# syamajala/cholesky

Measured on AMD Instinct MI355X. Metric: fp64 factorization GF/s (numeric level loop, F_ref flops) on 3-D Laplacian, higher is better.
Workload: dtype f64; 1 GPU; tests/lapl_3375x3375 (reference fixture: 7-point Laplacian, nested-dissection ordering from the fixture files); n=3375, levels=5, separators=31, B_alg_bytes=2932064, parallelism=single GPU, precision=fp64

## Files before the change

### cholesky_amd/_lib.py

```python
import ctypes as C
import os

_HERE = os.path.dirname(os.path.abspath(__file__))
LIB_PATH = os.environ.get("CHOLAMD_LIB") or os.path.join(_HERE, "lib", "libcholamd.so")
HEADER_PATH = os.path.join(os.path.dirname(_HERE), "include", "cholamd.h")


class Filled(C.Structure):
    _fields_ = [("filled", C.c_int), ("sep_x", C.c_int), ("sep_y", C.c_int), ("interval", C.c_int), ("cluster", C.c_int),
                ("lo_x", C.c_int), ("lo_y", C.c_int), ("hi_x", C.c_int), ("hi_y", C.c_int)]


class Op(C.Structure):
    _fields_ = [("op", C.c_int), ("level", C.c_int), ("m", C.c_int), ("n", C.c_int), ("k", C.c_int),
                ("a_sx", C.c_int), ("a_sy", C.c_int), ("a_z", C.c_int), ("b_sx", C.c_int), ("b_sy", C.c_int), ("b_z", C.c_int),
                ("c_sx", C.c_int), ("c_sy", C.c_int), ("c_z", C.c_int)]


class Region(C.Structure):
    _fields_ = [("ptr", C.c_void_p), ("ld", C.c_int), ("lo_x", C.c_int), ("lo_y", C.c_int), ("hi_x", C.c_int), ("hi_y", C.c_int),
                ("tile_row", C.POINTER(C.c_int))]


class SepInfo(C.Structure):
    _fields_ = [("levels", C.c_int), ("num_separators", C.c_int)]


_lib = None


def load():
    global _lib
    if _lib is not None:
        return _lib
    if not os.path.exists(LIB_PATH):
        raise ImportError(f"{LIB_PATH} is missing: run `make` (or __graft_entry__.build()) first; "
                          "cholesky_amd has no fallback path without its HIP library")
    try:
        import torch
    except ImportError:
        pass
    L = C.CDLL(LIB_PATH)
    vp, ci, cd, i64 = C.c_void_p, C.c_int, C.c_double, C.c_int64
    L.cholamd_last_error.restype = C.c_char_p
    L.cholamd_version.restype = C.c_char_p
    L.cholamd_read_separators.argtypes = [C.c_char_p, ci, vp, vp, C.POINTER(SepInfo)]
    L.cholamd_read_clusters.argtypes = [C.c_char_p, vp, vp, vp, i64, C.POINTER(i64)]
    L.cholamd_read_matrix.argtypes = [C.c_char_p, ci, vp, vp, vp]
    L.cholamd_read_vector.argtypes = [C.c_char_p, ci, vp]
    L.cholamd_write_solution.argtypes = [C.c_char_p, vp, ci, ci]
    L.cholamd_plan_create.argtypes = [C.c_char_p, C.c_char_p, C.c_char_p, C.POINTER(vp)]
    L.cholamd_plan_create_from_arrays.argtypes = [ci, ci, vp, vp, vp, vp, vp, i64, i64, vp, vp, vp, C.c_char_p, C.POINTER(vp)]
    L.cholamd_plan_destroy.argtypes = [vp]
    L.cholamd_generate_laplacian.argtypes = [ci, ci, ci, ci, ci, C.POINTER(vp)]
    L.cholamd_problem_destroy.argtypes = [vp]
    L.cholamd_problem_n.argtypes = [vp]
    L.cholamd_problem_nz.argtypes = [vp]
    L.cholamd_problem_write.argtypes = [vp, C.c_char_p]
    L.cholamd_plan_create_from_problem.argtypes = [vp, C.POINTER(vp)]
    L.cholamd_problem_rhs.argtypes = [vp, vp]
    for f in ("n", "nz", "levels", "num_separators", "max_int_size", "num_blocks"):
        getattr(L, "cholamd_plan_" + f).argtypes = [vp]
    for f in ("arena_doubles", "dropped_entries", "num_ops", "nnz_a", "nnz_l", "alg_bytes"):
        fn = getattr(L, "cholamd_plan_" + f)
        fn.argtypes = [vp]
        fn.restype = i64
    L.cholamd_plan_nnz_tiles.argtypes = [vp]
    L.cholamd_plan_nnz_tiles.restype = i64
    L.cholamd_plan_fmin.argtypes = [vp]
    L.cholamd_plan_fmin.restype = cd
    L.cholamd_plan_banner.argtypes = [vp]
    L.cholamd_plan_banner.restype = C.c_char_p
    for f in ("perm", "sep_sizes", "sep_offsets", "tree", "blocks", "ops"):
        getattr(L, "cholamd_plan_" + f).argtypes = [vp, vp]
    L.cholamd_plan_snapshot_count.argtypes = [vp, ci]
    L.cholamd_plan_snapshot_count.restype = i64
    L.cholamd_plan_snapshot.argtypes = [vp, ci, vp]
    L.cholamd_plan_counts.argtypes = [vp, ci, vp, vp]
    L.cholamd_plan_flops.argtypes = [vp]
    L.cholamd_plan_flops.restype = cd
    L.cholamd_plan_fill_host.argtypes = [vp, vp]
    L.cholamd_plan_arena_to_dense.argtypes = [vp, vp, vp]
    L.cholamd_plan_entries.argtypes = [vp, vp, vp]
    L.cholamd_plan_value_map.argtypes = [vp, vp]
    L.cholamd_plan_fill_host_values.argtypes = [vp, vp, i64, vp]
    L.cholamd_device_set_values.argtypes = [vp, vp, i64, ci, vp]
    L.cholamd_device_values_status.argtypes = [vp, vp, vp]
    L.cholamd_plan_fill_host_part.argtypes = [vp, vp, ci, ci, C.POINTER(i64)]
    L.cholamd_plan_level_work_counts.argtypes = [vp, ci, ci, ci, vp]
    L.cholamd_plan_level_work_volume.argtypes = [vp, ci, ci, ci, ci, vp]
    L.cholamd_plan_program_check.argtypes = [vp, ci, ci]
    L.cholamd_plan_program_check_opts.argtypes = [vp, ci, ci, ci, ci]
    L.cholamd_plan_program_counts.argtypes = [vp, ci, vp]
    L.cholamd_plan_program_jobs.argtypes = [vp, ci, i64, vp]
    L.cholamd_plan_program_jobs.restype = i64
    L.cholamd_plan_write_matrix.argtypes = [vp, vp, C.c_char_p, ci]
    L.cholamd_plan_write_debug_log.argtypes = [vp, vp]
    L.cholamd_device_create.argtypes = [vp, ci, C.POINTER(vp)]
    L.cholamd_device_destroy.argtypes = [vp]
    L.cholamd_device_set_partition.argtypes = [vp, ci, ci]
    L.cholamd_device_set_option.argtypes = [vp, C.c_char_p, ci]
    L.cholamd_comm_unique_id.argtypes = [vp]
    L.cholamd_comm_create.argtypes = [vp, ci, ci, vp, C.POINTER(vp)]
    L.cholamd_comm_create_local.argtypes = [vp, ci, vp]
    L.cholamd_factor_multi.argtypes = [vp, vp, vp, ci, vp]
    L.cholamd_gather_factor.argtypes = [vp, vp, ci, vp]
    L.cholamd_comm_adopt.argtypes = [vp, ci, ci, C.POINTER(vp)]
    L.cholamd_comm_destroy.argtypes = [vp]
    L.cholamd_comm_destroy.restype = None
    L.cholamd_comm_allreduce.argtypes = [vp, vp, i64, vp]
    L.cholamd_device_tail_offset.argtypes = [vp]
    L.cholamd_device_tail_offset.restype = i64
    L.cholamd_exchange_tail.argtypes = [vp, vp, vp, vp]
    L.cholamd_factor_sharded.argtypes = [vp, vp, vp, vp]
    L.cholamd_factor_sharded_f32.argtypes = [vp, vp, vp, vp]
    L.cholamd_gather_to_root.argtypes = [vp, vp, ci, vp, vp]
    L.cholamd_exchange_volume.argtypes = [vp, vp]
    L.cholamd_plan_exchange_volume.argtypes = [vp, ci, ci, ci, vp]
    L.cholamd_plan_exchange_pieces.argtypes = [vp, ci, ci, ci, vp]
    L.cholamd_plan_solve_counts.argtypes = [vp, ci, ci, ci, vp]
    L.cholamd_plan_solve_skips.argtypes = [vp, ci, vp, vp]
    L.cholamd_solve_sharded.argtypes = [vp, vp, vp, vp, vp, vp]
    L.cholamd_solve_sharded_f32.argtypes = [vp, vp, vp, vp, vp, vp]
    L.cholamd_solve_refine_sharded.argtypes = [vp, vp, vp, vp, ci, C.c_double, vp, vp, vp, vp]
    L.cholamd_solve_multi.argtypes = [vp, vp, vp, vp, vp, ci, vp]
    L.cholamd_solve_refine_multi.argtypes = [vp, vp, vp, vp, ci, C.c_double, vp, vp, vp, ci, vp]
    L.cholamd_follow_rounds.argtypes = [ci, ci, ci, vp, vp]
    L.cholamd_plan_program_followers.argtypes = [vp, i64, vp]
    L.cholamd_plan_program_followers.restype = i64
    L.cholamd_factor_multi_f32.argtypes = [vp, vp, vp, ci, vp]
    L.cholamd_gather_factor_f32.argtypes = [vp, vp, ci, vp]
    L.cholamd_device_alloc.argtypes = [vp, i64, C.POINTER(vp)]
    L.cholamd_device_free.argtypes = [vp, vp]
    L.cholamd_device_upload.argtypes = [vp, vp, vp, i64, vp]
    L.cholamd_device_download.argtypes = [vp, vp, vp, i64, vp]
    L.cholamd_device_sync.argtypes = [vp, vp]
    L.cholamd_device_fill.argtypes = [vp, vp, vp]
    L.cholamd_factor.argtypes = [vp, vp, vp]
    L.cholamd_factor_levels.argtypes = [vp, vp, ci, ci, vp]
    L.cholamd_device_program_trace.argtypes = [vp, vp, vp, i64, vp, C.POINTER(ci)]
    L.cholamd_factor_info.argtypes = [vp, C.POINTER(ci)]
    L.cholamd_solve.argtypes = [vp, vp, vp, vp, vp]
    L.cholamd_device_fill_f32.argtypes = [vp, vp, vp]
    L.cholamd_factor_f32.argtypes = [vp, vp, vp]
    L.cholamd_factor_levels_f32.argtypes = [vp, vp, ci, ci, vp]
    L.cholamd_solve_f32.argtypes = [vp, vp, vp, vp, vp]
    L.cholamd_solve_refine.argtypes = [vp, vp, vp, vp, ci, cd, C.POINTER(ci), C.POINTER(cd), vp]
    L.cholamd_residual.argtypes = [vp, vp, vp, vp, C.POINTER(cd), vp]
    L.cholamd_solve_nrhs.argtypes = [vp, vp, vp, i64, vp, i64, ci, vp]
    L.cholamd_solve_nrhs_f32.argtypes = [vp, vp, vp, i64, vp, i64, ci, vp]
    L.cholamd_solve_refine_nrhs.argtypes = [vp, vp, vp, i64, vp, i64, ci, ci, cd, C.POINTER(ci), vp, vp]
    L.cholamd_solve_half.argtypes = [vp, vp, vp, vp, ci, vp]
    L.cholamd_solve_half_f32.argtypes = [vp, vp, vp, vp, ci, vp]
    L.cholamd_solve_half_nrhs.argtypes = [vp, vp, vp, i64, vp, i64, ci, ci, vp]
    L.cholamd_solve_half_nrhs_f32.argtypes = [vp, vp, vp, i64, vp, i64, ci, ci, vp]
    L.cholamd_factor_logdet.argtypes = [vp, vp, C.POINTER(cd), vp]
    L.cholamd_factor_logdet_f32.argtypes = [vp, vp, C.POINTER(cd), vp]
    L.cholamd_factor_diag.argtypes = [vp, vp, vp, vp]
    L.cholamd_factor_diag_f32.argtypes = [vp, vp, vp, vp]
    L.cholamd_plan_diag_list.argtypes = [vp, vp, vp, vp, vp, vp, vp]
    L.cholamd_selinv.argtypes = [vp, vp, vp, vp]
    L.cholamd_selinv_diag.argtypes = [vp, vp, vp, vp]
    L.cholamd_selinv_entries.argtypes = [vp, vp, vp, i64, vp]
    L.cholamd_plan_selinv_blocks.argtypes = [vp, ci]
    L.cholamd_plan_selinv_front.argtypes = [vp, ci, ci, ci, vp, vp, vp]
    L.cholamd_device_alloc_arena.argtypes = [vp, ci, C.POINTER(vp), C.POINTER(C.c_int64)]
    L.cholamd_device_free_arena.argtypes = [vp, vp]
    L.cholamd_device_set_timing.argtypes = [vp, ci]
    L.cholamd_device_get_timing.argtypes = [vp, vp, vp]
    L.cholamd_device_get_timing_ex.argtypes = [vp, vp, vp]
    L.cholamd_device_bcast_phases.argtypes = [vp]
    L.cholamd_comm_count.argtypes = [vp, C.POINTER(ci)]
    L.cholamd_device_event_overhead.argtypes = [vp, vp, C.POINTER(C.c_float)]
    RP, FP = C.POINTER(Region), C.POINTER(Filled)
    L.cholamd_plan_region.argtypes = [vp, vp, ci, ci, RP]
    L.cholamd_plan_level_work_volume_opts.argtypes = [vp, ci, ci, ci, vp]
    L.cholamd_plan_level_mt_fill.argtypes = [vp, ci, vp]
    L.cholamd_plan_arena_dense_doubles.argtypes = [vp]
    L.cholamd_plan_arena_dense_doubles.restype = C.c_int64
    L.cholamd_plan_block_tile_map.argtypes = [vp, ci, ci, vp]
    L.cholamd_fused_dpotrf.argtypes = [RP, FP, ci, ci, ci, ci, vp]
    L.cholamd_fused_dtrsm.argtypes = [RP, RP, FP, ci, FP, ci, ci, ci, ci, vp]
    L.cholamd_fused_dsyrk.argtypes = [RP, RP, RP, FP, ci, FP, ci, FP, ci, ci, ci, ci, ci, vp]
    L.cholamd_fused_dgemm.argtypes = [RP, RP, RP, FP, ci, FP, ci, FP, ci, ci, ci, ci, ci, vp]
    L.cholamd_LAPACKE_dpotrf.argtypes = [ci, C.c_char, ci, vp, ci]
    L.cholamd_cblas_dtrsm.argtypes = [ci, ci, ci, ci, ci, ci, ci, cd, vp, ci, vp, ci]
    L.cholamd_cblas_dtrsm.restype = None
    L.cholamd_cblas_dgemm.argtypes = [ci, ci, ci, ci, ci, ci, cd, vp, ci, vp, ci, cd, vp, ci]
    L.cholamd_cblas_dgemm.restype = None
    L.cholamd_cblas_dsyrk.argtypes = [ci, ci, ci, ci, ci, cd, vp, ci, cd, vp, ci]
    L.cholamd_cblas_dsyrk.restype = None
    L.cholamd_cblas_dtrsv.argtypes = [ci, ci, ci, ci, ci, vp, ci, vp, ci]
    L.cholamd_cblas_dtrsv.restype = None
    L.cholamd_cblas_dgemv.argtypes = [ci, ci, ci, ci, cd, vp, ci, vp, ci, cd, vp, ci]
    L.cholamd_cblas_dgemv.restype = None
    L.cholamd_openblas_set_num_threads.argtypes = [ci]
    L.cholamd_openblas_set_num_threads.restype = None
    L.cholamd_dpotrf_dev.argtypes = [ci, vp, ci, vp, vp]
    L.cholamd_dtrsm_dev.argtypes = [ci, ci, vp, ci, vp, ci, vp]
    L.cholamd_dgemm_dev.argtypes = [ci, ci, ci, vp, ci, vp, ci, vp, ci, vp]
    L.cholamd_dsyrk_dev.argtypes = [ci, ci, vp, ci, vp, ci, vp]
    L.cholamd_dtrsv_dev.argtypes = [ci, ci, vp, ci, vp, vp]
    L.cholamd_dgemv_dev.argtypes = [ci, ci, ci, vp, ci, vp, vp, vp]
    _lib = L
    return L


class CholamdError(RuntimeError):
    pass


def check(rc, what=""):
    if rc != 0:
        msg = load().cholamd_last_error().decode(errors="replace")
        raise CholamdError(f"{what} failed with code {rc}: {msg}")
```

### cholesky_amd/csrc/chol_api.cpp

```cpp
#include <hip/hip_runtime.h>
#include <rccl/rccl.h>

#include <cstdio>
#include <algorithm>
#include <cstdlib>
#include <cfloat>
#include <cmath>
#include <cstring>
#include <string>
#include <type_traits>
#include <vector>

#include "chol_kernels.h"
#include "chol_plan.h"
#include "cholamd.h"

#define HIPCHK(call)                                                                                  \
  do {                                                                                                \
    hipError_t e_ = (call);                                                                           \
    if (e_ != hipSuccess) {                                                                           \
      chol_set_error("%s failed: %s (%s:%d)", #call, hipGetErrorString(e_), __FILE__, __LINE__);     \
      return (e_ == hipErrorNoDevice || e_ == hipErrorInvalidDevice) ? CHOLAMD_ERR_NO_DEVICE : CHOLAMD_ERR_HIP; \
    }                                                                                                 \
  } while (0)

struct level_dev {
  int n_potrf = 0, n_trsm = 0, n_task = 0, n_src = 0;
  std::vector<chol_phase> phase;
  chol_potrf_desc *potrf = nullptr;
  chol_trsm_desc *trsm = nullptr;
  chol_upd_task *task = nullptr, *task_mt = nullptr;
  chol_upd_src *src = nullptr;
  std::vector<chol_bcast> bcast;
};
struct solve_dev {
  int n_trsv = 0, n_grp = 0, n_fw = 0, n_bw = 0;
  chol_trsv_desc *trsv = nullptr;
  chol_gemv_desc *fw = nullptr, *bw = nullptr;
  int *grp_start = nullptr, *grp_rows = nullptr, *bw_start = nullptr;
  int n_ifw = 0, n_ibw = 0, max_n = 0, max_under = 0;
  int64_t w256_off = -1;
  int *ifw = nullptr, *ibw = nullptr;
};
struct selinv_dev {
  std::vector<chol_selinv_sep> host;
  chol_selinv_sep *sep = nullptr; chol_selinv_tile *tile = nullptr;
  int *chain_ld = nullptr, *chain_pos0 = nullptr; int64_t *rowoff = nullptr;
  int max_nblk = 0;
};
struct timed_launch { hipEvent_t a, b; int kind; };

struct cholamd_device {
  struct vmm_arena { void *va; size_t total; std::vector<hipMemGenericAllocationHandle_t> handles; };
  std::vector<vmm_arena> vmm;

  const cholamd_plan *plan = nullptr;
  int dev = 0, rank = 0, world = 1;
  std::vector<level_dev> lv;
  std::vector<solve_dev> sv;
  bool solve_ready = false;
  int solve_rank = 0, solve_world = 1;
  int *zr_sub = nullptr; int n_zr_sub = 0;
  double *ws = nullptr;
  double *ws_solve = nullptr;
  int *step_flags = nullptr;
  int step_gen = 0;
  double *w256 = nullptr;
  double *step_xt = nullptr;
  bool keep_inverses = false;
  int *info = nullptr;
  int *info_last = nullptr;
  int info_parity = 0; bool info_foreign = false;
  int *progress = nullptr;
  int epoch = 0, done_total = 0;
  int64_t *a_dst = nullptr; double *a_val = nullptr; int *perm = nullptr; double *ytmp = nullptr;
  int64_t *top_dst[2] = { nullptr, nullptr }; double *top_val[2] = { nullptr, nullptr }; int *top_e[2] = { nullptr, nullptr }; int64_t top_n[2] = { 0, 0 }; int top_gen[2] = { -1, -1 };
  int *a_src = nullptr, *csr_src = nullptr; unsigned char *e_cls = nullptr;
  int64_t *vs_dev = nullptr, *vs_init = nullptr, *vs_host = nullptr;
  int64_t vs_last[4] = { 0, 0, 0, 0 };
  bool vs_called = false, vs_last_valid = false;
  bool vs_in_force = false;
  bool f32_pending = false;
  bool timing = false;
  std::vector<timed_launch> tl;
  std::vector<hipEvent_t> pool;
  level_dev prog;
  chol_job *jobs = nullptr; chol_wait *pwaits = nullptr; chol_ext *exts = nullptr;
  int *pctr = nullptr, *pctr_total = nullptr;
  int n_job = 0, n_pctr = 0, prog_grid = 0, prog_epoch = 0, prog_epoch_limit = 0;
  bool prog_ready = false;
  unsigned long long *trace = nullptr;
  std::vector<chol_job> jobs_host;
  std::vector<level_dev> lv32;
  float *ws32 = nullptr;
  int f32_range = -1; int64_t f32_bad = -1;
  int64_t *csr_ptr = nullptr; int *csr_col = nullptr; double *csr_val = nullptr;
  double *rvec = nullptr, *dxvec = nullptr, *partial = nullptr;
  void *xstage = nullptr; size_t xstage_bytes = 0; void *xdesc = nullptr; int xdesc_gen = -1, xdesc_elem = 0, sched_gen = 0;
  chol_sched_opts opt;
  bool solve_reference_shape = false;
  double *ynrhs = nullptr, *bnrhs = nullptr, *rnrhs = nullptr, *dxnrhs = nullptr, *pnrhs = nullptr;
  chol_trsv_desc *dg_desc = nullptr; int *dg_prefix = nullptr; int n_dg = 0;
  double *ld_part = nullptr; int64_t *ld_ipart = nullptr, *ld_res = nullptr;
  std::vector<selinv_dev> si; double *si_ws = nullptr; bool si_ready = false;
};

static int no_device_error()
{
  chol_set_error("no usable HIP device (libcholamd has no CPU fallback)");
  return CHOLAMD_ERR_NO_DEVICE;
}

extern "C" int cholamd_device_count(void)
{
  int n = 0;
  if (hipGetDeviceCount(&n) != hipSuccess) return 0;
  return n;
}

template <class T> static int upload_vec(T **dptr, const T *h, size_t n)
{
  *dptr = nullptr;
  if (n == 0) return 0;
  HIPCHK(hipMalloc((void **)dptr, n * sizeof(T)));
  HIPCHK(hipMemcpy(*dptr, h, n * sizeof(T), hipMemcpyHostToDevice));
  return 0;
}

#define CHOL_POISON_GUARD ((size_t)64 << 10)
static bool poison_on()
{
  const char *e = std::getenv("CHOLAMD_POISON");
  return e && *e && atoi(e) != 0;
}
static hipError_t poison_fill(void *p, size_t bytes)
{
  hipError_t e = hipMemset(p, 0xFF, bytes);
  return e == hipSuccess ? hipDeviceSynchronize() : e;
}
static hipError_t fp_malloc(void **dptr, size_t bytes)
{
  if (!poison_on()) return hipMalloc(dptr, bytes);
  hipError_t e = hipMalloc(dptr, bytes + CHOL_POISON_GUARD);
  return e == hipSuccess ? poison_fill(*dptr, bytes + CHOL_POISON_GUARD) : e;
}

static void free_level(level_dev &l)
{
  (void)hipFree(l.potrf); (void)hipFree(l.trsm); (void)hipFree(l.task); (void)hipFree(l.task_mt); (void)hipFree(l.src);
  l = level_dev();
}
static void free_levels(cholamd_device *d)
{
  for (auto &l : d->lv) free_level(l);
  d->lv.clear();
  for (auto &l : d->lv32) free_level(l);
  d->lv32.clear();
  free_level(d->prog);
  (void)hipFree(d->jobs); (void)hipFree(d->pwaits); (void)hipFree(d->exts); (void)hipFree(d->pctr); (void)hipFree(d->pctr_total);
  d->jobs = nullptr; d->pwaits = nullptr; d->exts = nullptr; d->pctr = nullptr; d->pctr_total = nullptr;
  d->prog_ready = false;
}
static void free_solve_lists(cholamd_device *d)
{
  for (auto &s : d->sv) { (void)hipFree(s.trsv); (void)hipFree(s.fw); (void)hipFree(s.bw); (void)hipFree(s.grp_start); (void)hipFree(s.grp_rows); (void)hipFree(s.bw_start); (void)hipFree(s.ifw); (void)hipFree(s.ibw); }
  d->sv.clear();
  (void)hipFree(d->w256); d->w256 = nullptr;
  (void)hipFree(d->dg_desc); d->dg_desc = nullptr; (void)hipFree(d->dg_prefix); d->dg_prefix = nullptr; d->n_dg = 0;
  (void)hipFree(d->zr_sub); d->zr_sub = nullptr; d->n_zr_sub = 0;
  d->solve_ready = false;
}
static void free_selinv(cholamd_device *d)
{
  for (auto &l : d->si) { (void)hipFree(l.sep); (void)hipFree(l.tile); (void)hipFree(l.chain_ld); (void)hipFree(l.chain_pos0); (void)hipFree(l.rowoff); }
  d->si.clear();
  (void)hipFree(d->si_ws); d->si_ws = nullptr;
  d->si_ready = false;
}
static int upload_level(level_dev &l, const chol_level_work &w, bool with_tables = true)
{
  l.n_potrf = w.n_potrf; l.n_trsm = w.n_trsm; l.n_task = w.n_task; l.n_src = w.n_src;
  l.phase.assign(w.phase, w.phase + w.n_phase);
  l.bcast.assign(w.bcast, w.bcast + w.n_bcast);
  int rc = 0;
  if (w.n_potrf > 0 && with_tables && !std::getenv("CHOLAMD_NO_ROLE_TABLES")) {
    const size_t dbytes = ((size_t)w.n_potrf * sizeof(chol_potrf_desc) + 15) / 16 * 16;
    std::vector<unsigned char> buf(dbytes + (size_t)w.n_potrf * CHOL_RR_TAB_BYTES);
    for (int i = 0; i < w.n_potrf; i++) {
      chol_potrf_desc pd = w.potrf[i];
      if (pd.n <= CHOL_RR_MAXN) {
        const size_t at = dbytes + (size_t)i * CHOL_RR_TAB_BYTES;
        pd.tab = (int)(at - (size_t)i * sizeof(chol_potrf_desc));
        chol_potrf_table(pd.n, pd.sky, buf.data() + at);
      }
      std::memcpy(buf.data() + (size_t)i * sizeof(chol_potrf_desc), &pd, sizeof pd);
    }
    HIPCHK(hipMalloc((void **)&l.potrf, buf.size()));
    HIPCHK(hipMemcpy(l.potrf, buf.data(), buf.size(), hipMemcpyHostToDevice));
  } else rc = upload_vec(&l.potrf, w.potrf, (size_t)w.n_potrf);
  if (!rc) rc = upload_vec(&l.trsm, w.trsm, (size_t)w.n_trsm);
  if (!rc) rc = upload_vec(&l.task, w.task, (size_t)w.n_task);
  if (!rc) rc = upload_vec(&l.task_mt, w.task_mt, (size_t)w.n_task_mt);
  if (!rc) rc = upload_vec(&l.src, w.src, (size_t)w.n_src);
  return rc;
}

static int build_levels(cholamd_device *d)
{
  free_levels(d);
  d->sched_gen++;
  const int L = d->plan->levels;
  d->lv.resize(L);
  for (int lvl = 0; lvl < L; lvl++) {
    chol_level_work w;
    int rc = chol_build_level_work(d->plan, &d->opt, lvl, d->rank, d->world, &w);
    if (rc) return rc;
    rc = upload_level(d->lv[lvl], w);
    chol_level_work_free(&w);
    if (rc) return rc;
  }
  if (d->world == 1 && d->opt.program) {
    chol_level_work w;
    chol_program g;
    const bool built = chol_build_program(d->plan, &d->opt, &w, &g) == 0;
    const bool live = built && chol_program_check_built(d->plan, &d->opt, 4, &w, &g) == 0;
    if (built && !live) { chol_level_work_free(&w); chol_program_free(&g); }
    if (live) {
      int rc = upload_level(d->prog, w);
      std::vector<int> tot(g.ctr_total, g.ctr_total + g.n_ctr);
      int ncu = 256;
      hipDeviceProp_t prop;
      if (hipGetDeviceProperties(&prop, d->dev) == hipSuccess && prop.multiProcessorCount > 0) ncu = prop.multiProcessorCount;
      d->prog_grid = g.n_job < ncu ? g.n_job : ncu;
      tot.push_back(g.n_job + d->prog_grid);
      int mx = 1;
      for (int t : tot) mx = t > mx ? t : mx;
      d->prog_epoch_limit = (1 << 30) / mx;
      d->n_job = g.n_job; d->n_pctr = (int)tot.size(); d->prog_epoch = 0;
      d->jobs_host.assign(g.job, g.job + g.n_job);
      if (!rc) rc = upload_vec(&d->jobs, g.job, (size_t)g.n_job);
      const chol_wait no_wait = { 0, 0 };
      chol_ext no_ext;
      std::memset(&no_ext, 0, sizeof no_ext);
      if (!rc) rc = g.n_wait > 0 ? upload_vec(&d->pwaits, g.wait, (size_t)g.n_wait) : upload_vec(&d->pwaits, &no_wait, (size_t)1);
      if (!rc) rc = g.n_ext > 0 ? upload_vec(&d->exts, g.ext, (size_t)g.n_ext) : upload_vec(&d->exts, &no_ext, (size_t)1);
      if (!rc) rc = upload_vec(&d->pctr_total, tot.data(), tot.size());
      if (!rc) {
        HIPCHK(hipMalloc((void **)&d->pctr, tot.size() * sizeof(int)));
        HIPCHK(hipMemset(d->pctr, 0, tot.size() * sizeof(int)));
      }
      chol_level_work_free(&w);
      chol_program_free(&g);
      if (rc) return rc;
      d->prog_ready = d->n_job > 0;
    }
  }
  return 0;
}

extern "C" int cholamd_device_create(const cholamd_plan *plan, int device_id, cholamd_device **out)
{
  *out = nullptr;
  if (!plan) { chol_set_error("null plan"); return CHOLAMD_ERR_ARG; }
  int ndev = 0;
  if (hipGetDeviceCount(&ndev) != hipSuccess || ndev <= 0) return no_device_error();
  if (device_id < 0 || device_id >= ndev) { chol_set_error("device %d out of range (%d devices)", device_id, ndev); return CHOLAMD_ERR_NO_DEVICE; }
  HIPCHK(hipSetDevice(device_id));
  cholamd_device *d = new cholamd_device();
  d->plan = plan; d->dev = device_id;
  chol_sched_opts_from_env(&d->opt);
  { const char *e = getenv("CHOLAMD_SOLVE_REFERENCE_SHAPE"); d->solve_reference_shape = e && *e && atoi(e) != 0; }
  int rc = build_levels(d);
  if (!rc) {
    hipError_t e = fp_malloc((void **)&d->ws, (size_t)(plan->ws_doubles > 0 ? plan->ws_doubles : 1) * sizeof(double));
    if (e == hipSuccess) e = hipMalloc((void **)&d->info, 4 * sizeof(int));
    if (e == hipSuccess) e = hipMemset(d->info, 0, 4 * sizeof(int));
    if (e == hipSuccess) e = hipMalloc((void **)&d->progress, (size_t)(plan->nsep + 2) * sizeof(int));
    if (e == hipSuccess) e = hipMemset(d->progress, 0, (size_t)(plan->nsep + 2) * sizeof(int));
    if (e != hipSuccess) { chol_set_error("hipMalloc: %s", hipGetErrorString(e)); rc = CHOLAMD_ERR_HIP; }
  }
  if (!rc) rc = upload_vec(&d->a_dst, plan->a_dst, (size_t)plan->nnz_a);
  if (!rc) rc = upload_vec(&d->a_val, plan->a_val, (size_t)plan->nnz_a);
  if (!rc) rc = upload_vec(&d->perm, plan->perm, (size_t)plan->n);
  if (rc) { cholamd_device_destroy(d); return rc; }
  *out = d;
  return 0;
}

extern "C" void cholamd_device_destroy(cholamd_device *d)
{
  if (!d) return;
  (void)hipSetDevice(d->dev);
  free_levels(d);
  for (auto &a : d->vmm) {
    (void)hipDeviceSynchronize();
    (void)hipMemUnmap(a.va, a.total);
    for (auto h : a.handles) (void)hipMemRelease(h);
    (void)hipMemAddressFree(a.va, a.total);
  }
  free_solve_lists(d);
  free_selinv(d);
  (void)hipFree(d->ws32); (void)hipFree(d->csr_ptr); (void)hipFree(d->csr_col); (void)hipFree(d->csr_val); (void)hipFree(d->rvec); (void)hipFree(d->dxvec); (void)hipFree(d->partial);
  (void)hipFree(d->xstage); (void)hipFree(d->xdesc);
  (void)hipFree(d->ws); (void)hipFree(d->ws_solve); (void)hipFree(d->step_flags); (void)hipFree(d->w256); (void)hipFree(d->step_xt); (void)hipFree(d->info); (void)hipFree(d->progress); (void)hipFree(d->a_dst); (void)hipFree(d->a_val); (void)hipFree(d->perm); (void)hipFree(d->ytmp);
  (void)hipFree(d->ld_part); (void)hipFree(d->ld_ipart); (void)hipFree(d->ld_res);
  (void)hipFree(d->ynrhs); (void)hipFree(d->bnrhs); (void)hipFree(d->rnrhs); (void)hipFree(d->dxnrhs); (void)hipFree(d->pnrhs);
  for (int q = 0; q < 2; q++) { (void)hipFree(d->top_dst[q]); (void)hipFree(d->top_val[q]); (void)hipFree(d->top_e[q]); }
  (void)hipFree(d->a_src); (void)hipFree(d->csr_src); (void)hipFree(d->e_cls); (void)hipFree(d->vs_dev); (void)hipFree(d->vs_init); (void)hipHostFree(d->vs_host);
  for (auto &t : d->tl) { d->pool.push_back(t.a); d->pool.push_back(t.b); }
  for (auto e : d->pool) (void)hipEventDestroy(e);
  delete d;
}

extern "C" int cholamd_device_set_partition(cholamd_device *d, int rank, int world)
{
  HIPCHK(hipSetDevice(d->dev));
  if (world < 1 || (world & (world - 1)) || rank < 0 || rank >= world || chol_split_level(world) > d->plan->levels - 1) {
    chol_set_error("bad partition: rank %d of %d for a %d-level tree", rank, world, d->plan->levels);
    return CHOLAMD_ERR_ARG;
  }
  d->rank = rank; d->world = world;
  free_solve_lists(d);
  return build_levels(d);
}

extern "C" int cholamd_device_bcast_phases(const cholamd_device *d)
{
  int n = 0;
  for (const level_dev &l : d->lv) for (const chol_phase &ph : l.phase) n += ph.kind == 6;
  return n;
}
extern "C" int cholamd_device_set_option(cholamd_device *d, const char *name, int value)
{
  HIPCHK(hipSetDevice(d->dev));
  const std::string n(name ? name : "");
  bool rebuild = true;
  if (n == "split_min") d->opt.split_min = value;
  else if (n == "split_nb") d->opt.split_nb = value;
  else if (n == "fuse") d->opt.fuse = value != 0;
  else if (n == "fuse_update_max") d->opt.fuse_update_max = value;
  else if (n == "mt_min_tiles") d->opt.mt_min_tiles = value;
  else if (n == "cells") d->opt.cells = value != 0;
  else if (n == "program") d->opt.program = value != 0;
  else if (n == "follow") d->opt.follow = value != 0;
  else if (n == "super_blocks") d->opt.super_blocks = value;
  else if (n == "follow_tail") d->opt.follow_tail = value;
  else if (n == "follow_tail_split") d->opt.follow_tail_split = value;
  else if (n == "staged") d->opt.staged = value != 0;
  else if (n == "fine_upd") d->opt.fine_upd = value != 0;
  else if (n == "skyline") d->opt.skyline = value != 0;
  else if (n == "merge_targets") d->opt.merge_targets = value != 0;
  else if (n == "leaf_envelope") d->opt.leaf_envelope = value != 0;
  else if (n == "trsm_wt_min") d->opt.trsm_wt_min = value < 0 ? 0 : value;
  else if (n == "stage_chunk") d->opt.stage_chunk = value < 0 ? 0 : value;
  else if (n == "dist_top") d->opt.dist_top = value;
  else if (n == "solve_reference_shape") { d->solve_reference_shape = value != 0; rebuild = false; }
  else { chol_set_error("unknown option '%s'", n.c_str()); return CHOLAMD_ERR_ARG; }
  return rebuild ? build_levels(d) : 0;
}

extern "C" int cholamd_device_alloc(cholamd_device *d, int64_t doubles, double **dptr)
{
  HIPCHK(hipSetDevice(d->dev));
  HIPCHK(fp_malloc((void **)dptr, (size_t)doubles * sizeof(double)));
  return 0;
}
extern "C" int cholamd_device_free(cholamd_device *d, double *dptr)
{
  HIPCHK(hipSetDevice(d->dev));
  HIPCHK(hipFree(dptr));
  return 0;
}
extern "C" int cholamd_device_upload(cholamd_device *d, double *d_dst, const double *h_src, int64_t doubles, void *stream)
{
  HIPCHK(hipSetDevice(d->dev));
  HIPCHK(hipMemcpyAsync(d_dst, h_src, (size_t)doubles * sizeof(double), hipMemcpyHostToDevice, (hipStream_t)stream));
  HIPCHK(hipStreamSynchronize((hipStream_t)stream));
  return 0;
}
extern "C" int cholamd_device_download(cholamd_device *d, double *h_dst, const double *d_src, int64_t doubles, void *stream)
{
  HIPCHK(hipSetDevice(d->dev));
  HIPCHK(hipMemcpyAsync(h_dst, d_src, (size_t)doubles * sizeof(double), hipMemcpyDeviceToHost, (hipStream_t)stream));
  HIPCHK(hipStreamSynchronize((hipStream_t)stream));
  return 0;
}
extern "C" int cholamd_device_sync(cholamd_device *d, void *stream)
{
  HIPCHK(hipSetDevice(d->dev));
  HIPCHK(hipStreamSynchronize((hipStream_t)stream));
  return 0;
}

static void owned_ranges(const cholamd_device *d, std::vector<std::pair<int64_t, int64_t>> &out)
{
  const cholamd_plan *p = d->plan;
  out.clear();
  if (d->world <= 1 || d->rank == 0) { out.push_back({ 0, p->arena }); return; }
  for (int s = 1; s <= p->nsep; s++) {
    const int o = chol_owner_of(p, s, d->world);
    if (o >= 0 && o != d->rank) continue;
    const int64_t lo = p->panel_off[s], hi = s < p->nsep ? p->panel_off[s + 1] : p->arena;
    if (!out.empty() && out.back().second == lo) out.back().second = hi; else out.push_back({ lo, hi });
  }
}
static int clear_owned(cholamd_device *d, void *arena, size_t elem, hipStream_t st)
{
  bool sharded = false;
  for (const auto &v : d->vmm) if (v.va == arena) sharded = true;
  if (!sharded) { HIPCHK(hipMemsetAsync(arena, 0, (size_t)d->plan->arena * elem, st)); return 0; }
  std::vector<std::pair<int64_t, int64_t>> r;
  owned_ranges(d, r);
  for (auto &x : r) HIPCHK(hipMemsetAsync((char *)arena + (size_t)x.first * elem, 0, (size_t)(x.second - x.first) * elem, st));
  return 0;
}
#define CHOL_VMM_CHUNK ((size_t)2 << 20)
#define CHOL_VMM_SCRATCH ((size_t)64 << 20)
extern "C" int cholamd_device_alloc_arena(cholamd_device *d, int elem_bytes, void **dptr, int64_t *backed_bytes)
{
  HIPCHK(hipSetDevice(d->dev));
  if (elem_bytes != 4 && elem_bytes != 8) { chol_set_error("alloc_arena: element size %d", elem_bytes); return CHOLAMD_ERR_ARG; }
  const size_t full = (size_t)d->plan->arena * (size_t)elem_bytes;
  if (d->world <= 1 || d->rank == 0) {
    HIPCHK(fp_malloc(dptr, full > 0 ? full : 1));
    if (backed_bytes) *backed_bytes = (int64_t)full;
    return 0;
  }
  hipMemAllocationProp prop = {};
// ... 141 lines not shown
{
  float ms[CHOL_TIMING_KINDS]; int n[CHOL_TIMING_KINDS];
  const int rc = cholamd_device_get_timing_ex(d, ms, n);
  if (rc) return rc;
  for (int k = 0; k < 4; k++) { ms_by_kind[k] = ms[k]; launches_by_kind[k] = n[k]; }
  return 0;
}

extern "C" int cholamd_device_event_overhead(cholamd_device *d, void *stream, float *ms_out)
{
  HIPCHK(hipSetDevice(d->dev));
  hipStream_t st = (hipStream_t)stream;
  const int reps = 64;
  std::vector<hipEvent_t> ev(2 * reps);
  for (auto &e : ev) e = get_event(d);
  for (int i = 0; i < reps; i++) { HIPCHK(hipEventRecord(ev[2 * i], st)); HIPCHK(hipEventRecord(ev[2 * i + 1], st)); }
  HIPCHK(hipStreamSynchronize(st));
  double acc = 0.0;
  for (int i = 0; i < reps; i++) { float ms = 0.f; HIPCHK(hipEventElapsedTime(&ms, ev[2 * i], ev[2 * i + 1])); acc += ms; }
  for (auto e : ev) d->pool.push_back(e);
  *ms_out = (float)(acc / reps);
  return 0;
}

static int launch_phase(cholamd_device *d, const level_dev &l, const chol_phase &ph, double *d_arena, hipStream_t st)
{
  if (ph.kind == 5) {
    if (d->epoch >= (1 << 24) || d->done_total >= (1 << 30)) { HIPCHK(hipMemsetAsync(d->progress, 0, (size_t)(d->plan->nsep + 2) * sizeof(int), st)); d->epoch = 0; d->done_total = 0; }
    d->epoch++;
    if (ph.n3 > 0) d->done_total += (ph.n2 + 2) / 3;
    HIPCHK((hipError_t)chol_launch_potrf_trsm(d_arena, d->ws, l.potrf + ph.first, ph.n, l.trsm + ph.first2, ph.n2, l.task + ph.first3, l.src, ph.n3,
                                              d->info, d->progress, d->epoch * 64, d->progress + d->plan->nsep + 1, d->done_total, st));
  } else if (ph.kind == 0) HIPCHK((hipError_t)chol_launch_potrf(d_arena, d->ws, l.potrf + ph.first, ph.n, d->info, st));
  else if (ph.kind == 1) HIPCHK((hipError_t)chol_launch_trsm(d_arena, d->ws, l.trsm + ph.first, ph.n, st));
  else if (ph.kind == 4) HIPCHK((hipError_t)chol_launch_trsm_w(d_arena, d->ws, l.trsm + ph.first, ph.n, st));
  else if (ph.kind == 7) HIPCHK((hipError_t)chol_launch_trsm_wt(d_arena, d->ws, l.trsm + ph.first, ph.n, st));
  else if (ph.kind == 2) HIPCHK((hipError_t)chol_launch_update(d_arena, l.task + ph.first, l.src, ph.n, st));
  else if (ph.kind == 3) HIPCHK((hipError_t)chol_launch_update_mt(d_arena, l.task_mt + ph.first, l.src, ph.n, (int64_t)d->plan->arena, st));
  return 0;
}
struct cholamd_comm;
static int bcast_rank(cholamd_device *d, const level_dev &l, const chol_phase &ph, double *d_arena, cholamd_comm *c, hipStream_t st);
static int factor_levels_comm(cholamd_device *d, double *d_arena, int level_hi, int level_lo, cholamd_comm *c, hipStream_t st)
{
  HIPCHK(hipSetDevice(d->dev));
  const int L = d->plan->levels;
  if (level_hi >= L) level_hi = L - 1;
  if (level_lo < 0) level_lo = 0;
  if (level_hi == L - 1) HIPCHK(hipMemsetAsync(d->info, 0, 2 * sizeof(int), st));
  d->info_last = d->info; d->info_foreign = true;
  for (int lvl = level_hi; lvl >= level_lo; lvl--) {
    const level_dev &l = d->lv[lvl];
    for (const chol_phase &ph : l.phase) {
      if (ph.kind == 6) {
        scoped_timer t(d, st, CHOL_TK_BCAST, ph.n > 0);
        int rc = bcast_rank(d, l, ph, d_arena, c, st);
        if (rc) return rc;
        continue;
      }
      scoped_timer t(d, st, ph.kind == 3 ? 2 : (ph.kind == 4 || ph.kind == 7) ? 1 : ph.kind == 5 ? 0 : ph.kind, ph.n > 0);
      int rc = launch_phase(d, l, ph, d_arena, st);
      if (rc) return rc;
    }
  }
  return 0;
}
extern "C" int cholamd_factor_levels(cholamd_device *d, double *d_arena, int level_hi, int level_lo, void *stream)
{
  return factor_levels_comm(d, d_arena, level_hi, level_lo, nullptr, (hipStream_t)stream);
}
extern "C" int cholamd_factor(cholamd_device *d, double *d_arena, void *stream)
{
  if (!d->prog_ready) return cholamd_factor_levels(d, d_arena, d->plan->levels - 1, 0, stream);
  HIPCHK(hipSetDevice(d->dev));
  hipStream_t st = (hipStream_t)stream;
  if (d->info_foreign) { HIPCHK(hipMemsetAsync(d->info, 0, 4 * sizeof(int), st)); d->info_foreign = false; }
  int *const info_cur = d->info + 2 * d->info_parity, *const info_next = d->info + 2 * (d->info_parity ^ 1);
  d->info_parity ^= 1; d->info_last = info_cur;
  if (d->prog_epoch >= d->prog_epoch_limit) { HIPCHK(hipMemsetAsync(d->pctr, 0, (size_t)d->n_pctr * sizeof(int), st)); d->prog_epoch = 0; }
  const level_dev &l = d->prog;
  {
    scoped_timer t(d, st, 3, true);
    HIPCHK((hipError_t)chol_launch_program(d_arena, d->ws, d->jobs, d->n_job, d->pwaits, l.potrf, l.trsm, l.task, l.src, d->exts, d->pctr, d->pctr_total, d->prog_epoch,
                                           d->pctr + d->n_pctr - 1, d->prog_epoch * (d->n_job + d->prog_grid), d->prog_grid, info_cur, info_next, d->trace, st));
  }
  d->prog_epoch++;
  return 0;
}
extern "C" int cholamd_device_program_trace(cholamd_device *d, double *d_arena, void *stream, int64_t cap, int64_t *out, int *njobs_out)
{
  HIPCHK(hipSetDevice(d->dev));
  if (!d->prog_ready) { chol_set_error("no program launch for this problem / these options"); return CHOLAMD_ERR_ARG; }
  *njobs_out = d->n_job;
  if (cap < (int64_t)5 * d->n_job) return 0;
  const size_t nst = (size_t)(4 + CHOL_TRACE_X) * d->n_job;
  HIPCHK(hipMalloc((void **)&d->trace, nst * sizeof(unsigned long long)));
  HIPCHK(hipMemset(d->trace, 0, nst * sizeof(unsigned long long)));
  int rc = cholamd_factor(d, d_arena, stream);
  std::vector<unsigned long long> h(nst);
  if (!rc) {
    HIPCHK(hipStreamSynchronize((hipStream_t)stream));
    HIPCHK(hipMemcpy(h.data(), d->trace, h.size() * sizeof(unsigned long long), hipMemcpyDeviceToHost));
  }
  (void)hipFree(d->trace);
  d->trace = nullptr;
  if (rc) return rc;
  unsigned long long t0 = ~0ull;
  for (int j = 0; j < d->n_job; j++) if (h[4 * j] && h[4 * j] < t0) t0 = h[4 * j];
  for (int j = 0; j < d->n_job; j++) {
    out[5 * j] = d->jobs_host[j].kind + (d->jobs_host[j].kind == 0 && d->jobs_host[j].n_ext > 0 ? 10 : 0);
    for (int q = 0; q < 3; q++) out[5 * j + 1 + q] = (int64_t)(h[4 * j + q] - t0);
    out[5 * j + 4] = (int64_t)h[4 * j + 3];
  }
  if (const char *path = getenv("CHOLAMD_TRACE_FOLLOW")) {
    if (FILE *fp = fopen(path, "w")) {
      for (int j = 0; j < d->n_job; j++) {
        const unsigned long long *x = &h[(size_t)4 * d->n_job + (size_t)CHOL_TRACE_X * j];
        const int kind = d->jobs_host[j].kind;
        bool any = false;
        for (int i = 0; i < CHOL_TRACE_X; i++) any = any || x[i] != 0;
        if (kind == 2 || !any) continue;
        fprintf(fp, "job %d kind %d", j, kind);
        if (kind == 0 && x[1]) {
          fprintf(fp, " items %llu own-tiles-wait-over %.1f rounds:", x[1], x[0] ? (double)(x[0] - t0) * 0.01 : -1.0);
          for (unsigned long long i = 0; i < x[1] && i < 44; i++) if (x[2 + i]) fprintf(fp, " %llu:%.1f", i, (double)(x[2 + i] - t0) * 0.01);
        }
        if (kind == 0 && x[24]) { fprintf(fp, " | prologue (entry, LDS init, tables, slot tables read, columns 0-1 requested, tiles requested, columns 0-1 parked):"); const int ord[7] = { 0, 1, 2, 5, 6, 3, 4 }; for (int k = 0; k < 7; k++) fprintf(fp, " %.1f", x[24 + ord[k]] ? (double)(x[24 + ord[k]] - t0) * 0.01 : -1.0); }
        fprintf(fp, kind == 0 ? " | column started:" : " | POTRF column seen:");
        for (int k = 0; k < 24; k++) if (x[72 + k]) fprintf(fp, " %d:%.1f", k, (double)(x[72 + k] - t0) * 0.01);
        fprintf(fp, kind == 0 ? " | column published:" : " | column tile on the channel:");
        for (int k = 0; k < 24; k++) if (x[48 + k]) fprintf(fp, " %d:%.1f", k, (double)(x[48 + k] - t0) * 0.01);
        fprintf(fp, "\n");
      }
      fclose(fp);
    }
  }
  return 0;
}
extern "C" int cholamd_factor_info(cholamd_device *d, int *sep_out)
{
  HIPCHK(hipSetDevice(d->dev));
  int h[2] = { 0, 0 };
  HIPCHK(hipMemcpy(h, d->info_last ? d->info_last : d->info, sizeof h, hipMemcpyDeviceToHost));
  if (sep_out) *sep_out = h[1];
  if (h[0] == CHOLAMD_ERR_STALL)
    chol_set_error("factorisation stalled: a workgroup of a fused launch waited ~50 ms for a progress word of the same launch and gave up; the factor is not valid");
  else if (h[0] < 0) chol_set_error("factorisation failed with internal code %d", h[0]);
  return h[0];
}

__global__ void k_zero_ranges(double *y, const int *ranges, int nr)
{
  const int off = ranges[2 * blockIdx.y], len = ranges[2 * blockIdx.y + 1];
  for (int i = blockIdx.x * blockDim.x + threadIdx.x; i < len; i += gridDim.x * blockDim.x) y[off + i] = 0.0;
}
static int build_solve(cholamd_device *d, int rank = 0, int world = 1)
{
  const int L = d->plan->levels;
  if (d->solve_ready && d->solve_rank == rank && d->solve_world == world) return 0;
  free_solve_lists(d);
  d->solve_rank = rank; d->solve_world = world;
  d->sv.resize(L);
  if (world > 1) {
    const cholamd_plan *p = d->plan;
    std::vector<int> zr;
    for (int s = 1; s <= p->nsep; s++) {
      const int o = chol_owner_of(p, s, world);
      if ((o >= 0 && o != rank) || (o < 0 && rank != 0)) {
        if (!zr.empty() && zr[zr.size() - 2] + zr.back() == p->sep_off[s]) zr.back() += p->sep_size[s];
        else { zr.push_back(p->sep_off[s]); zr.push_back(p->sep_size[s]); }
      }
    }
    d->n_zr_sub = (int)zr.size() / 2;
    if (!zr.empty()) { int rc = upload_vec(&d->zr_sub, zr.data(), zr.size()); if (rc) return rc; }
  }
  std::vector<chol_trsv_desc> diag;
  for (int lvl = 0; lvl < L; lvl++) {
    chol_solve_level w;
    int rc = chol_build_solve_level_part(d->plan, lvl, rank, world, &w);
    if (rc) return rc;
    if (world == 1) diag.insert(diag.end(), w.trsv, w.trsv + w.n_trsv);
    solve_dev &s = d->sv[lvl];
    s.n_trsv = w.n_trsv; s.n_grp = w.n_grp; s.n_fw = w.n_fw; s.n_bw = w.n_bw;
    rc = upload_vec(&s.trsv, w.trsv, (size_t)w.n_trsv);
    if (!rc) rc = upload_vec(&s.fw, w.fw, (size_t)w.n_fw);
    if (!rc) rc = upload_vec(&s.bw, w.bw, (size_t)w.n_bw);
    if (!rc) rc = upload_vec(&s.grp_start, w.grp_start, (size_t)w.n_grp + 1);
    if (!rc) rc = upload_vec(&s.grp_rows, w.grp_rows, (size_t)2 * w.n_grp);
    if (!rc) rc = upload_vec(&s.bw_start, w.bw_start, (size_t)w.n_trsv + 1);
    s.n_ifw = w.n_ifw; s.n_ibw = w.n_ibw; s.max_n = w.max_n; s.max_under = w.banded && w.max_rows_under_span > 0 ? -w.max_rows_under_span : w.max_rows_under_span;
    if (!rc) rc = upload_vec(&s.ifw, w.ifw, (size_t)4 * w.n_ifw);
    if (!rc) rc = upload_vec(&s.ibw, w.ibw, (size_t)4 * w.n_ibw);
    chol_solve_level_free(&w);
    if (rc) return rc;
  }
  if (!diag.empty()) {
    std::vector<int> prefix(diag.size() + 1);
    int rc = chol_diag_list(d->plan, diag.data(), (int)diag.size(), prefix.data());
    if (!rc) rc = upload_vec(&d->dg_desc, diag.data(), diag.size());
    if (!rc) rc = upload_vec(&d->dg_prefix, prefix.data(), prefix.size());
    if (rc) return rc;
    d->n_dg = (int)diag.size();
  }
  if (!d->ytmp) HIPCHK(fp_malloc((void **)&d->ytmp, (size_t)d->plan->n * sizeof(double)));
  if (!d->ws_solve) HIPCHK(fp_malloc((void **)&d->ws_solve, (size_t)(d->plan->ws_doubles > 0 ? d->plan->ws_doubles : 1) * sizeof(double)));
  if (!d->step_flags) { HIPCHK(hipMalloc((void **)&d->step_flags, CHOL_STEPW_MAX_SEPS * 16 * sizeof(int))); HIPCHK(hipMemset(d->step_flags, 0, CHOL_STEPW_MAX_SEPS * 16 * sizeof(int))); }
  if (!d->step_xt) { HIPCHK(fp_malloc((void **)&d->step_xt, CHOL_STEPW_MAX_SEPS * 256 * sizeof(double))); HIPCHK(hipMemset(d->step_xt, 0, CHOL_STEPW_MAX_SEPS * 256 * sizeof(double))); }
  int64_t w256 = 0;
  if (!std::getenv("CHOLAMD_SOLVE_NO_INV256"))
    for (int lvl = 0; lvl < L; lvl++) {
      solve_dev &s = d->sv[lvl];
      if (s.n_trsv < 1 || s.n_trsv > CHOL_STEPW_MAX_SEPS || s.max_n <= 256 || s.max_under < 0) continue;
      s.w256_off = w256;
      w256 += (int64_t)s.n_trsv * ((s.max_n + 255) / 256) * 65536;
    }
  if (w256 > 0) HIPCHK(fp_malloc((void **)&d->w256, (size_t)w256 * sizeof(double)));
  d->solve_ready = true;
  return 0;
}

// ... 1889 lines not shown
```

### cholesky_amd/csrc/chol_kernels.h

```cpp
#ifndef CHOL_KERNELS_H
#define CHOL_KERNELS_H
#include <hip/hip_runtime_api.h>
#include <stdint.h>
#include "chol_plan.h"
#ifdef __cplusplus
extern "C" {
#endif
int chol_launch_scatter(double *arena, const int64_t *dst, const double *val, int64_t nnz, hipStream_t st);
#define CHOL_VALUES_STATUS 1
#define CHOL_VALUES_GATHER 2
int chol_launch_set_values(const double *vals, int64_t nz, const unsigned char *cls, double *a_val, const int *a_src, int64_t nnz_a,
                           double *csr_val, const int *csr_src, int64_t ncsr, int parts, int64_t *status, hipStream_t st);
int chol_launch_gather(double *out, const double *in, const int *idx, int64_t n, hipStream_t st);
int chol_launch_potrf(double *base, double *ws, const chol_potrf_desc *descs, int n, int *info, hipStream_t st);
int chol_launch_potrf_big(double *base, double *ws, const chol_potrf_desc *descs, int n, int *info, hipStream_t st);
int chol_launch_potrf_trsm(double *base, double *ws, const chol_potrf_desc *pdescs, int n_potrf, const chol_trsm_desc *tdescs, int n_trsm,
                           const chol_upd_task *tasks, const chol_upd_src *srcs, int n_task,
                           int *info, int *progress, int progress_base, int *done, int done_target, hipStream_t st);
int chol_launch_program(double *base, double *ws, const chol_job *jobs, int njobs, const chol_wait *waits, const chol_potrf_desc *pdescs, const chol_trsm_desc *tdescs,
                        const chol_upd_task *tasks, const chol_upd_src *srcs, const chol_ext *exts, int *ctr, const int *ctr_total, int epoch, int *head, int head_base,
                        int grid, int *info, int *info_next, unsigned long long *trace, hipStream_t st);
int chol_launch_trsm_w(double *base, const double *ws, const chol_trsm_desc *descs, int n, hipStream_t st);
int chol_launch_trsm_wt(double *base, const double *ws, const chol_trsm_desc *descs, int n, hipStream_t st);
int chol_launch_trsm_big(double *base, const double *ws, const chol_trsm_desc *descs, int n, hipStream_t st);
int chol_launch_dinv(const double *L, int n, int ldl, double *W, hipStream_t st);
int chol_launch_trsm(double *base, const double *ws, const chol_trsm_desc *descs, int n, hipStream_t st);
int chol_launch_update(double *base, const chol_upd_task *tasks, const chol_upd_src *srcs, int ntask, hipStream_t st);
int chol_launch_update_mt(double *base, const chol_upd_task *tasks, const chol_upd_src *srcs, int ntask, int64_t arena_elems, hipStream_t st);
int chol_launch_permute(const double *in, const int *perm, double *out, int n, int inverse, hipStream_t st);
int chol_launch_solve_dinv(const double *base, const chol_trsv_desc *descs, int n, int max_n, double *W, hipStream_t st);
int chol_launch_solve_trsv(const double *base, const chol_trsv_desc *descs, int n, int max_n, int max_under, const double *W, double *y, int backward, int *flags, int *gen, const double *W256, double *xt, hipStream_t st);
#define CHOL_STEPW_MAX_SEPS 128
int chol_launch_solve_inv256(const double *base, const chol_trsv_desc *descs, int n, int max_n, const double *W16, double *W256, hipStream_t st);
int chol32_launch_solve_inv256(const float *base, const chol_trsv_desc *descs, int n, int max_n, const double *W16, double *W256, hipStream_t st);
int chol_launch_solve_offdiag(const double *base, const chol_gemv_desc *blocks, const int *items, int n_items, double *y, int backward, hipStream_t st);
int chol_launch_trsv_fwd(const double *base, const chol_trsv_desc *descs, int n, double *y, hipStream_t st);
int chol_launch_gemv_fwd(const double *base, const chol_gemv_desc *descs, const int *grp_start, const int *grp_rows, int ngroups, double *y, hipStream_t st);
int chol_launch_bwd(const double *base, const chol_trsv_desc *descs, const chol_gemv_desc *gd, const int *gstart, int n, double *y, hipStream_t st);
int chol32_launch_scatter(float *arena, const int64_t *dst, const double *val, int64_t nnz, hipStream_t st);
int chol32_launch_potrf(float *base, float *ws, const chol_potrf_desc *descs, int n, int *info, hipStream_t st);
int chol32_launch_trsm(float *base, const float *ws, const chol_trsm_desc *descs, int n, hipStream_t st);
int chol32_launch_trsm_wt(float *base, const float *ws, const chol_trsm_desc *descs, int n, hipStream_t st);
int chol32_launch_update(float *base, const chol_upd_task *tasks, const chol_upd_src *srcs, int ntask, hipStream_t st);
int chol32_launch_update_mt(float *base, const chol_upd_task *tasks, const chol_upd_src *srcs, int ntask, int64_t arena_elems, hipStream_t st);
int chol32_launch_solve_dinv(const float *base, const chol_trsv_desc *descs, int n, int max_n, double *W, hipStream_t st);
int chol32_launch_solve_trsv(const float *base, const chol_trsv_desc *descs, int n, int max_n, int max_under, const double *W, double *y, int backward, int *flags, int *gen, const double *W256, double *xt, hipStream_t st);
int chol32_launch_solve_offdiag(const float *base, const chol_gemv_desc *blocks, const int *items, int n_items, double *y, int backward, hipStream_t st);
int chol_launch_residual(const int64_t *ptr, const int *col, const double *val, const double *b, const double *x, double *r, int n, double *partial, hipStream_t st);
int chol_launch_axpy1(double *x, const double *dx, int n, hipStream_t st);
#define CHOL_NRHS_W 32
int chol_nrhs_launch_permute(const double *B, int64_t ldb, const int *perm, double *Y, double *X, int64_t ldx, int n, int c0, int cols, int inverse, hipStream_t st);
int chol_nrhs_launch_trsv(const double *base, const chol_trsv_desc *descs, int n, int max_n, int max_under, const double *W16, const double *W256, double *Y, int backward, hipStream_t st);
int chol32_nrhs_launch_trsv(const float *base, const chol_trsv_desc *descs, int n, int max_n, int max_under, const double *W16, const double *W256, double *Y, int backward, hipStream_t st);
int chol_nrhs_launch_offdiag(const double *base, const chol_gemv_desc *blocks, const int *items, int n_items, double *Y, int backward, hipStream_t st);
int chol32_nrhs_launch_offdiag(const float *base, const chol_gemv_desc *blocks, const int *items, int n_items, double *Y, int backward, hipStream_t st);
int chol_nrhs_launch_residual(const int64_t *ptr, const int *col, const double *val, const double *B, int64_t ldb, const double *X, int64_t ldx, double *R, int64_t ldr,
                              int n, int cols, double *partial, hipStream_t st);
int chol_nrhs_launch_axpy(double *X, int64_t ldx, const double *D, int64_t ldd, int n, int cols, hipStream_t st);
#define CHOL_LOGDET_MAX_BLOCKS 1024
int chol_launch_factor_diag(const double *base, const chol_trsv_desc *descs, const int *prefix, int nd, int n, const int *perm, double *diag, hipStream_t st);
int chol32_launch_factor_diag(const float *base, const chol_trsv_desc *descs, const int *prefix, int nd, int n, const int *perm, double *diag, hipStream_t st);
int chol_launch_factor_logdet(const double *base, const chol_trsv_desc *descs, const int *prefix, int nd, int n, double *part, int64_t *ipart, int64_t *res, hipStream_t st);
int chol32_launch_factor_logdet(const float *base, const chol_trsv_desc *descs, const int *prefix, int nd, int n, double *part, int64_t *ipart, int64_t *res, hipStream_t st);
int chol_launch_selinv_step(const double *L, double *Z, double *ws, const chol_selinv_sep *seps, int n_act, const chol_selinv_tile *tiles, const int *chain_ld,
                            const int *chain_pos0, const int64_t *rowoff, int step, int max_below_tiles, hipStream_t st);
int chol_launch_selinv_entries(const double *Z, const int64_t *a_dst, const int *a_src, int64_t nnz, double *vals, int64_t nz, hipStream_t st);
#define CHOL_TRACE_X 96
#ifdef __cplusplus
}
#endif
#endif
```

### cholesky_amd/csrc/chol_kernels.hip

```cpp
#include <hip/hip_runtime.h>
#include <float.h>
#include <stdint.h>

#include "chol_plan.h"
#include "chol_kernels.h"

typedef double d4 __attribute__((ext_vector_type(4)));

__device__ __forceinline__ void lds_barrier()
{
  asm volatile("s_waitcnt lgkmcnt(0)\n\ts_barrier" ::: "memory");
}


template <bool PUB> __device__ __forceinline__ void gstore(double *p, double v)
{
  if (PUB) __hip_atomic_store(p, v, __ATOMIC_RELAXED, __HIP_MEMORY_SCOPE_AGENT);
  else *p = v;
}
template <bool PUB> __device__ __forceinline__ double gload(const double *p)
{
  if (PUB) return __hip_atomic_load(p, __ATOMIC_RELAXED, __HIP_MEMORY_SCOPE_AGENT);
  return *p;
}
// ... 1495 lines not shown
          const d4 x = solve16(tile[s1], wpre);
          tile[s1] = x;
          PUBLISH_X(J + 1, x);
        }
      } else {
        if (J >= 1 && (J & 3) == wave) {
#pragma unroll
          for (int s = 0; s < SLOTS; ++s) {
            const int J2 = wave + 4 * s;
            if (J2 > J && J2 < T && J2 <= J - 1 + bw) APPLY_X(J - 1, s);
          }
        }
#pragma unroll
        for (int s = 0; s < SLOTS; ++s) {
          const int J2 = wave + 4 * s;
          if (J2 > J + 1 && J2 < T && J2 <= J + bw) APPLY_X(J, s);
        }
      }
      STAMP(2);
      if ((J + 2 < T) && (((J + 2) & 3) == wave)) LOAD_W(J + 2, wpre);
      LOAD_L(J + 2, lpre[(J + 2) % 3]);
      STAMP(3);
    }
  }
  if (wave == 1 && blockIdx.x == 0) { STAMP_FLUSH; }
#undef LOAD_L
#undef LOAD_W
#undef PUBLISH_X
#undef APPLY_X
#undef LS
#undef VOFF
}

__global__ __launch_bounds__(256) void k_trsm_rr(double *__restrict__ base, const double *__restrict__ ws,
                                                 const chol_trsm_desc *__restrict__ descs)
{
  __shared__ double sX[3][TS * TS];
  trsm_rr_body<false, TRSM_SLOTS>(base, ws, descs[blockIdx.x], sX, __builtin_amdgcn_readfirstlane(threadIdx.x >> 6), threadIdx.x & 63, nullptr, 0, nullptr);
}

#define FUSED_SLOTS ((CHOL_FUSE_MAXN / TS + 3) / 4)
__global__ __launch_bounds__(RR_THREADS) void k_potrf_trsm(double *__restrict__ base, double *__restrict__ ws,
                                                           const chol_potrf_desc *__restrict__ pdescs, int n_potrf,
                                                           const chol_trsm_desc *__restrict__ tdescs, int n_trsm,
                                                           const chol_upd_task *__restrict__ tasks, const chol_upd_src *__restrict__ srcs, int n_task, int n_upd_wg,
                                                           int *__restrict__ info, int *__restrict__ progress, int progress_base,
                                                           int *__restrict__ done, int done_target)
{
  __shared__ double smem[RR_SMEM_DOUBLES];
  const int wave = __builtin_amdgcn_readfirstlane(threadIdx.x >> 6);
  const int lane = threadIdx.x & 63;
  const int grp = wave >> 2;
  const int n_tg = (n_trsm + 2) / 3;
  if ((int)blockIdx.x < n_potrf) {
    potrf_rr_body<true>(base, ws, pdescs[blockIdx.x], info, progress + blockIdx.x, progress_base, smem, pdescs[blockIdx.x].sky);
  } else if ((int)blockIdx.x < n_potrf + n_tg) {
    double (*sX)[3][TS * TS] = (double (*)[3][TS * TS])smem;
    const int id = ((int)blockIdx.x - n_potrf) * 3 + grp;
    chol_trsm_desc d = tdescs[min(id, n_trsm - 1)];
    if (id >= n_trsm) d.m = 0;
    trsm_rr_body<true, FUSED_SLOTS>(base, ws, d, sX[grp], wave & 3, lane, progress + d.flag, progress_base, info);
    if (n_task > 0) {
      asm volatile("s_waitcnt vmcnt(0)" ::: "memory");
      lds_barrier();
      if (threadIdx.x == 0) __hip_atomic_fetch_add(done, 1, __ATOMIC_RELAXED, __HIP_MEMORY_SCOPE_AGENT);
    }
  } else {
    double (*sAcc)[3][3][4][64] = (double (*)[3][3][4][64])smem;
    const int u = (int)blockIdx.x - n_potrf - n_tg;
    int round = 0;
    for (int t0 = u * 3; t0 < n_task; t0 += n_upd_wg * 3, ++round) {
      const int tid = t0 + grp;
      const bool live = tid < n_task;
      update_task_body<true>(base, tasks[live ? tid : t0], srcs, sAcc[round & 1][grp], wave & 3, lane, live, round == 0 ? done : nullptr, done_target, info);
    }
  }
}

template <bool TR>
__global__ __launch_bounds__(RR_THREADS) void k_program(double *__restrict__ base, double *__restrict__ ws, const chol_job *__restrict__ jobs, int njobs,
                                                        const chol_wait *__restrict__ waits, const chol_potrf_desc *__restrict__ pdescs,
                                                        const chol_trsm_desc *__restrict__ tdescs, const chol_upd_task *__restrict__ tasks,
                                                        const chol_upd_src *__restrict__ srcs, const chol_ext *__restrict__ exts,
                                                        int *__restrict__ ctr, const int *__restrict__ ctr_total, int epoch, int *__restrict__ head, int head_base,
                                                        int *__restrict__ info, int *__restrict__ info_next, unsigned long long *__restrict__ trace)
{
  if (info_next && blockIdx.x == 0 && threadIdx.x == 0) { info_next[0] = 0; info_next[1] = 0; }
  __shared__ double smem[RR_SMEM_DOUBLES];
  __shared__ int s_job;
  const int wave_id = __builtin_amdgcn_readfirstlane(threadIdx.x >> 6);
  for (;;) {
#ifdef TID_PLAIN
    int tid = threadIdx.x;
#else
    int tid = wave_id * 64 + (int)__builtin_amdgcn_mbcnt_hi(~0u, __builtin_amdgcn_mbcnt_lo(~0u, 0u));
#endif
    asm volatile("" : "+v"(tid));
    const int wave = wave_id;
    const int lane = tid & 63;
    const int grp = wave >> 2;
    __syncthreads();
    if (tid == 0) s_job = atomicAdd(head, 1) - head_base;
    __syncthreads();
    const int j = s_job;
    if (j >= njobs) break;
    const chol_job jb = jobs[j];
    if (TR && trace && tid == 0) { trace[4 * j] = __builtin_amdgcn_s_memrealtime(); trace[4 * j + 3] = blockIdx.x; }
    chol_upd_task tpre;
    if (jb.kind == 2) {
      const int tk = jb.first + min(jb.mode == 0 ? wave : grp, jb.n - 1);
      tpre = tasks[tk];
      int touch = 0;
      for (int sx = tpre.src_begin; sx < tpre.src_end; ++sx) touch += srcs[sx].k;
      asm volatile("" :: "s"(touch));
    }
    if (jb.n_pre > 0 && !(jb.kind == 0 && jb.n_ext > 0)) {
      if (wave == 0) wait_list(waits + jb.wait_first, jb.n_pre, ctr, ctr_total, epoch, lane, info);
      lds_barrier();
    }
    if (TR && trace && tid == 0) trace[4 * j + 1] = __builtin_amdgcn_s_memrealtime();
    if (jb.kind == 0) {
      const chol_potrf_desc pd = pdescs[jb.first];
      follow_args fa;
      fa.ext = exts + jb.ext_first; fa.n_ext = jb.n_ext; fa.ctr = ctr; fa.ctr_total = ctr_total; fa.epoch = epoch; fa.wl = waits + jb.wait_first; fa.n_wl = jb.n_wait; fa.stamp = TR && trace ? &trace[4 * j + 1] : nullptr; fa.xstamp = TR && trace ? &trace[4 * njobs + CHOL_TRACE_X * j] : nullptr;
      potrf_rr_body<true, true, TR>(base, ws, pd, info, ctr + pd.ctr, epoch * ctr_total[pd.ctr], smem, pdescs[jb.first].sky, fa, tid);
    } else if (jb.kind == 1) {
      double (*sX)[3][TS * TS] = (double (*)[3][TS * TS])smem;
      chol_trsm_desc d = tdescs[jb.first + min(grp, jb.n - 1)];
      if (grp >= jb.n) d.m = 0;
      if (d.band > 0)
        trsm_rr_body<true, (CHOL_RR_MAXN / TS + 3) / 4, true, TR>(base, ws, d, sX[grp], wave & 3, lane, ctr + d.flag, epoch * ctr_total[d.flag], info, d.chan >= 0 ? ctr + d.chan : nullptr,
                                                                   TR && trace && grp == 0 ? &trace[4 * njobs + CHOL_TRACE_X * j] : nullptr);
      else
        trsm_rr_body<true, FUSED_SLOTS, false, TR>(base, ws, d, sX[grp], wave & 3, lane, ctr + d.flag, epoch * ctr_total[d.flag], info, d.chan >= 0 ? ctr + d.chan : nullptr,
                                                   TR && trace && grp == 0 ? &trace[4 * njobs + CHOL_TRACE_X * j] : nullptr);
    } else {
      stage_waits sw;
      sw.w = waits + jb.wait_first + jb.n_pre; sw.n = jb.n_wait - jb.n_pre; sw.ctr = ctr; sw.ctr_total = ctr_total; sw.epoch = epoch; sw.info = info;
      if (jb.mode == 0) {
        for (int t0 = jb.first; t0 < jb.first + jb.n; t0 += RR_NW + 1) {
          const int tk = t0 + wave;
          if (tk < jb.first + jb.n) update_task_wave<true>(base, t0 == jb.first ? tpre : tasks[tk], srcs, lane, sw);
        }
      } else {
        double (*sAcc)[3][3][4][64] = (double (*)[3][3][4][64])smem;
        int round = 0;
        for (int t0 = jb.first; t0 < jb.first + jb.n; t0 += 3, ++round) {
          const int tk = t0 + grp;
          const bool live = tk < jb.first + jb.n;
          update_task_body<true>(base, t0 == jb.first ? tpre : tasks[live ? tk : t0], srcs, sAcc[round & 1][grp], wave & 3, lane, live, nullptr, 0, info, sw);
        }
      }
    }
    if (jb.sig[0] >= 0) {
      asm volatile("s_waitcnt vmcnt(0)" ::: "memory");
      lds_barrier();
      if (tid == 0) {
        __hip_atomic_fetch_add(&ctr[jb.sig[0]], jb.sig_add, __ATOMIC_RELAXED, __HIP_MEMORY_SCOPE_AGENT);
        if (jb.sig[1] >= 0) __hip_atomic_fetch_add(&ctr[jb.sig[1]], jb.sig_add, __ATOMIC_RELAXED, __HIP_MEMORY_SCOPE_AGENT);
      }
    }
    if (TR && trace && tid == 0) trace[4 * j + 2] = __builtin_amdgcn_s_memrealtime();
  }
}

#define TW_MAXT ((CHOL_TRSM_W_MAXN + TS - 1) / TS)
template <int T, int NT> __device__ __forceinline__ void trsm_w_solve(d4 (&tile)[NT], const double *s0, double *__restrict__ B, int n, int ldb,
                                                              bool vrow, int r15, int g)
{
#pragma unroll
  for (int J = 0; J < T; ++J) {
    const double *sd = s0 + (J * T - J * (J - 1) / 2) * (TS * TS);
    double wv[4];
#pragma unroll
    for (int st = 0; st < 4; ++st) wv[st] = sd[st * 64];
    const d4 x = solve16(tile[J], wv);
    if (vrow) {
      int ro = r15;
      asm volatile("" : "+v"(ro));
#pragma unroll
      for (int q = 0; q < 4; ++q) {
        const int col = J * TS + g + 4 * q;
        if (J + 1 < T || col < n) B[ro + (int64_t)col * ldb] = x[q];
      }
    }
    double nx[4];
#pragma unroll
    for (int st = 0; st < 4; ++st) {
      nx[st] = -x[st];
      asm volatile("" : "+v"(nx[st]));
// ... 1234 lines not shown
    }
  }
  return (int)hipGetLastError();
}
template <class TL> static int launch_solve_inv256_t(const TL *base, const chol_trsv_desc *descs, int n, int max_n, const double *W16, double *W256, hipStream_t st)
{
  if (n <= 0 || max_n <= SSPAN) return 0;
  const int nspan = (max_n + SSPAN - 1) / SSPAN;
  hipLaunchKernelGGL(k_solve_inv256<TL>, dim3(n, nspan, SSPAN / TS), dim3(64), 0, st, base, descs, W16, W256, nspan);
  return (int)hipGetLastError();
}
template <class TL> static int launch_solve_offdiag_t(const TL *base, const chol_gemv_desc *blocks, const int *items, int n_items, double *y, int backward, hipStream_t st)
{
  if (n_items <= 0) return 0;
  if (backward) hipLaunchKernelGGL(k_solve_gather_bwd<TL>, dim3(n_items), dim3(256), 0, st, base, blocks, items, y);
  else hipLaunchKernelGGL(k_solve_gemv_fwd<TL>, dim3(n_items), dim3(256), 0, st, base, blocks, items, y);
  return (int)hipGetLastError();
}

extern "C" {

int chol_launch_scatter(double *arena, const int64_t *dst, const double *val, int64_t nnz, hipStream_t st)
{
  if (nnz <= 0) return 0;
  int blocks = (int)((nnz + 255) / 256);
  if (blocks > 2048) blocks = 2048;
  hipLaunchKernelGGL(k_scatter, dim3(blocks), dim3(256), 0, st, arena, dst, val, nnz);
  return (int)hipGetLastError();
}
int chol_launch_set_values(const double *vals, int64_t nz, const unsigned char *cls, double *a_val, const int *a_src, int64_t nnz_a,
                           double *csr_val, const int *csr_src, int64_t ncsr, int parts, int64_t *status, hipStream_t st)
{
  const int64_t i0 = (parts & CHOL_VALUES_STATUS) ? 0 : nz, i1 = (parts & CHOL_VALUES_GATHER) ? nz + nnz_a + ncsr : nz;
  if (i1 <= i0) return 0;
  int blocks = (int)((i1 - i0 + 255) / 256);
  if (blocks > 2048) blocks = 2048;
  hipLaunchKernelGGL(k_set_values, dim3(blocks), dim3(256), 0, st, vals, nz, cls, a_val, a_src, nnz_a, csr_val, csr_src, i0, i1, status);
  return (int)hipGetLastError();
}
int chol_launch_gather(double *out, const double *in, const int *idx, int64_t n, hipStream_t st)
{
  if (n <= 0) return 0;
  int blocks = (int)((n + 255) / 256);
  if (blocks > 2048) blocks = 2048;
  hipLaunchKernelGGL(k_gather, dim3(blocks), dim3(256), 0, st, out, in, idx, n);
  return (int)hipGetLastError();
}
int chol_launch_potrf(double *base, double *ws, const chol_potrf_desc *descs, int n, int *info, hipStream_t st)
{
  if (n <= 0) return 0;
  hipLaunchKernelGGL(k_potrf_rr, dim3(n), dim3(RR_THREADS), 0, st, base, ws, descs, info);
  return (int)hipGetLastError();
}
int chol_launch_potrf_big(double *base, double *ws, const chol_potrf_desc *descs, int n, int *info, hipStream_t st)
{
  if (n <= 0) return 0;
  hipLaunchKernelGGL(k_potrf_big, dim3(n), dim3(256), 0, st, base, ws, descs, info);
  return (int)hipGetLastError();
}
int chol_launch_dinv(const double *L, int n, int ldl, double *W, hipStream_t st)
{
  if (n <= 0) return 0;
  hipLaunchKernelGGL(k_dinv, dim3((n + TS - 1) / TS), dim3(64), 0, st, L, n, ldl, W);
  return (int)hipGetLastError();
}
int chol_launch_trsm(double *base, const double *ws, const chol_trsm_desc *descs, int n, hipStream_t st)
{
  if (n <= 0) return 0;
  hipLaunchKernelGGL(k_trsm_rr, dim3(n), dim3(256), 0, st, base, ws, descs);
  return (int)hipGetLastError();
}
int chol_launch_potrf_trsm(double *base, double *ws, const chol_potrf_desc *pdescs, int n_potrf, const chol_trsm_desc *tdescs, int n_trsm,
                           const chol_upd_task *tasks, const chol_upd_src *srcs, int n_task,
                           int *info, int *progress, int progress_base, int *done, int done_target, hipStream_t st)
{
  if (n_potrf <= 0) return 0;
  int n_upd_wg = (n_task + 2) / 3;
  if (n_upd_wg > 1024) n_upd_wg = 1024;
  hipLaunchKernelGGL(k_potrf_trsm, dim3(n_potrf + (n_trsm + 2) / 3 + n_upd_wg), dim3(RR_THREADS), 0, st, base, ws, pdescs, n_potrf, tdescs, n_trsm,
                     tasks, srcs, n_task, n_upd_wg, info, progress, progress_base, done, done_target);
  return (int)hipGetLastError();
}
int chol_launch_program(double *base, double *ws, const chol_job *jobs, int njobs, const chol_wait *waits, const chol_potrf_desc *pdescs, const chol_trsm_desc *tdescs,
                        const chol_upd_task *tasks, const chol_upd_src *srcs, const chol_ext *exts, int *ctr, const int *ctr_total, int epoch, int *head, int head_base,
                        int grid, int *info, int *info_next, unsigned long long *trace, hipStream_t st)
{
  if (njobs <= 0) return 0;
  if (trace) hipLaunchKernelGGL(k_program<true>, dim3(grid), dim3(RR_THREADS), 0, st, base, ws, jobs, njobs, waits, pdescs, tdescs, tasks, srcs, exts, ctr, ctr_total, epoch, head, head_base, info, info_next, trace);
  else hipLaunchKernelGGL(k_program<false>, dim3(grid), dim3(RR_THREADS), 0, st, base, ws, jobs, njobs, waits, pdescs, tdescs, tasks, srcs, exts, ctr, ctr_total, epoch, head, head_base, info, info_next, trace);
  return (int)hipGetLastError();
}
int chol_launch_trsm_w(double *base, const double *ws, const chol_trsm_desc *descs, int n, hipStream_t st)
{
  if (n <= 0) return 0;
  hipLaunchKernelGGL(k_trsm_w, dim3((n + 3) / 4), dim3(256), 0, st, base, ws, descs, n);
  return (int)hipGetLastError();
}
int chol_launch_trsm_wt(double *base, const double *ws, const chol_trsm_desc *descs, int n, hipStream_t st)
{
  if (n <= 0) return 0;
  hipLaunchKernelGGL(k_trsm_wt, dim3((n + TT_WAVES - 1) / TT_WAVES), dim3(64 * TT_WAVES), 0, st, base, ws, descs, n);
  return (int)hipGetLastError();
}
int chol_launch_trsm_big(double *base, const double *ws, const chol_trsm_desc *descs, int n, hipStream_t st)
{
  if (n <= 0) return 0;
  hipLaunchKernelGGL(k_trsm_big, dim3((n + 3) / 4), dim3(256), 0, st, base, ws, descs, n);
  return (int)hipGetLastError();
}
int chol_launch_update(double *base, const chol_upd_task *tasks, const chol_upd_src *srcs, int ntask, hipStream_t st)
{
  if (ntask <= 0) return 0;
  const int per_xcd = (ntask + 7) / 8;
  hipLaunchKernelGGL(k_update, dim3(per_xcd * 8), dim3(256), 0, st, base, tasks, srcs, ntask, per_xcd);
  return (int)hipGetLastError();
}
int chol_launch_update_mt(double *base, const chol_upd_task *tasks, const chol_upd_src *srcs, int ntask, int64_t arena_elems, hipStream_t st)
{
  if (ntask <= 0) return 0;
  const int per_xcd = (ntask + 7) / 8;
  hipLaunchKernelGGL(k_update_mt, dim3(per_xcd * 8), dim3(256), 0, st, base, tasks, srcs, ntask, per_xcd, arena_elems);
  return (int)hipGetLastError();
}
int chol_launch_permute(const double *in, const int *perm, double *out, int n, int inverse, hipStream_t st)
{
  if (n <= 0) return 0;
  if (inverse) hipLaunchKernelGGL(k_permute_out, dim3((n + 255) / 256), dim3(256), 0, st, in, perm, out, n);
  else hipLaunchKernelGGL(k_permute_in, dim3((n + 255) / 256), dim3(256), 0, st, in, perm, out, n);
  return (int)hipGetLastError();
}
int chol_launch_solve_dinv(const double *base, const chol_trsv_desc *descs, int n, int max_n, double *W, hipStream_t st) { return launch_solve_dinv_t(base, descs, n, max_n, W, st); }
int chol_launch_solve_trsv(const double *base, const chol_trsv_desc *descs, int n, int max_n, int max_under, const double *W, double *y, int backward, int *flags, int *gen, const double *W256, double *xt, hipStream_t st) { return launch_solve_trsv_t(base, descs, n, max_n, max_under, W, y, backward, flags, gen, W256, xt, st); }
int chol_launch_solve_inv256(const double *base, const chol_trsv_desc *descs, int n, int max_n, const double *W16, double *W256, hipStream_t st) { return launch_solve_inv256_t(base, descs, n, max_n, W16, W256, st); }
int chol32_launch_solve_inv256(const float *base, const chol_trsv_desc *descs, int n, int max_n, const double *W16, double *W256, hipStream_t st) { return launch_solve_inv256_t(base, descs, n, max_n, W16, W256, st); }
int chol_launch_solve_offdiag(const double *base, const chol_gemv_desc *blocks, const int *items, int n_items, double *y, int backward, hipStream_t st) { return launch_solve_offdiag_t(base, blocks, items, n_items, y, backward, st); }
int chol32_launch_solve_dinv(const float *base, const chol_trsv_desc *descs, int n, int max_n, double *W, hipStream_t st) { return launch_solve_dinv_t(base, descs, n, max_n, W, st); }
int chol32_launch_solve_trsv(const float *base, const chol_trsv_desc *descs, int n, int max_n, int max_under, const double *W, double *y, int backward, int *flags, int *gen, const double *W256, double *xt, hipStream_t st) { return launch_solve_trsv_t(base, descs, n, max_n, max_under, W, y, backward, flags, gen, W256, xt, st); }
int chol32_launch_solve_offdiag(const float *base, const chol_gemv_desc *blocks, const int *items, int n_items, double *y, int backward, hipStream_t st) { return launch_solve_offdiag_t(base, blocks, items, n_items, y, backward, st); }
int chol_launch_trsv_fwd(const double *base, const chol_trsv_desc *descs, int n, double *y, hipStream_t st)
{
  if (n <= 0) return 0;
  hipLaunchKernelGGL(k_trsv_fwd, dim3(n), dim3(256), 0, st, base, descs, y);
  return (int)hipGetLastError();
}
int chol_launch_gemv_fwd(const double *base, const chol_gemv_desc *descs, const int *grp_start, const int *grp_rows, int ngroups, double *y, hipStream_t st)
{
  if (ngroups <= 0) return 0;
  hipLaunchKernelGGL(k_gemv_fwd, dim3(ngroups), dim3(256), 0, st, base, descs, grp_start, grp_rows, y);
  return (int)hipGetLastError();
}
int chol_launch_bwd(const double *base, const chol_trsv_desc *descs, const chol_gemv_desc *gd, const int *gstart, int n, double *y, hipStream_t st)
{
  if (n <= 0) return 0;
  hipLaunchKernelGGL(k_bwd, dim3(n), dim3(256), 0, st, base, descs, gd, gstart, y);
  return (int)hipGetLastError();
}

}
```

### cholesky_amd/csrc/chol_plan.h

```cpp
#ifndef CHOL_PLAN_H
#define CHOL_PLAN_H

#include <stdint.h>
#include "cholamd.h"

#ifdef __cplusplus
extern "C" {
#endif

#define CHOL_ENTRY_OUT 0
#define CHOL_ENTRY_IN 1
#define CHOL_ENTRY_DROPPED 2
#define CHOL_NB 16
#define CHOL_RR_MAXN 272
#ifndef CHOL_FOLLOW_ALL_MAXT
#define CHOL_FOLLOW_ALL_MAXT 4
#endif
#define CHOL_FOLLOW_TAIL 3
#define CHOL_FOLLOW_MAXT 10
#define CHOL32_TRSM_GROUP 16
#define CHOL32_MAXN 128

typedef struct {
  int n_int;
// ... 31 lines not shown
#define CHOL_RR_MAXT 17
#define CHOL_RR_NW 11
#define CHOL_RR_NHEAVY 9
#define CHOL_RR_SLOTS 12
#ifndef CHOL_RR_HEAVY_ONLY
#define CHOL_RR_HEAVY_ONLY 36
#endif
#define CHOL_RR_M_SOLVE0 12
#define CHOL_RR_M_SOLVE1 13
#define CHOL_RR_KM_ZERO 0x80
#define CHOL_RR_TAB_MASK 0
#define CHOL_RR_TAB_IJ (CHOL_RR_MAXT * CHOL_RR_NW * 4)
#define CHOL_RR_TAB_KM (CHOL_RR_TAB_IJ + CHOL_RR_SLOTS * CHOL_RR_NW * 2)
#define CHOL_RR_TAB_BYTES ((CHOL_RR_TAB_KM + CHOL_RR_SLOTS * CHOL_RR_NW + 15) / 16 * 16)
#ifdef __HIPCC__
#define CHOL_HD __host__ __device__ __forceinline__
#else
#define CHOL_HD static inline
#endif
CHOL_HD void chol_rr_tile_of_index(int idx, int T, int *ti, int *tj)
{
  int j = 0;
  while (j < T && idx >= T - j) { idx -= T - j; ++j; }
  if (j >= T) { *ti = -1; *tj = 1 << 20; } else { *ti = j + idx; *tj = j; }
}
CHOL_HD void chol_rr_owner(int idx, int ntl2, int *w, int *slot)
{
  if (ntl2 <= CHOL_RR_HEAVY_ONLY) { const int off = idx % CHOL_RR_NHEAVY; *w = off + off / 3; *slot = idx / CHOL_RR_NHEAVY; return; }
  const int cyc = idx / 51, pos = idx % 51;
  const int round = pos < 11 ? 0 : pos < 20 ? 1 : pos < 31 ? 2 : pos < 40 ? 3 : 4;
  const int off = pos - (round == 0 ? 0 : round == 1 ? 11 : round == 2 ? 20 : round == 3 ? 31 : 40);
  if (off < CHOL_RR_NHEAVY) {
    *w = off + off / 3;
    *slot = cyc * 5 + round;
  } else {
    *w = off == CHOL_RR_NHEAVY ? 3 : 7;
    *slot = cyc * 3 + round / 2;
  }
}
void chol_potrf_table(int n, const unsigned char *sky, unsigned char *out);

typedef struct {
  int64_t l_off;
  int64_t dinv_off;
  int64_t b_off;
  int n, ldl, m, ldb;
  int flag;
  int chan;
  int band, pad;
} chol_trsm_desc;

#define CHOL_TRSM_W_MAXN 64
#define CHOL_TRSM_WT_MAXN 144
#define CHOL_TRSM_WT_GROUP 12
#define CHOL_TRSM_WT_MIN 2048
#define CHOL_FUSE_MAXN 192
#define CHOL_FUSE_UPDATE_MAX 0
#define CHOL_TRSM_ROWS 16

typedef struct {
  int64_t a_off, b_off;
  int lda, ldb, k;
  int range;
  int stage, pad;
} chol_upd_src;

typedef struct {
  int64_t c_off;
  int ldc;
  short mv, nv;
  int lower;
  int src_begin, src_end;
  int ar, br;
  int blk;
} chol_upd_task;

typedef struct { int ctr, value; } chol_wait;
typedef struct {
  int kind;
  int first, n;
  int wait_first, n_wait;
  int sig[2], sig_add;
  int ext_first, n_ext;
  int mode, n_pre;
} chol_job;
typedef struct {
  int64_t off;
  int ld, ncol;
  int ctr, need;
} chol_ext;
#define CHOL_FOLLOW_PAIR_MAXT 17
#define CHOL_FOLLOW_SINGLE_TAIL 0
#define CHOL_FOLLOW_OWN_BEFORE 2
#if defined(__HIPCC__)
#define CHOL_HD __host__ __device__ __forceinline__
#else
#define CHOL_HD static inline
#endif
CHOL_HD int chol_follow_round(int i, int n_ext, int T)
{
  const int pair_lim = 2 * T <= CHOL_FOLLOW_PAIR_MAXT ? n_ext - CHOL_FOLLOW_SINGLE_TAIL : 0;
  return i + 1 < pair_lim ? 2 : 1;
}
CHOL_HD int chol_follow_own_at(int n_ext, int T)
{
  int own_at = 0;
  for (int i = 0; i < n_ext; i += chol_follow_round(i, n_ext, T))
    if (i <= n_ext - CHOL_FOLLOW_OWN_BEFORE) own_at = i;
  return own_at;
}

typedef struct {
  int n_job; chol_job *job;
  int n_wait; chol_wait *wait;
  int n_ext; chol_ext *ext;
  int n_ctr; int *ctr_total;
  int follow;
} chol_program;

typedef struct {
  int kind;
  int first, n, first2, n2, first3, n3;
} chol_phase;
typedef struct { int64_t off, count; int owner, heap; } chol_bcast;
static inline unsigned chol_top_contributors(int heap, int world)
{
  int d = 0, l = 0;
  while ((1 << d) < world) d++;
  while ((heap >> (l + 1)) > 0) l++;
  const int lo = (heap << (d - l)) - (1 << d), hi = ((heap + 1) << (d - l)) - (1 << d);
  unsigned m = 0u;
  for (int g = lo; g < hi; g++) m |= 1u << g;
  return m;
}

#define CHOL_DIST_MIN 1024
#define CHOL_MT_MIN_TILES 8192
typedef struct {
  int split_min, split_nb;
  int fuse;
  int fuse_update_max;
  int mt_min_tiles;
  int trsm_group;
  int trsm_wt_min;
  int cells;
  int program;
  int follow;
  int dist_top;
  int skyline;
  int stage_chunk;
  int fine_upd;
  int staged;
  int follow_tail_split;
  int follow_tail;
  int merge_targets;
  int leaf_envelope;
  int super_blocks;
} chol_sched_opts;
#define CHOL_SUPER_BLOCKS 3
#define CHOL_STAGE_CHUNK 0
void chol_sched_opts_default(chol_sched_opts *o);
void chol_sched_opts_from_env(chol_sched_opts *o);

#define CHOL_SPLIT_MIN 144
#ifndef CHOL_PROG_SPLIT_MIN
#define CHOL_PROG_SPLIT_MIN 176
#endif
#define CHOL_SPLIT_NB 144

typedef struct {
  int level;
  int n_phase; chol_phase *phase;
  int n_potrf; chol_potrf_desc *potrf;
  int n_trsm; chol_trsm_desc *trsm;
  int n_task; chol_upd_task *task;
  int n_task_mt; chol_upd_task *task_mt;
  int n_src; chol_upd_src *src;
  int n_bcast; chol_bcast *bcast;
} chol_level_work;

typedef struct {
  int64_t a_off; int n, lda; int x_off; int sep;
  int64_t dinv_off;
  int band;
} chol_trsv_desc;
typedef struct {
  int64_t a_off; int m, n, lda; int x_off, y_off;
  int c_lo;
} chol_gemv_desc;

struct cholamd_plan {
  int n, nz_file, levels, nsep, max_int_size;
  char banner[160];
  MM_typecode typecode;
  int *perm;
  int *iperm;
  int *sep_of_pos;
  int *sep_size, *sep_off;
  int *tree;
  int *heap_of, *level_of;
  chol_clusters *cl;
  int nblk; chol_block *blk;
  int *blk_index;
  int64_t *panel_off; int *panel_ld, *panel_rows;
  int compact;
  int64_t arena_dense;
  int64_t arena;
  int64_t ws_doubles;
  int64_t *dinv_off;
  int64_t nnz_a, dropped; int64_t *a_dst; double *a_val;
  int64_t *csr_ptr; int *csr_col; double *csr_val;
  int *e_row, *e_col, *a_src, *csr_src; unsigned char *e_cls;
  int64_t *snap_n; cholamd_filled **snap;
  int64_t nops, cap_ops; cholamd_op *ops;
  int64_t calls[16][4]; double flops[16][4];
  int64_t nnz_l;
  int64_t nnz_tiles;
  double fmin;
};

int chol_plan_finish(struct cholamd_plan *p, int nz, const int *a_row, const int *a_col, const double *a_val);
const chol_block *chol_plan_block(const struct cholamd_plan *p, int r, int c);
int chol_ntiles(const struct cholamd_plan *p, int sep, int interval);
int chol_build_program(const struct cholamd_plan *p, const chol_sched_opts *opts, chol_level_work *w, chol_program *prog);
void chol_program_free(chol_program *prog);
int chol_program_check(const struct cholamd_plan *p, const chol_sched_opts *opts, int workers);
int chol_program_check_built(const struct cholamd_plan *p, const chol_sched_opts *opts, int workers, const chol_level_work *w, const chol_program *g);
int chol_build_level_work(const struct cholamd_plan *p, const chol_sched_opts *opts , int level, int rank, int world, chol_level_work *out);
void chol_level_work_free(chol_level_work *w);
int chol_owner_of(const struct cholamd_plan *p, int label, int world);
int chol_split_level(int world);
typedef struct {
  int n_trsv; chol_trsv_desc *trsv;
  int n_fw; chol_gemv_desc *fw;
  int n_grp; int *grp_start; int *grp_rows;
  int n_bw; chol_gemv_desc *bw; int *bw_start;
  int n_ifw; int *ifw;
  int n_ibw; int *ibw;
  int max_n;
  int max_rows_under_span;
  int banded;
} chol_solve_level;
#define CHOL_SOLVE_FW_ROWS 256
#define CHOL_SOLVE_BW_ROWS 1024
#define CHOL_SOLVE_BW_COLS 64
#define CHOL_SOLVE_BW_ITEMS 4096
#define CHOL_SOLVE_COLS 1024
int chol_build_solve_level(const struct cholamd_plan *p, int level, chol_solve_level *out);
int chol_build_solve_level_part(const struct cholamd_plan *p, int level, int rank, int world, chol_solve_level *out);
void chol_solve_level_free(chol_solve_level *w);
int chol_diag_list(const struct cholamd_plan *p, chol_trsv_desc *list, int count, int *prefix);

#define CHOL_SELINV_W 64
#define CHOL_SELINV_MAX_TILES 65535
typedef struct { int q0, nrows, pos0, k; } chol_selinv_tile;
typedef struct {
  int64_t panel_off;
  int64_t ws_off;
  int64_t rowoff_first;
  int ld, w, prows, nblk;
  int sep;
  int tile_first, ntile, nown;
  int chain_first, nchain;
  int pad;
} chol_selinv_sep;
typedef struct {
  int level;
  int n_sep; chol_selinv_sep *sep;
  int n_tile; chol_selinv_tile *tile;
  int n_chain; int *chain_ld, *chain_pos0;
  int64_t n_rowoff; int64_t *rowoff;
  int max_nblk, max_tiles;
  int64_t ws_doubles;
} chol_selinv_level;
int chol_build_selinv_level(const struct cholamd_plan *p, int level, chol_selinv_level *out);
void chol_selinv_level_free(chol_selinv_level *w);
void chol_set_error(const char *fmt, ...);

#ifdef __cplusplus
}
#endif
#endif
```

### cholesky_amd/csrc/chol_schedule.c

```c
#define _GNU_SOURCE
#include <stdlib.h>
#include <string.h>

#include "chol_plan.h"
#include "cholamd.h"

typedef struct cholamd_plan plan_t;
#define BIDX(p, r, c) ((p)->blk_index[(size_t)(r) * ((p)->nsep + 1) + (c)])

int chol_split_level(int world)
{
  int d = 0;
  while ((1 << d) < world) d++;
  return d;
}

int chol_owner_of(const plan_t *p, int label, int world)
{
  int d = chol_split_level(world), lvl = p->level_of[label];
  if (lvl < d) return -1;
  return (p->heap_of[label] >> (lvl - d)) - (1 << d);
}

typedef struct {
  int64_t key;
  int64_t seq;
  int64_t c_off, a_off, b_off;
  int ldc, lda, ldb, m, n, k, syrk;
  int bc, crow, ccol;
  int src_sep;
} upd_tuple;

typedef struct { int i, e, bc, crow, ccol, m, n, syrk; int64_t c_off; int ldc, dead; } tgt_group;
static int cmp_group_rows(const void *x, const void *y)
{
  const tgt_group *a = x, *b = y;
  if (a->bc != b->bc) return a->bc < b->bc ? -1 : 1;
  if (a->ccol != b->ccol) return a->ccol < b->ccol ? -1 : 1;
  if (a->n != b->n) return a->n < b->n ? -1 : 1;
  return a->crow < b->crow ? -1 : (a->crow > b->crow);
}
static int cmp_group_first(const void *x, const void *y)
{
  const tgt_group *a = x, *b = y;
  return a->i < b->i ? -1 : (a->i > b->i);
}
static int cmp_group_source(const void *x, const void *y, void *tu_)
{
  const tgt_group *a = x, *b = y;
  const upd_tuple *cmp_group_tu = tu_;
  const int sa = cmp_group_tu[a->i].src_sep, sb = cmp_group_tu[b->i].src_sep;
  if (sa != sb) return sa < sb ? -1 : 1;
  return a->i < b->i ? -1 : (a->i > b->i);
}
static int same_sources(const upd_tuple *tu, const tgt_group *a, const tgt_group *b, int dr, int dc);

static int cmp_tuple(const void *x, const void *y)
{
  const upd_tuple *a = x, *b = y;
  if (a->key != b->key) return a->key < b->key ? -1 : 1;
  return a->seq < b->seq ? -1 : (a->seq > b->seq);
}

static int same_sources(const upd_tuple *tu, const tgt_group *a, const tgt_group *b, int dr, int dc)
{
  if (a->e - a->i != b->e - b->i) return 0;
  for (int q = 0; q < a->e - a->i; q++) {
    const upd_tuple *x = &tu[a->i + q], *y = &tu[b->i + q];
    if (x->src_sep != y->src_sep || x->lda != y->lda || x->ldb != y->ldb || x->k != y->k || y->a_off != x->a_off + dr || y->b_off != x->b_off + dc) return 0;
  }
  return 1;
}

static void index_snapshot(const plan_t *p, int lbl, int64_t *first, int *count)
{
  for (int b = 0; b < p->nblk; b++) { first[b] = 0; count[b] = 0; }
  const cholamd_filled *v = p->snap[lbl];
  for (int64_t i = 0; i < p->snap_n[lbl]; i++) {
    int b = BIDX(p, v[i].sep_x, v[i].sep_y);
    if (count[b] == 0) first[b] = i;
    count[b]++;
  }
}

typedef struct { int64_t c_off; int ldc, m, n, syrk, src_begin, src_end, blk, ar0, br0; } upd_target;
typedef struct { chol_level_work *w; const chol_sched_opts *o; int force_fine; int cur_blk; const int *follow_lim;
  int dist_world, dist_rank; const struct cholamd_plan *dist_plan; int tgt_sep, tgt_col0; int cap_b;
  const int *sw_of;
  int cur_band; const int *bw_of;
  int cap_p, cap_t, cap_k, cap_km, cap_s, cap_ph; upd_target *pend; int n_pend, cap_pend; } builder;
static int env_int(const char *name, int dflt) { const char *e = getenv(name); return e && *e ? atoi(e) : dflt; }
void chol_sched_opts_default(chol_sched_opts *o)
{
  o->split_min = CHOL_SPLIT_MIN; o->split_nb = CHOL_SPLIT_NB; o->fuse = 1; o->fuse_update_max = CHOL_FUSE_UPDATE_MAX;
  o->mt_min_tiles = CHOL_MT_MIN_TILES; o->trsm_wt_min = CHOL_TRSM_WT_MIN; o->trsm_group = 0; o->cells = 1; o->program = 1; o->follow = 1; o->super_blocks = CHOL_SUPER_BLOCKS; o->dist_top = 2; o->follow_tail = CHOL_FOLLOW_TAIL; o->follow_tail_split = CHOL_FOLLOW_TAIL; o->staged = 1; o->fine_upd = 1; o->skyline = 1; o->stage_chunk = CHOL_STAGE_CHUNK; o->merge_targets = 1; o->leaf_envelope = 1;
}
void chol_sched_opts_from_env(chol_sched_opts *o)
{
  chol_sched_opts_default(o);
  o->split_min = env_int("CHOLAMD_SPLIT_MIN", o->split_min);
  o->split_nb = env_int("CHOLAMD_SPLIT_NB", o->split_nb);
  o->fuse = !env_int("CHOLAMD_NO_FUSE", 0);
  o->fuse_update_max = env_int("CHOLAMD_FUSE_UPDATE_MAX", o->fuse_update_max);
  o->mt_min_tiles = env_int("CHOLAMD_MT_MIN_TILES", o->mt_min_tiles);
  o->trsm_wt_min = env_int("CHOLAMD_TRSM_WT_MIN", o->trsm_wt_min);
  o->cells = !env_int("CHOLAMD_NO_CELLS", 0);
  o->program = !env_int("CHOLAMD_NO_PROGRAM", 0);
  o->follow = !env_int("CHOLAMD_NO_FOLLOW", 0);
  o->dist_top = env_int("CHOLAMD_DIST_TOP", o->dist_top);
  o->super_blocks = env_int("CHOLAMD_SUPER_BLOCKS", o->super_blocks);
  o->follow_tail = env_int("CHOLAMD_FOLLOW_TAIL", o->follow_tail);
  o->follow_tail_split = env_int("CHOLAMD_FOLLOW_TAIL_SPLIT", o->follow_tail_split);
  o->staged = !env_int("CHOLAMD_NO_STAGED", 0);
  o->fine_upd = !env_int("CHOLAMD_NO_FINE_UPD", 0);
  o->skyline = !env_int("CHOLAMD_NO_SKYLINE", 0);
  o->merge_targets = !env_int("CHOLAMD_NO_MERGE_TARGETS", 0);
  o->leaf_envelope = !env_int("CHOLAMD_NO_LEAF_ENVELOPE", 0);
  o->stage_chunk = env_int("CHOLAMD_STAGE_CHUNK", o->stage_chunk);
}
static int split_nb(const chol_sched_opts *o) { int v = o->split_nb; if (v > CHOL_RR_MAXN) v = CHOL_RR_MAXN; v = (v + 15) / 16 * 16; if (v < 16) v = 16; return v; }
static int pivot_blocks(const chol_sched_opts *o, int n) { return n > o->split_min || n > CHOL_RR_MAXN ? (n + split_nb(o) - 1) / split_nb(o) : 1; }
static int pivot_block_width(const chol_sched_opts *o, int n) { const int nb = pivot_blocks(o, n); return nb == 1 ? n : ((n + nb - 1) / nb + 15) / 16 * 16; }


static void push_phase_f(builder *B, int kind, int first, int n, int force);
static void push_phase(builder *B, int kind, int first, int n) { push_phase_f(B, kind, first, n, 0); }
static void push_phase_f(builder *B, int kind, int first, int n, int force)
{
  if (n <= 0 && !force) return;
  if (n < 0) n = 0;
  chol_level_work *w = B->w;
  if (w->n_phase == B->cap_ph) { B->cap_ph = B->cap_ph ? 2 * B->cap_ph : 16; w->phase = realloc(w->phase, B->cap_ph * sizeof(chol_phase)); }
  chol_phase ph = { kind, first, n, 0, 0, 0, 0 };
  w->phase[w->n_phase++] = ph;
}
void chol_potrf_table(int n, const unsigned char *sky, unsigned char *out)
{
  int *mask = (int *)(out + CHOL_RR_TAB_MASK);
  unsigned short *ij = (unsigned short *)(out + CHOL_RR_TAB_IJ);
  unsigned char *km = out + CHOL_RR_TAB_KM;
  memset(out, 0, CHOL_RR_TAB_BYTES);
  for (int t = 0; t < CHOL_RR_SLOTS * CHOL_RR_NW; t++) ij[t] = 0xffff;
  const int T = (n + CHOL_NB - 1) / CHOL_NB, ntl = T * (T + 1) / 2, ntl2 = (T - 2) * (T - 1) / 2;
  for (int t = 2 * T - 1; t < ntl; t++) {
    int ti, tj, ow, os;
    chol_rr_tile_of_index(t, T, &ti, &tj);
    chol_rr_owner(ntl - 1 - t, ntl2, &ow, &os);
    ij[os * CHOL_RR_NW + ow] = (unsigned short)(ti | (tj << 8));
    const int si = sky[ti < 23 ? ti : 23], sj = sky[tj < 23 ? tj : 23], kmin = si > sj ? si : sj;
    km[os * CHOL_RR_NW + ow] = (unsigned char)(kmin | (tj < si ? CHOL_RR_KM_ZERO : 0));
    const int last = ti == tj ? tj - 2 : tj - 1;
    for (int k = kmin < last ? kmin : last; k <= last; k++) mask[k * CHOL_RR_NW + ow] |= 1 << os;
  }
  for (int k = 0; k < T; k++)
    for (int i = k + 2; i < T; i++)
      if (sky[i < 23 ? i : 23] <= k) {
        const int hv = i % CHOL_RR_NHEAVY;
        mask[k * CHOL_RR_NW + hv + hv / 3] |= 1 << (i < k + 2 + CHOL_RR_NHEAVY ? CHOL_RR_M_SOLVE0 : CHOL_RR_M_SOLVE1);
      }
}
static void push_potrf(builder *B, chol_potrf_desc d)
{
  chol_level_work *w = B->w;
  if (w->n_potrf == B->cap_p) { B->cap_p = B->cap_p ? 2 * B->cap_p : 32; w->potrf = realloc(w->potrf, B->cap_p * sizeof(chol_potrf_desc)); }
  w->potrf[w->n_potrf++] = d;
}
static void push_trsm_run(builder *B, int64_t l_off, int64_t dinv_off, int64_t b_off, int n, int ld, int m, int flag)
{
  chol_level_work *w = B->w;
  for (int r0 = 0; r0 < m; r0 += CHOL_TRSM_ROWS) {
    if (w->n_trsm == B->cap_t) { B->cap_t = B->cap_t ? 2 * B->cap_t : 64; w->trsm = realloc(w->trsm, B->cap_t * sizeof(chol_trsm_desc)); }
    const int mm = m - r0 < CHOL_TRSM_ROWS ? m - r0 : CHOL_TRSM_ROWS;
    chol_trsm_desc td = { l_off, dinv_off, b_off + r0, n, ld, mm, ld, flag, -1, B->cur_band, 0 };
    w->trsm[w->n_trsm++] = td;
  }
}
static void pad_trsm_group(builder *B, int phase_first, int group, int64_t l_off, int64_t dinv_off, int64_t b_off, int n, int ld, int flag)
{
  chol_level_work *w = B->w;
  while ((w->n_trsm - phase_first) % group != 0) {
    if (w->n_trsm == B->cap_t) { B->cap_t = B->cap_t ? 2 * B->cap_t : 64; w->trsm = realloc(w->trsm, B->cap_t * sizeof(chol_trsm_desc)); }
    chol_trsm_desc td = { l_off, dinv_off, b_off, n, ld, 0, ld, flag, -1, B->cur_band, 0 };
    w->trsm[w->n_trsm++] = td;
  }
}
static int push_src(builder *B, chol_upd_src sd)
{
  chol_level_work *w = B->w;
  if (w->n_src == B->cap_s) { B->cap_s = B->cap_s ? 2 * B->cap_s : 256; w->src = realloc(w->src, B->cap_s * sizeof(chol_upd_src)); }
  w->src[w->n_src] = sd;
  return w->n_src++;
}
#ifndef MT_ORDER
#define MT_ORDER 8
#endif
static void emit_tasks(builder *B, int macro, int64_t c_off, int ldc, int m, int n, int syrk, int src_begin, int src_end, int blk, int ar0, int br0)
{
  chol_level_work *w = B->w;
  const int ts = macro ? 64 : 16;
  const int tr = (m + ts - 1) / ts, tc = (n + ts - 1) / ts;
  const int blk_o = macro ? MT_ORDER : (tr > tc ? tr : tc) + 1;
// ... 482 lines not shown
            const int fb_ = rows_first(rfirst[s_], (int)((tu[q].b_off - p->panel_off[s_]) % tu[q].ldb), G[a].n, tu[q].k);
            int k0_ = (fa_ > fb_ ? fa_ : fb_) & ~15;
            if (k0_ > ((tu[q].k - 1) & ~15)) k0_ = (tu[q].k - 1) & ~15;
            if (k0_ > 0) { sd.a_off += (int64_t)k0_ * sd.lda; sd.b_off += (int64_t)k0_ * sd.ldb; sd.k -= k0_; }
          }
          push_src(B, sd);
        }
        if (dist) { B->tgt_sep = p->blk[G[a].bc].c; B->tgt_col0 = G[a].ccol; }
        push_tasks(B, G[a].c_off, G[a].ldc, G[a].m, G[a].n, G[a].syrk, sb, w->n_src);
      }
      free(G);
    }
    flush_targets(B);
    if (dist) push_phase(B, 2, k0, w->n_task - k0); else
    if (fused_last >= 0 && fused_last == w->n_phase - 1 && w->phase[fused_last].n3 == 0 && w->n_task - k0 <= opts->fuse_update_max) {
      w->phase[fused_last].first3 = k0;
      w->phase[fused_last].n3 = w->n_task - k0;
    } else push_phase(B, 2, k0, w->n_task - k0);
    push_phase(B, 3, km0, w->n_task_mt - km0);
  }
  if (rfirst) { for (int s = 1; s <= p->nsep; s++) free(rfirst[s]); free(rfirst); }
  free(tu); free(first); free(count); free(hs); free(B->pend); B->pend = NULL; B->cap_pend = 0;
  return 0;
}


#ifndef PROG_JOB_TASKS
#define PROG_JOB_TASKS 12
#endif
#ifndef PROG_HEAVY_STEPS
#define PROG_HEAVY_STEPS 48
#endif
#define PROG_MAX_TASKS 24000
typedef struct { int potrf, c_prog, c_strips, n_groups, c0, nb, emitted; int ch_below, ns_below; int ch_par, ns_par; int64_t par_off;
  int ch_rest, ns_rest;
} pblock;
typedef struct { chol_program *pg; int cap_j, cap_w, cap_e, cap_c;
  int *c_updp, *cnt_updp;
} pbuild;
static int new_ctr(pbuild *P, int total)
{
  chol_program *g = P->pg;
  if (g->n_ctr == P->cap_c) { P->cap_c = P->cap_c ? 2 * P->cap_c : 256; g->ctr_total = realloc(g->ctr_total, P->cap_c * sizeof(int)); }
  g->ctr_total[g->n_ctr] = total;
  return g->n_ctr++;
}
static void add_wait(pbuild *P, int ctr, int value)
{
  chol_program *g = P->pg;
  if (value <= 0) return;
  if (g->n_wait == P->cap_w) { P->cap_w = P->cap_w ? 2 * P->cap_w : 1024; g->wait = realloc(g->wait, P->cap_w * sizeof(chol_wait)); }
  chol_wait wt = { ctr, value };
  g->wait[g->n_wait++] = wt;
}
static int add_ext(pbuild *P, chol_ext e)
{
  chol_program *g = P->pg;
  if (g->n_ext == P->cap_e) { P->cap_e = P->cap_e ? 2 * P->cap_e : 64; g->ext = realloc(g->ext, P->cap_e * sizeof(chol_ext)); }
  g->ext[g->n_ext] = e;
  return g->n_ext++;
}
typedef struct { chol_ext x; int key, seq; } ext_item;
static int cmp_ext_item(const void *a, const void *b)
{
  const ext_item *x = a, *y = b;
  if (x->key != y->key) return x->key < y->key ? -1 : 1;
  return x->seq < y->seq ? -1 : (x->seq > y->seq);
}
static void push_ext_items(ext_item **items, int *n, int *cap, int64_t off, int ld, int k, int chan, int nstrip, int key0, int e_from)
{
  for (int e = e_from; e * CHOL_NB < k; e++) {
    if (*n == *cap) { *cap = *cap ? 2 * *cap : 64; *items = realloc(*items, *cap * sizeof(ext_item)); }
    ext_item *it = &(*items)[(*n)];
    it->x.off = off + (int64_t)e * CHOL_NB * ld; it->x.ld = ld; it->x.ncol = k - e * CHOL_NB < CHOL_NB ? k - e * CHOL_NB : CHOL_NB;
    it->x.ctr = chan + e; it->x.need = nstrip;
    it->key = key0 + e; it->seq = *n;
    (*n)++;
  }
}
static chol_job *add_job(pbuild *P, int kind, int first, int n, int wait_first)
{
  chol_program *g = P->pg;
  if (g->n_job == P->cap_j) { P->cap_j = P->cap_j ? 2 * P->cap_j : 1024; g->job = realloc(g->job, P->cap_j * sizeof(chol_job)); }
  chol_job j = { kind, first, n, wait_first, g->n_wait - wait_first, { -1, -1 }, 0, g->n_ext, 0, 0, g->n_wait - wait_first };
  g->job[g->n_job] = j;
  return &g->job[g->n_job++];
}
void chol_program_free(chol_program *g)
{
  free(g->job); free(g->wait); free(g->ext); free(g->ctr_total);
  memset(g, 0, sizeof *g);
}
static int push_block_rows(builder *B, const plan_t *p, int anc, int s, int lo, int hi, const cholamd_filled *snap, const int64_t *first, const int *count,
                           int64_t diag, int64_t dinv, int nb, int ld, int64_t colbase, int flag, int chan)
{
  chol_level_work *w = B->w;
  const int b = BIDX(p, anc, s);
  const chol_block *Bk = &p->blk[b];
  const int t_before = w->n_trsm;
  int run_lo = -1, run_hi = -1;
  for (int q = 0; q <= count[b]; q++) {
    int a0 = -1, a1 = -1;
    if (q < count[b]) {
      const cholamd_filled *f = &snap[first[b] + q];
      a0 = f->lo_x - Bk->lo_x; a1 = f->hi_x - Bk->lo_x + 1;
      if (a0 < lo) a0 = lo;
      if (a1 > hi) a1 = hi;
      if (a0 >= a1) continue;
      if (run_hi == a0) { run_hi = a1; continue; }
    }
    if (run_lo >= 0) {
      push_trsm_run(B, diag, dinv, chol_block_row(Bk, run_lo) + colbase, nb, ld, run_hi - run_lo, flag);
    }
    run_lo = a0; run_hi = a1;
  }
  for (int i = t_before; i < w->n_trsm; i++) w->trsm[i].chan = chan;
  return w->n_trsm - t_before;
}
static int emit_trsm_jobs(pbuild *P, builder *B, int t0, int c_upd, int need_upd, int c_strips,
                          int ch_par, int c_updp, int need_updp, int ch_below, int c_updd, int need_updd)
{
  chol_level_work *w = B->w;
  int njobs = 0;
  for (int i = t0; i < w->n_trsm;) {
    int e = i + 1;
    while (e < w->n_trsm && e - i < 3 && w->trsm[e].chan == w->trsm[i].chan) e++;
    const int wf = P->pg->n_wait;
    const int ch = w->trsm[i].chan;
    if (ch >= 0 && ch == ch_par && c_updp >= 0) add_wait(P, c_updp, need_updp);
    else if (ch >= 0 && ch == ch_below && ch_par >= -1 && c_updp >= 0) add_wait(P, c_updd, need_updd);
    else add_wait(P, c_upd, need_upd);
    chol_job *j = add_job(P, 1, i, e - i, wf);
    j->sig[0] = c_strips; j->sig_add = 1;
    njobs++;
    i = e;
  }
  return njobs;
}
static void emit_update_jobs(pbuild *P, builder *B, const plan_t *p, int k0, const int *c_upd, const int *c_updd, const int *snap_upd, int *cnt_upd, int *cnt_updd,
                             const int *src_ctr, const int *src_need, int n_src_ctr, const int *stage_sep )
{
  chol_level_work *w = B->w;
  for (int i = k0; i < w->n_task;) {
#define TASK_STEPS(T_) ({ int st_ = 0; for (int q_ = w->task[T_].src_begin; q_ < w->task[T_].src_end; q_++) st_ += (w->src[q_].k + 3) / 4; st_; })
    const int heavy = TASK_STEPS(i) >= PROG_HEAVY_STEPS;
    const int lim = heavy ? 3 : PROG_JOB_TASKS;
    int e = i + 1;
    while (e < w->n_task && e - i < lim && w->task[e].blk == w->task[i].blk && (TASK_STEPS(e) >= PROG_HEAVY_STEPS) == heavy) e++;
#undef TASK_STEPS
    const chol_block *Bc = &p->blk[w->task[i].blk];
    const int wf = P->pg->n_wait;
    if (stage_sep) add_wait(P, c_upd[Bc->c], snap_upd[Bc->c]);
    const int n_pre = P->pg->n_wait - wf;
    for (int q = 0; q < n_src_ctr; q++) add_wait(P, src_ctr[q], src_need[q]);
    if (!stage_sep) add_wait(P, c_upd[Bc->c], snap_upd[Bc->c]);
    chol_job *j = add_job(P, 2, i, e - i, wf);
    j->mode = heavy;
    if (stage_sep) {
      j->n_pre = n_pre;
      for (int t = i; t < e; t++) {
        chol_upd_task *tk = &w->task[t];
        for (int q = tk->src_begin; q < tk->src_end; q++) {
          if (w->src[q].stage > 0) continue;
          int st = n_src_ctr;
          if (w->src[q].stage < 0) {
            const int tag = -w->src[q].stage - 1;
            for (int z = n_src_ctr - 1; z >= 0; z--) if (stage_sep[z] / 64 == tag / 64 && stage_sep[z] % 64 <= tag % 64) { st = z + 1; break; }
// ... 45 lines not shown
    sky[s] = malloc(T);
    for (int i = 0; i < T; i++) {
      int f = n;
      for (int r = i * CHOL_NB; r < n && r < (i + 1) * CHOL_NB; r++) if (first[s][r] < f) f = first[s][r];
      sky[s][i] = (unsigned char)(f / CHOL_NB);
    }
    free(first[s]);
  }
  free(first);
  return sky;
}
static void free_skylines(unsigned char **sky, int ns) { if (!sky) return; for (int s = 1; s <= ns; s++) free(sky[s]); free(sky); }
static int **leaf_row_first(const plan_t *p)
{
  const int ns = p->nsep, L = p->levels;
  int **first = calloc(ns + 1, sizeof(int *));
  for (int h = 1 << (L - 1); h <= ns; h++) {
    const int s = p->tree[h], n = p->sep_size[s], ld = p->panel_ld[s];
    if (n <= 0) continue;
    first[s] = malloc((size_t)ld * sizeof(int));
    for (int r = 0; r < ld; r++) first[s][r] = r < n ? r : n;
  }
  for (int64_t e = 0; e < p->nnz_a; e++) {
    const int64_t off = p->a_dst[e];
    int lo = 1, hi = ns;
    while (lo < hi) { const int mid = (lo + hi + 1) / 2; if (p->panel_off[mid] <= off) lo = mid; else hi = mid - 1; }
    const int s = lo;
    if (!first[s]) continue;
    const int64_t rel = off - p->panel_off[s];
    const int ld = p->panel_ld[s], row = (int)(rel % ld), col = (int)(rel / ld);
    if (col < first[s][row]) first[s][row] = col;
  }
  return first;
}

typedef struct { int64_t off; int ld, k, ctr, need; } early_src;
#ifndef EARLY_CHUNK
#define EARLY_CHUNK 2
#endif
static void emit_early_cells(pbuild *P, builder *B, const plan_t *p, int64_t c_off, int ldc, int lim, int blk, const early_src *es, int nes,
                             const int *c_upd, const int *c_updd, int *snap_upd, int *cnt_upd, int *cnt_updd)
{
  chol_level_work *w = B->w;
  int nst = 0, maxch = 0;
  for (int q = 0; q < nes; q++) if (es[q].k > 0) { const int ch = ((es[q].k + CHOL_NB - 1) / CHOL_NB + EARLY_CHUNK - 1) / EARLY_CHUNK; nst += ch; if (ch > maxch) maxch = ch; }
  if (nst == 0) return;
  int *sc = malloc(nst * sizeof(int)), *sn = malloc(nst * sizeof(int)), *sq = malloc(nst * sizeof(int)), *sch = malloc(nst * sizeof(int));
  nst = 0;
  for (int c = 0; c < maxch; c++)
    for (int q = 0; q < nes; q++) {
      if (es[q].k <= 0) continue;
      const int et = (es[q].k + CHOL_NB - 1) / CHOL_NB;
      if (c * EARLY_CHUNK >= et) continue;
      const int last = (c + 1) * EARLY_CHUNK < et ? (c + 1) * EARLY_CHUNK - 1 : et - 1;
      sc[nst] = es[q].ctr - (et - 1) + last; sn[nst] = es[q].need; sq[nst] = q; sch[nst] = c; nst++;
    }
  const int staged = B->o->staged;
  const int k0 = w->n_task, Tl = (lim + CHOL_NB - 1) / CHOL_NB;
  for (int I = 0; I < Tl; I++)
    for (int J = 0; J <= I; J++) {
      const int sb = w->n_src;
      for (int z = 0; z < nst; z++) {
        const early_src *e = &es[sq[z]];
        const int col0 = sch[z] * EARLY_CHUNK * CHOL_NB, kc = e->k - col0 < EARLY_CHUNK * CHOL_NB ? e->k - col0 : EARLY_CHUNK * CHOL_NB;
        chol_upd_src sd = { e->off + CHOL_NB * I + (int64_t)col0 * e->ld, e->off + CHOL_NB * J + (int64_t)col0 * e->ld, e->ld, e->ld, kc, 0, staged ? z + 1 : 0, 0 };
        push_src(B, sd);
      }
      if (w->n_task == B->cap_k) { B->cap_k = B->cap_k ? 2 * B->cap_k : 256; w->task = realloc(w->task, B->cap_k * sizeof(chol_upd_task)); }
      chol_upd_task *t = &w->task[w->n_task++];
      memset(t, 0, sizeof *t);
      t->c_off = c_off + CHOL_NB * I + (int64_t)(CHOL_NB * J) * ldc; t->ldc = ldc;
      t->mv = (short)(lim - CHOL_NB * I < CHOL_NB ? lim - CHOL_NB * I : CHOL_NB);
      t->nv = (short)(lim - CHOL_NB * J < CHOL_NB ? lim - CHOL_NB * J : CHOL_NB);
      t->lower = I == J;
      t->src_begin = sb; t->src_end = w->n_src;
      t->blk = blk;
    }
  const int col_sep = p->blk[blk].c;
  snap_upd[col_sep] = cnt_upd[col_sep];
  emit_update_jobs(P, B, p, k0, c_upd, c_updd, snap_upd, cnt_upd, cnt_updd, sc, sn, nst, staged ? sq : NULL);
  free(sc); free(sn); free(sq); free(sch);
}

static chol_sched_opts chol_program_opts(const chol_sched_opts *o)
{
  chol_sched_opts r = *o;
  if (r.split_min == CHOL_SPLIT_MIN && r.split_nb == CHOL_SPLIT_NB) r.split_min = CHOL_PROG_SPLIT_MIN;
  return r;
}
int chol_build_program(const plan_t *p, const chol_sched_opts *opts, chol_level_work *w, chol_program *pg)
{
  memset(w, 0, sizeof *w);
  memset(pg, 0, sizeof *pg);
  w->level = -1;
  chol_sched_opts dflt, prog;
  if (!opts) { chol_sched_opts_default(&dflt); opts = &dflt; }
  prog = chol_program_opts(opts); opts = &prog;
  builder Bd; memset(&Bd, 0, sizeof Bd); Bd.w = w; Bd.o = opts; Bd.force_fine = 1;
  builder *B = &Bd;
  pbuild Pd; memset(&Pd, 0, sizeof Pd); Pd.pg = pg;
  pbuild *P = &Pd;
  const int L = p->levels, ns = p->nsep;
  int rc = 0;
  unsigned char **sky = opts->skyline ? leaf_skylines(p) : calloc(ns + 1, sizeof(unsigned char *));
  int *bw_of = malloc((ns + 1) * sizeof(int)), *band_of = calloc(ns + 1, sizeof(int));
  for (int s = 1; s <= ns; s++) {
    const int n = p->sep_size[s];
    bw_of[s] = pivot_block_width(opts, n);
    if (sky[s] && n > CHOL_FUSE_MAXN && n <= CHOL_RR_MAXN && pivot_blocks(opts, n) > 1) {
      int band = 1;
      for (int i = 0; i * CHOL_NB < n; i++) if (i - sky[s][i] > band) band = i - sky[s][i];
      if (band <= 4) { bw_of[s] = n; band_of[s] = band; }
    }
  }
  B->bw_of = bw_of;
  int *sw_of = malloc((ns + 1) * sizeof(int));
  for (int s = 1; s <= ns; s++) {
    sw_of[s] = bw_of[s];
    if (band_of[s] && opts->staged && opts->stage_chunk > 0 && opts->stage_chunk * CHOL_NB < p->sep_size[s]) sw_of[s] = opts->stage_chunk * CHOL_NB;
  }
  B->sw_of = sw_of;
  for (int s = 1; s <= ns && !rc; s++) {
    const int bw = bw_of[s];
    if ((bw > CHOL_FUSE_MAXN && !band_of[s]) || bw > CHOL_RR_MAXN) { chol_set_error("program launch: pivot block of %d columns (separator %d) exceeds %d", bw, s, CHOL_FUSE_MAXN); rc = CHOLAMD_ERR_ARG; }
  }
  {
    double est = 0;
    for (int s = 1; s <= ns; s++) {
      const int n = p->sep_size[s], rows = p->panel_rows[s];
      if (n <= 0) continue;
      const int bw = bw_of[s], nbk = (n + bw - 1) / bw;
      for (int st = 0; st + 1 < nbk; st++) est += (double)((rows - (st + 1) * bw) / 16 + 1) * ((n - (st + 1) * bw) / 16 + 1);
      est += (double)(rows / 16 + 1) * (n / 16 + 1) * (L - 1 - p->level_of[s]);
    }
    if (est > 2.0 * PROG_MAX_TASKS) { chol_set_error("program launch: about %.0f update tasks", est); rc = CHOLAMD_ERR_ARG; }
  }
  if (rc) { free_skylines(sky, ns); free(bw_of); free(band_of); free(sw_of); return rc; }
  const int follow = opts->follow && opts->cells;
  pg->follow = follow;
  int64_t *first = malloc(p->nblk * sizeof(int64_t));
  int *count = malloc(p->nblk * sizeof(int));
  int *c_upd = malloc((ns + 1) * sizeof(int)), *c_updd = malloc((ns + 1) * sizeof(int));
  if (opts->fine_upd && opts->follow && opts->cells) { P->c_updp = malloc((ns + 1) * sizeof(int)); P->cnt_updp = calloc(ns + 1, sizeof(int)); }
  int *cnt_upd = calloc(ns + 1, sizeof(int)), *cnt_updd = calloc(ns + 1, sizeof(int)), *snap_upd = calloc(ns + 1, sizeof(int));
  int *nblk_of = calloc(ns + 1, sizeof(int));
  pblock **pb = calloc(ns + 1, sizeof(pblock *));
  int *follow_lim = calloc(p->nblk, sizeof(int));
  for (int s = 1; s <= ns; s++) {
    c_upd[s] = new_ctr(P, 0); c_updd[s] = new_ctr(P, 0);
    if (P->c_updp) P->c_updp[s] = new_ctr(P, 0);
    const int n = p->sep_size[s];
    const int bw = bw_of[s], nbk = n > 0 ? (n + bw - 1) / bw : 0;
    nblk_of[s] = nbk;
    pb[s] = calloc(nbk > 0 ? nbk : 1, sizeof(pblock));
    for (int st = 0; st < nbk; st++) {
      pblock *b = &pb[s][st];
      b->c0 = st * bw; b->nb = n - b->c0 < bw ? n - b->c0 : bw;
      b->potrf = -1; b->ch_below = b->ch_par = b->ch_rest = -1;
      b->c_prog = new_ctr(P, (b->nb + CHOL_NB - 1) / CHOL_NB);
      b->c_strips = new_ctr(P, 0);
    }
  }
  int *est_start = calloc(ns + 1, sizeof(int));
  for (int h = ns; h >= 1; h--) {
    int st0 = 0;
    for (int c = 2 * h; c <= 2 * h + 1 && c <= ns; c++) {
// ... 324 lines not shown
      if (!rc) {
        if (tuples_are_small(opts, tu, ntu) || any_follow) { B->follow_lim = follow_lim; emit_cell_tasks(B, p, tu, ntu); B->follow_lim = NULL; }
        else {
          for (int i = 0; i < ntu;) {
            int e = i + 1;
            while (e < ntu && tu[e].key == tu[i].key) e++;
            const int sb = w->n_src;
            for (int q = i; q < e; q++) { chol_upd_src sd = { tu[q].a_off, tu[q].b_off, tu[q].lda, tu[q].ldb, tu[q].k, 0, -(64 * tu[q].src_sep + 63) - 1, 0 }; push_src(B, sd); }
            B->cur_blk = tu[i].bc;
            push_tasks(B, tu[i].c_off, tu[i].ldc, tu[i].m, tu[i].n, tu[i].syrk, sb, w->n_src);
            i = e;
          }
          flush_targets(B);
        }
        typedef struct { int i, e, prio; } blk_range;
        int nrg = 0, caprg = 64;
        blk_range *rg = malloc(caprg * sizeof(blk_range));
        for (int i = k0; i < w->n_task;) {
          int e = i + 1;
          while (e < w->n_task && w->task[e].blk == w->task[i].blk) e++;
          const chol_block *Bc = &p->blk[w->task[i].blk];
          if (nrg == caprg) { caprg *= 2; rg = realloc(rg, caprg * sizeof(blk_range)); }
          rg[nrg].i = i; rg[nrg].e = e;
          rg[nrg].prio = (L - p->level_of[Bc->c]) * 4 * L + (Bc->r == Bc->c ? 0 : 1 + (p->level_of[Bc->c] - p->level_of[Bc->r]));
          nrg++;
          i = e;
        }
        for (int a = 1; a < nrg; a++) {
          blk_range t = rg[a];
          int b = a - 1;
          while (b >= 0 && rg[b].prio > t.prio) { rg[b + 1] = rg[b]; b--; }
          rg[b + 1] = t;
        }
        for (int q = 0; q < nrg; q++) {
          const int i = rg[q].i, e = rg[q].e;
          const chol_block *Bc = &p->blk[w->task[i].blk];
          const int hpar = p->heap_of[Bc->c], dl = level - p->level_of[Bc->c];
          int nsc = 0, capsc = 1;
          for (int hh = hpar << dl; hh < ((hpar + 1) << dl); hh++) capsc += nblk_of[p->tree[hh]] + 2 * ((p->sep_size[p->tree[hh]] + CHOL_NB - 1) / CHOL_NB);
          int *sc = malloc(capsc * sizeof(int)), *sn = malloc(capsc * sizeof(int)), *ssep = malloc(capsc * sizeof(int)), *sest = malloc(capsc * sizeof(int));
          for (int hh = hpar << dl; hh < ((hpar + 1) << dl); hh++) {
            const int s = p->tree[hh];
            int through = 0;
            for (int st = 0; st < nblk_of[s]; st++) {
              const pblock *b = &pb[s][st];
              if (sw_of[s] < bw_of[s] && b->n_groups > 0) {
                const int nt = (b->nb + CHOL_NB - 1) / CHOL_NB, ct = sw_of[s] / CHOL_NB;
                for (int c = 0; c * ct < nt; c++) {
                  const int last = (c + 1) * ct < nt ? (c + 1) * ct - 1 : nt - 1;
                  if (b->ch_par >= 0) { sc[nsc] = b->ch_par + last; sn[nsc] = b->ns_par; ssep[nsc] = 64 * s + c; sest[nsc] = est_start[s] + last + 1; nsc++; }
                  if (b->ch_rest >= 0) { sc[nsc] = b->ch_rest + last; sn[nsc] = b->ns_rest; ssep[nsc] = 64 * s + c; sest[nsc] = est_start[s] + last + 1; nsc++; }
                }
                through += nt;
                continue;
              }
              through += (b->nb + CHOL_NB - 1) / CHOL_NB;
              if (b->n_groups > 0) { sc[nsc] = b->c_strips; sn[nsc] = b->n_groups; ssep[nsc] = 64 * s + st; sest[nsc] = est_start[s] + through; nsc++; }
            }
          }
          for (int a = 1; a < nsc; a++) {
            const int c0_ = sc[a], n0_ = sn[a], s0_ = ssep[a], e0_ = sest[a];
            int b = a - 1;
            while (b >= 0 && sest[b] > e0_) { sc[b + 1] = sc[b]; sn[b + 1] = sn[b]; ssep[b + 1] = ssep[b]; sest[b + 1] = sest[b]; b--; }
            sc[b + 1] = c0_; sn[b + 1] = n0_; ssep[b + 1] = s0_; sest[b + 1] = e0_;
          }
          const int keep = w->n_task;
          w->n_task = e;
          emit_update_jobs(P, B, p, i, c_upd, c_updd, snap_upd, cnt_upd, cnt_updd, sc, sn, nsc, opts->staged ? ssep : NULL);
          w->n_task = keep;
          free(ssep); free(sest);
          free(sc); free(sn);
        }
        free(rg);
      }
      free(tu);
    }
    free(hs);
    if (w->n_task > PROG_MAX_TASKS && !rc) { chol_set_error("program launch: more than %d update tasks", PROG_MAX_TASKS); rc = CHOLAMD_ERR_ARG; }
  }
  #undef EMIT_POTRF
  if (!rc && w->n_task_mt > 0) { chol_set_error("program launch: macro-tile update phases"); rc = CHOLAMD_ERR_ARG; }
  if (!rc && w->n_task > PROG_MAX_TASKS) { chol_set_error("program launch: %d update tasks", w->n_task); rc = CHOLAMD_ERR_ARG; }
  for (int s = 1; s <= ns; s++) { pg->ctr_total[c_upd[s]] = cnt_upd[s]; pg->ctr_total[c_updd[s]] = cnt_updd[s]; if (P->c_updp) pg->ctr_total[P->c_updp[s]] = P->cnt_updp[s]; }
  free(P->c_updp); free(P->cnt_updp); P->c_updp = P->cnt_updp = NULL;
  for (int s = 1; s <= ns; s++) free(pb[s]);
  free_skylines(sky, ns); free(bw_of); free(band_of); free(sw_of);
  free(est_start); free(pb); free(nblk_of); free(first); free(count); free(c_upd); free(c_updd); free(cnt_upd); free(cnt_updd); free(snap_upd); free(follow_lim);
  free(B->pend);
  if (rc) { chol_level_work_free(w); chol_program_free(pg); }
  return rc;
}


typedef struct { int64_t a, b, c, d; } quad;
static int cmp_quad(const void *x, const void *y) { return memcmp(x, y, sizeof(quad)); }
int chol_program_check(const plan_t *p, const chol_sched_opts *opts, int workers)
{
  chol_level_work w;
  chol_program g;
  int rc = chol_build_program(p, opts, &w, &g);
  if (rc) return rc;
  rc = chol_program_check_built(p, opts, workers, &w, &g);
  chol_level_work_free(&w);
  chol_program_free(&g);
  return rc;
}
int chol_program_check_built(const plan_t *p, const chol_sched_opts *opts, int workers, const chol_level_work *wp, const chol_program *gp)
{
  const chol_level_work w = *wp;
  const chol_program g = *gp;
  int rc = 0;
  int *val = calloc(g.n_ctr > 0 ? g.n_ctr : 1, sizeof(int));
  char *state = calloc(g.n_job > 0 ? g.n_job : 1, 1);
  int next = 0, running = 0, done = 0;
  while (done < g.n_job && !rc) {
    while (running < workers && next < g.n_job) { state[next++] = 1; running++; }
    int progressed = 0;
    for (int j = 0; j < next; j++) {
      if (state[j] != 1) continue;
      const chol_job *jb = &g.job[j];
      int ok = 1;
      for (int q = 0; q < jb->n_wait && ok; q++) {
        const chol_wait *wt = &g.wait[jb->wait_first + q];
        if (wt->ctr < 0 || wt->ctr >= g.n_ctr || wt->value > g.ctr_total[wt->ctr]) { chol_set_error("program job %d waits for %d on counter %d (total %d)", j, wt->value, wt->ctr, wt->ctr >= 0 && wt->ctr < g.n_ctr ? g.ctr_total[wt->ctr] : -1); rc = CHOLAMD_ERR_ARG; ok = 0; break; }
        if (val[wt->ctr] < wt->value) ok = 0;
      }
      if (rc) break;
      if (ok && jb->kind == 0)
        for (int x = 0; x < jb->n_ext && ok; x++) {
          const chol_ext *e = &g.ext[jb->ext_first + x];
          if (val[e->ctr] < e->need) ok = 0;
        }
      if (ok && jb->kind == 1 && val[w.trsm[jb->first].flag] < g.ctr_total[w.trsm[jb->first].flag]) ok = 0;
      if (!ok) continue;
      if (jb->kind == 0) val[w.potrf[jb->first].ctr] = g.ctr_total[w.potrf[jb->first].ctr];
      if (jb->kind == 1)
        for (int i = jb->first; i < jb->first + jb->n; i++)
          if (w.trsm[i].chan >= 0 && w.trsm[i].m > 0)
            for (int t = 0; t < (w.trsm[i].n + CHOL_NB - 1) / CHOL_NB; t++) val[w.trsm[i].chan + t]++;
      for (int q = 0; q < 2; q++) if (jb->sig[q] >= 0) val[jb->sig[q]] += jb->sig_add;
      state[j] = 2; running--; done++; progressed = 1;
    }
    if (!rc && !progressed && (running == workers || next == g.n_job)) {
      int j = 0;
      while (j < next && state[j] != 1) j++;
      chol_set_error("program dead-locks with %d resident workgroups: job %d (kind %d) can never run; %d of %d jobs done", workers, j, j < g.n_job ? g.job[j].kind : -1, done, g.n_job);
      rc = CHOLAMD_ERR_ARG;
    }
  }
  for (int c = 0; c < g.n_ctr && !rc; c++)
    if (val[c] != g.ctr_total[c]) { chol_set_error("program counter %d ends at %d, total %d", c, val[c], g.ctr_total[c]); rc = CHOLAMD_ERR_ARG; }
  free(val); free(state);
  if (!rc) {
    quad *a = NULL, *b = NULL;
    int64_t na = 0, nb = 0, ca = 0, cb = 0;
#define PUSHQ(V_, N_, C_, A_, B_, C2_, D_) do { if (N_ == C_) { C_ = C_ ? 2 * C_ : 4096; V_ = realloc(V_, C_ * sizeof(quad)); } quad q_ = { A_, B_, C2_, D_ }; V_[N_++] = q_; } while (0)
    for (int l = 0; l < p->levels && !rc; l++) {
      chol_level_work lw;
      chol_sched_opts lo = *opts; lo.leaf_envelope = 0;
      rc = chol_build_level_work(p, &lo, l, 0, 1, &lw);
      if (rc) break;
      for (int i = 0; i < lw.n_potrf; i++) for (int ct = 0; ct * CHOL_NB < lw.potrf[i].n; ct++) for (int r = ct * CHOL_NB; r < lw.potrf[i].n; r++) PUSHQ(a, na, ca, -1, lw.potrf[i].a_off + r + (int64_t)ct * CHOL_NB * lw.potrf[i].lda, 0, 0);
      for (int i = 0; i < lw.n_trsm; i++) for (int r = 0; r < lw.trsm[i].m; r++) for (int ct = 0; ct * CHOL_NB < lw.trsm[i].n; ct++) PUSHQ(a, na, ca, -1, lw.trsm[i].b_off + r + (int64_t)ct * CHOL_NB * lw.trsm[i].ldb, 0, 0);
      chol_level_work_free(&lw);
    }
    for (int i = 0; i < w.n_potrf; i++) for (int ct = 0; ct * CHOL_NB < w.potrf[i].n; ct++) for (int r = ct * CHOL_NB; r < w.potrf[i].n; r++) PUSHQ(b, nb, cb, -1, w.potrf[i].a_off + r + (int64_t)ct * CHOL_NB * w.potrf[i].lda, 0, 0);
    for (int i = 0; i < w.n_trsm; i++) for (int r = 0; r < w.trsm[i].m; r++) for (int ct = 0; ct * CHOL_NB < w.trsm[i].n; ct++) PUSHQ(b, nb, cb, -1, w.trsm[i].b_off + r + (int64_t)ct * CHOL_NB * w.trsm[i].ldb, 0, 0);
#undef PUSHQ
    if (!rc) {
      qsort(a, na, sizeof(quad), cmp_quad);
      qsort(b, nb, sizeof(quad), cmp_quad);
      if (na != nb || (na > 0 && memcmp(a, b, na * sizeof(quad)))) { chol_set_error("program pivot blocks / TRSM rows differ from the level lists (%lld vs %lld items)", (long long)nb, (long long)na); rc = CHOLAMD_ERR_ARG; }
    }
    free(a); free(b);
  }
  return rc;
}
int cholamd_plan_program_check(const cholamd_plan *p, int follow, int workers)
{
  chol_sched_opts o;
  chol_sched_opts_default(&o);
  o.follow = follow;
  return chol_program_check(p, &o, workers);
}
int cholamd_plan_program_check_opts(const cholamd_plan *p, int follow_tail, int split_min, int split_nb, int workers)
{
  chol_sched_opts o;
  chol_sched_opts_from_env(&o);
  if (follow_tail >= 0) o.follow_tail = follow_tail;
  if (split_min >= 0) o.split_min = split_min;
  if (split_nb >= 0) o.split_nb = split_nb;
  return chol_program_check(p, &o, workers);
}
int64_t cholamd_plan_program_jobs(const cholamd_plan *p, int follow, int64_t cap, int *out)
{
  chol_sched_opts o;
  chol_sched_opts_default(&o);
  o.follow = follow;
  chol_level_work w; chol_program g;
  if (chol_build_program(p, &o, &w, &g)) return -1;
  const int64_t need = (int64_t)8 * g.n_job + (int64_t)3 * g.n_wait + 1;
  if (cap >= need) {
    int64_t k = 0;
    for (int j = 0; j < g.n_job; j++) {
      const chol_job *jb = &g.job[j];
      int a = 0, b = 0;
      if (jb->kind == 0) { a = w.potrf[jb->first].sep; b = w.potrf[jb->first].col0; }
      else if (jb->kind == 1) { for (int i = 0; i < w.n_potrf; i++) if (w.potrf[i].ctr == w.trsm[jb->first].flag) { a = w.potrf[i].sep; b = w.potrf[i].col0; } }
      else { a = p->blk[w.task[jb->first].blk].c; b = p->blk[w.task[jb->first].blk].r; }
      out[k++] = jb->kind; out[k++] = a; out[k++] = b; out[k++] = jb->first; out[k++] = jb->n; out[k++] = jb->sig[0]; out[k++] = jb->kind == 1 ? w.trsm[jb->first].chan : jb->sig[1]; out[k++] = jb->n_wait;
    }
    for (int j = 0; j < g.n_job; j++)
      for (int q = 0; q < g.job[j].n_wait; q++) { out[k++] = j; out[k++] = g.wait[g.job[j].wait_first + q].ctr; out[k++] = g.wait[g.job[j].wait_first + q].value; }
    out[k++] = g.n_job;
  }
  chol_level_work_free(&w); chol_program_free(&g);
  return need;
}
int cholamd_follow_rounds(int n_ext, int tile_columns, int cap, int *rounds_out, int *own_at_out)
{
  int n = 0;
  for (int i = 0; i < n_ext; i += chol_follow_round(i, n_ext, tile_columns), n++)
    if (n < cap && rounds_out) rounds_out[n] = chol_follow_round(i, n_ext, tile_columns);
  if (own_at_out) *own_at_out = chol_follow_own_at(n_ext, tile_columns);
  return n;
}
int64_t cholamd_plan_program_followers(const cholamd_plan *p, int64_t cap, int *out)
{
  chol_sched_opts o;
  chol_sched_opts_default(&o);
  chol_level_work w; chol_program g;
  if (chol_build_program(p, &o, &w, &g)) return -1;
  int64_t n = 0;
  for (int j = 0; j < g.n_job; j++) {
    const chol_job *jb = &g.job[j];
    if (jb->kind != 0 || jb->n_ext <= 0) continue;
    if (4 * n + 3 < cap) { out[4 * n] = j; out[4 * n + 1] = jb->n_ext; out[4 * n + 2] = (w.potrf[jb->first].n + CHOL_NB - 1) / CHOL_NB; out[4 * n + 3] = jb->n_wait; }
    n++;
  }
  chol_level_work_free(&w); chol_program_free(&g);
  return n;
}
int cholamd_plan_program_counts(const cholamd_plan *p, int follow, int out[6])
{
  chol_sched_opts o;
  chol_sched_opts_default(&o);
  o.follow = follow;
  chol_level_work w; chol_program g;
  int rc = chol_build_program(p, &o, &w, &g);
  if (rc) return rc;
  int nf = 0;
  for (int j = 0; j < g.n_job; j++) nf += g.job[j].kind == 0 && g.job[j].n_ext > 0;
  out[0] = g.n_job; out[1] = nf; out[2] = w.n_task; out[3] = w.n_trsm; out[4] = g.n_ctr; out[5] = g.n_ext;
  chol_level_work_free(&w); chol_program_free(&g);
  return 0;
}

static int level_work_volume(const cholamd_plan *p, const chol_sched_opts *o, int level, int rank, int world, int64_t out[6], int64_t counts[3])
{
  chol_level_work w;
  int rc = chol_build_level_work(p, o, level, rank, world, &w);
  if (rc) return rc;
  memset(out, 0, 6 * sizeof(int64_t));
  if (counts) { counts[0] = w.n_task; counts[1] = w.n_task_mt; counts[2] = 0; for (int i = 0; i < w.n_trsm; i++) counts[2] += w.trsm[i].m > 0; }
  for (int i = 0; i < w.n_potrf; i++) out[0] += w.potrf[i].n;
  for (int i = 0; i < w.n_trsm; i++) out[1] += (int64_t)w.trsm[i].m * w.trsm[i].n;
  for (int pass = 0; pass < 2; pass++) {
    const chol_upd_task *T = pass ? w.task_mt : w.task;
    const int nt = pass ? w.n_task_mt : w.n_task;
    for (int i = 0; i < nt; i++) {
      const chol_upd_task *t = &T[i];
      int64_t full = 0;
      for (int c = 0; c < t->nv; c++) full += t->lower ? (t->mv - c > 0 ? t->mv - c : 0) : t->mv;
      for (int q = t->src_begin; q < t->src_end; q++) {
        const chol_upd_src *sd = &w.src[q];
        const int r0 = sd->range & 255, r1 = (sd->range >> 8) & 255, c0 = (sd->range >> 16) & 255, c1 = (sd->range >> 24) & 255;
        out[2] += (sd->range ? (int64_t)(r1 - r0) * (c1 - c0) : full) * sd->k;
      }
    }
  }
  out[3] = w.n_bcast;
// ... 513 lines not shown
```

### cholesky_amd/device.py

```python
import ctypes as C

import numpy as np

from ._lib import check, load

_check = check

HALF_FORWARD, HALF_BACKWARD = 0, 1


def _stream_ptr(stream):
    if stream is None:
        return None
    if hasattr(stream, "cuda_stream"):
        return C.c_void_p(stream.cuda_stream)
    return C.c_void_p(int(stream))


class RankArena:

    def __init__(self, dev, ptr, elem_bytes, backed_bytes):
        self.dev, self._ptr, self.elem_bytes, self.backed_bytes = dev, ptr, elem_bytes, backed_bytes
        self.nbytes = dev.plan.arena_doubles * elem_bytes

# ... 34 lines not shown
                self.L.cholamd_device_destroy(self.h)
                self.h = None
        except Exception:
            pass

    def alloc(self, doubles):
        p = C.c_void_p()
        check(self.L.cholamd_device_alloc(self.h, int(doubles), C.byref(p)), "cholamd_device_alloc")
        self._owned.append(p)
        return p.value

    def new_arena(self):
        import torch
        return torch.empty(self.plan.arena_doubles, dtype=torch.float64, device=f"cuda:{self.device_id}")

    def alloc_arena(self, elem_bytes=8):
        p, backed = C.c_void_p(), C.c_int64(0)
        check(self.L.cholamd_device_alloc_arena(self.h, int(elem_bytes), C.byref(p), C.byref(backed)), "cholamd_device_alloc_arena")
        return RankArena(self, p.value, int(elem_bytes), backed.value)

    @staticmethod
    def ptr(t):
        return C.c_void_p(t if isinstance(t, int) else t.data_ptr())

    def upload(self, dptr, host, stream=None):
        host = np.ascontiguousarray(host, dtype=np.float64)
        check(self.L.cholamd_device_upload(self.h, self.ptr(dptr), host.ctypes.data, host.size, _stream_ptr(stream)), "upload")

    def download(self, dptr, doubles, stream=None):
        out = np.empty(int(doubles), dtype=np.float64)
        check(self.L.cholamd_device_download(self.h, out.ctypes.data, self.ptr(dptr), out.size, _stream_ptr(stream)), "download")
        return out

    def sync(self, stream=None):
        check(self.L.cholamd_device_sync(self.h, _stream_ptr(stream)), "sync")

    def fill(self, arena, stream=None):
        check(self.L.cholamd_device_fill(self.h, self.ptr(arena), _stream_ptr(stream)), "cholamd_device_fill")

    VALUES_NOCHECK = 1
    HALF_FORWARD, HALF_BACKWARD = 0, 1

    def set_values(self, values, check=True, stream=None):
        import torch
        nz = self.plan.nz
        if isinstance(values, np.ndarray):
            if values.dtype != np.float64 or values.ndim != 1 or values.size != nz or not values.flags.c_contiguous:
                raise ValueError(f"values must be a contiguous 1-D float64 array of plan.nz = {nz} elements; got {values.dtype} {values.shape}")
            if self._values_buf is None:
                self._values_buf = torch.empty(max(nz, 1), dtype=torch.float64, device=f"cuda:{self.device_id}")
            self.upload(self._values_buf, values, stream)
            ptr = self._values_buf.data_ptr()
        elif isinstance(values, torch.Tensor):
            if values.dtype != torch.float64 or values.dim() != 1 or values.numel() != nz or not values.is_contiguous():
                raise ValueError(f"values must be a contiguous 1-D float64 tensor of plan.nz = {nz} elements; got {values.dtype} {tuple(values.shape)} strides {values.stride()}")
            if not values.is_cuda or values.device.index != self.device_id:
                raise ValueError(f"values must live on cuda:{self.device_id}; got {values.device}")
            ptr = values.data_ptr()
        else:
            raise ValueError("values must be a float64 numpy array or CUDA tensor")
        _check(self.L.cholamd_device_set_values(self.h, C.c_void_p(ptr), nz, 0 if check else self.VALUES_NOCHECK, _stream_ptr(stream)),
               "cholamd_device_set_values")

    def values_status(self, stream=None):
        out = np.zeros(4, dtype=np.int64)
        _check(self.L.cholamd_device_values_status(self.h, _stream_ptr(stream), out.ctypes.data), "cholamd_device_values_status")
        return tuple(int(v) for v in out)

    def factor(self, arena, stream=None):
        check(self.L.cholamd_factor(self.h, self.ptr(arena), _stream_ptr(stream)), "cholamd_factor")

    def factor_levels(self, arena, level_hi, level_lo, stream=None):
        check(self.L.cholamd_factor_levels(self.h, self.ptr(arena), level_hi, level_lo, _stream_ptr(stream)), "cholamd_factor_levels")

    def set_partition(self, rank, world):
        check(self.L.cholamd_device_set_partition(self.h, rank, world), "cholamd_device_set_partition")

    def dist_top_active(self):
        return self.L.cholamd_device_bcast_phases(self.h) > 0

    def set_option(self, name, value):
        check(self.L.cholamd_device_set_option(self.h, name.encode(), int(value)), "cholamd_device_set_option")

    def program_trace(self, arena, stream=None):
        n = C.c_int(0)
        check(self.L.cholamd_device_program_trace(self.h, self.ptr(arena), _stream_ptr(stream), 0, None, C.byref(n)), "cholamd_device_program_trace")
        out = np.zeros((n.value, 5), dtype=np.int64)
        check(self.L.cholamd_device_program_trace(self.h, self.ptr(arena), _stream_ptr(stream), out.size, out.ctypes.data, C.byref(n)), "cholamd_device_program_trace")
        return out

    def tail_offset(self):
        return int(self.L.cholamd_device_tail_offset(self.h))

    def exchange_tail(self, arena, comm, stream=None):
        check(self.L.cholamd_exchange_tail(self.h, self.ptr(arena), comm.h, _stream_ptr(stream)), "cholamd_exchange_tail")

    def factor_sharded(self, arena, comm, stream=None):
        check(self.L.cholamd_factor_sharded(self.h, self.ptr(arena), comm.h if comm is not None else None, _stream_ptr(stream)), "cholamd_factor_sharded")

    def factor_sharded_f32(self, arena32, comm, stream=None):
        check(self.L.cholamd_factor_sharded_f32(self.h, self.ptr(arena32), comm.h if comm is not None else None, _stream_ptr(stream)), "cholamd_factor_sharded_f32")

    def gather_to_root(self, arena, comm, stream=None):
        check(self.L.cholamd_gather_to_root(self.h, self.ptr(arena), int(arena.element_size()), comm.h, _stream_ptr(stream)), "cholamd_gather_to_root")

    def exchange_volume(self):
        out = np.zeros(4, dtype=np.int64)
        check(self.L.cholamd_exchange_volume(self.h, out.ctypes.data), "cholamd_exchange_volume")
        return tuple(int(v) for v in out)

    def info(self):
        sep = C.c_int(0)
        rc = self.L.cholamd_factor_info(self.h, C.byref(sep))
        if rc < 0:
            check(rc, "cholamd_factor_info")
        return rc, sep.value

    def solve(self, arena, b, x, stream=None):
        check(self.L.cholamd_solve(self.h, self.ptr(arena), self.ptr(b), self.ptr(x), _stream_ptr(stream)), "cholamd_solve")

    def new_arena_f32(self):
        import torch
        return torch.empty(self.plan.arena_doubles, dtype=torch.float32, device=f"cuda:{self.device_id}")

    def fill_f32(self, arena32, stream=None):
        check(self.L.cholamd_device_fill_f32(self.h, self.ptr(arena32), _stream_ptr(stream)), "cholamd_device_fill_f32")

    def factor_f32(self, arena32, stream=None):
        check(self.L.cholamd_factor_f32(self.h, self.ptr(arena32), _stream_ptr(stream)), "cholamd_factor_f32")

    def factor_levels_f32(self, arena32, level_hi, level_lo, stream=None):
        check(self.L.cholamd_factor_levels_f32(self.h, self.ptr(arena32), level_hi, level_lo, _stream_ptr(stream)), "cholamd_factor_levels_f32")

    def solve_f32(self, arena32, b, x, stream=None):
        check(self.L.cholamd_solve_f32(self.h, self.ptr(arena32), self.ptr(b), self.ptr(x), _stream_ptr(stream)), "cholamd_solve_f32")

    def solve_refine(self, arena32, b, x, max_iter=20, tol=1e-12, stream=None):
        it, rel = C.c_int(0), C.c_double(0.0)
        check(self.L.cholamd_solve_refine(self.h, self.ptr(arena32), self.ptr(b), self.ptr(x), int(max_iter), float(tol),
                                          C.byref(it), C.byref(rel), _stream_ptr(stream)), "cholamd_solve_refine")
        return it.value, rel.value

    def solve_sharded(self, arena, b, x, comm, stream=None):
        import torch
        f32 = arena.elem_bytes == 4 if isinstance(arena, RankArena) else arena.dtype == torch.float32
        fn = self.L.cholamd_solve_sharded_f32 if f32 else self.L.cholamd_solve_sharded
        check(fn(self.h, self.ptr(arena), self.ptr(b), self.ptr(x), comm.h if comm is not None else None, _stream_ptr(stream)), "cholamd_solve_sharded")

    def solve_refine_sharded(self, arena32, b, x, comm, max_iter=20, tol=1e-12, stream=None):
        it, rel = C.c_int(0), C.c_double(0.0)
        check(self.L.cholamd_solve_refine_sharded(self.h, self.ptr(arena32), self.ptr(b), self.ptr(x), max_iter, tol, C.byref(it), C.byref(rel),
                                                  comm.h if comm is not None else None, _stream_ptr(stream)), "cholamd_solve_refine_sharded")
        return int(it.value), float(rel.value)

    @staticmethod
    def _block(t, what, n):
        import torch
        if not isinstance(t, torch.Tensor) or t.dim() != 2 or not t.is_cuda or t.dtype != torch.float64:
            raise ValueError(f"{what} must be a 2-D CUDA float64 tensor, e.g. torch.empty(k, n).T")
        if t.shape[0] != n:
            raise ValueError(f"{what} has {t.shape[0]} rows, the system has n = {n}")
        if t.shape[1] > 0 and t.stride(0) != 1:
            raise ValueError(f"{what} must be column-major (stride(0) == 1), e.g. torch.empty(k, n).T; got strides {t.stride()}")
        if t.shape[1] > 1 and t.stride(1) < n:
            raise ValueError(f"{what} has column stride {t.stride(1)} < n = {n}: its columns overlap")
        return (int(t.stride(1)) if t.shape[1] > 1 else n), int(t.shape[1])

    def _blocks(self, B, X):
        ldb, k = self._block(B, "B", self.plan.n)
        ldx, kx = self._block(X, "X", self.plan.n)
        if kx != k:
# ... 189 lines not shown
```

### cholesky_amd/plan.py

```python
import ctypes as C
import os

import numpy as np

from ._lib import Filled, Op, check, load

OP_NAMES = ("POTRF", "TRSM", "SYRK", "GEMM")


class Plan:
    def __init__(self, matrix_file=None, separator_file=None, clusters_file=None, _handle=None):
        self.L = load()
        if _handle is not None:
            self.h = _handle
        else:
            h = C.c_void_p()
            check(self.L.cholamd_plan_create(os.fsencode(matrix_file), os.fsencode(separator_file), os.fsencode(clusters_file), C.byref(h)),
                  "cholamd_plan_create")
            self.h = h
        g = self.L
        self.n = g.cholamd_plan_n(self.h)
        self.nz = g.cholamd_plan_nz(self.h)
        self.levels = g.cholamd_plan_levels(self.h)
        self.nsep = g.cholamd_plan_num_separators(self.h)
# ... 130 lines not shown
        return tuple(int(v) for v in out)

    def exchange_volume(self, rank, world, dist_top=2):
        out = np.zeros(4, dtype=np.int64)
        check(self.L.cholamd_plan_exchange_volume(self.h, rank, world, dist_top, out.ctypes.data), "cholamd_plan_exchange_volume")
        return tuple(int(v) for v in out)

    def solve_counts(self, level, rank=0, world=1):
        out = np.zeros(5, dtype=np.int64)
        check(self.L.cholamd_plan_solve_counts(self.h, level, rank, world, out.ctypes.data), "cholamd_plan_solve_counts")
        return tuple(int(v) for v in out)

    def solve_skips(self, level):
        cnt = self.solve_counts(level)
        seps = np.zeros((max(cnt[0], 1), 3), dtype=np.int32)
        runs = np.zeros((max(cnt[1], 1), 5), dtype=np.int32)
        check(self.L.cholamd_plan_solve_skips(self.h, level, seps.ctypes.data, runs.ctypes.data), "cholamd_plan_solve_skips")
        return seps[:cnt[0]], runs[:cnt[1]]

    def diag_list(self):
        m = self.nsep
        a_off = np.zeros(m, dtype=np.int64)
        cols, lda, x_off, sep = (np.zeros(m, dtype=np.int32) for _ in range(4))
        prefix = np.zeros(m + 1, dtype=np.int32)
        n = self.L.cholamd_plan_diag_list(self.h, a_off.ctypes.data, cols.ctypes.data, lda.ctypes.data, x_off.ctypes.data, sep.ctypes.data, prefix.ctypes.data)
        if n < 0:
            check(n, "cholamd_plan_diag_list")
        return a_off[:n], cols[:n], lda[:n], x_off[:n], sep[:n], prefix[:n + 1]

    SELINV_BLOCK = 64
    SELINV_FRONT_MAX = 8192

    def selinv_blocks(self, sep):
        n = self.L.cholamd_plan_selinv_blocks(self.h, int(sep))
        if n < 0:
            check(n, "cholamd_plan_selinv_blocks")
        return n

    def selinv_front(self, sep, block):
        cols = np.zeros(2, dtype=np.int32)
        m = self.L.cholamd_plan_selinv_front(self.h, int(sep), int(block), 0, cols.ctypes.data, None, None)
        if m < 0:
            check(m, "cholamd_plan_selinv_front")
        pos = np.zeros(max(m, 1), dtype=np.int32)
        off = np.zeros((max(m, 1), max(m, 1)), dtype=np.int64)
        m2 = self.L.cholamd_plan_selinv_front(self.h, int(sep), int(block), m, cols.ctypes.data, pos.ctypes.data, off.ctypes.data)
        if m2 < 0:
            check(m2, "cholamd_plan_selinv_front")
        return int(cols[0]), int(cols[1]), pos[:m], off[:m, :m]

    def exchange_pieces(self, world, dist_top=2):
        out = np.zeros((4096, 4), dtype=np.int64)
        n = self.L.cholamd_plan_exchange_pieces(self.h, world, dist_top, len(out), out.ctypes.data)
        if n < 0:
            check(n, "cholamd_plan_exchange_pieces")
        return out[:min(n, len(out))]

    def level_work_volume(self, level, rank=0, world=1, dist_top=2):
        out = np.zeros(6, dtype=np.int64)
        check(self.L.cholamd_plan_level_work_volume(self.h, level, rank, world, dist_top, out.ctypes.data), "cholamd_plan_level_work_volume")
        return tuple(int(v) for v in out)

    def level_work_volume_opts(self, level, merge_targets=1, mt_min_tiles=-1):
        out = np.zeros(9, dtype=np.int64)
        check(self.L.cholamd_plan_level_work_volume_opts(self.h, level, int(merge_targets), int(mt_min_tiles), out.ctypes.data), "cholamd_plan_level_work_volume_opts")
        return tuple(int(v) for v in out)

    def level_mt_fill(self, level):
        out = np.zeros(4, dtype=np.int64)
        check(self.L.cholamd_plan_level_mt_fill(self.h, level, out.ctypes.data), "cholamd_plan_level_mt_fill")
        return tuple(int(v) for v in out)

    def program_check(self, follow=True, workers=64):
        check(self.L.cholamd_plan_program_check(self.h, int(follow), int(workers)), "cholamd_plan_program_check")

    def program_check_opts(self, follow_tail=-1, split_min=-1, split_nb=-1, workers=64):
        check(self.L.cholamd_plan_program_check_opts(self.h, follow_tail, split_min, split_nb, int(workers)), "cholamd_plan_program_check_opts")

    def program_counts(self, follow=True):
        out = np.zeros(6, dtype=np.int32)
        check(self.L.cholamd_plan_program_counts(self.h, int(follow), out.ctypes.data), "cholamd_plan_program_counts")
        return dict(zip(("jobs", "followers", "tasks", "strips", "counters", "followed_panels"), (int(v) for v in out)))

    def program_jobs(self, follow=True):
        need = self.L.cholamd_plan_program_jobs(self.h, int(follow), 0, None)
        buf = np.zeros(need, dtype=np.int32)
        self.L.cholamd_plan_program_jobs(self.h, int(follow), need, buf.ctypes.data)
        nj = int(buf[-1])
        return buf[:8 * nj].reshape(nj, 8), buf[8 * nj:-1].reshape(-1, 3)

    def arena_to_dense(self, arena):
        arena = np.ascontiguousarray(arena, dtype=np.float64)
        assert arena.size == self.arena_doubles
        d = np.zeros((self.n, self.n), dtype=np.float64, order="F")
        check(self.L.cholamd_plan_arena_to_dense(self.h, arena.ctypes.data, d.ctypes.data), "cholamd_plan_arena_to_dense")
        return d

    def write_matrix(self, arena, path, full_precision=False):
        arena = np.ascontiguousarray(arena, dtype=np.float64)
        check(self.L.cholamd_plan_write_matrix(self.h, arena.ctypes.data, os.fsencode(path), int(full_precision)), "cholamd_plan_write_matrix")

    def write_debug_log(self, path):
        libc = C.CDLL(None)
        libc.fopen.restype = C.c_void_p
        libc.fopen.argtypes = [C.c_char_p, C.c_char_p]
        libc.fclose.argtypes = [C.c_void_p]
        fp = libc.fopen(os.fsencode(path), b"w")
        if not fp:
            raise IOError(path)
        try:
            check(self.L.cholamd_plan_write_debug_log(self.h, fp), "cholamd_plan_write_debug_log")
        finally:
            libc.fclose(fp)


def read_vector(path, n):
    out = np.zeros(n, dtype=np.float64)
    check(load().cholamd_read_vector(os.fsencode(path), n, out.ctypes.data), "cholamd_read_vector")
    return out


def write_solution(path, x, full_precision=False):
    x = np.ascontiguousarray(x, dtype=np.float64)
    check(load().cholamd_write_solution(os.fsencode(path), x.ctypes.data, x.size, int(full_precision)), "cholamd_write_solution")


class Problem:

    def __init__(self, nx, ny=1, nz=1, levels=3, tile=32):
        self.L = load()
        h = C.c_void_p()
        check(self.L.cholamd_generate_laplacian(nx, ny, nz, levels, tile, C.byref(h)), "cholamd_generate_laplacian")
        self.h = h
        self.n = self.L.cholamd_problem_n(h)
        self.nz = self.L.cholamd_problem_nz(h)
        self.levels = levels

    def __del__(self):
        try:
            if getattr(self, "h", None):
                self.L.cholamd_problem_destroy(self.h)
                self.h = None
        except Exception:
            pass

    def write(self, prefix):
        check(self.L.cholamd_problem_write(self.h, os.fsencode(prefix)), "cholamd_problem_write")
        lv = self.levels
        return f"{prefix}.mtx", f"{prefix}_ord_{lv}.txt", f"{prefix}_clust_{lv}.txt", f"{prefix}_B.mtx"

    def plan(self):
        h = C.c_void_p()
        check(self.L.cholamd_plan_create_from_problem(self.h, C.byref(h)), "cholamd_plan_create_from_problem")
        return Plan(_handle=h)

    def rhs(self):
        b = np.zeros(self.n, dtype=np.float64)
        self.L.cholamd_problem_rhs(self.h, b.ctypes.data)
        return b
```

### include/cholamd.h

```cpp
#ifndef CHOLAMD_H
#define CHOLAMD_H

#include <stdint.h>
#include <stdio.h>

#ifdef __cplusplus
extern "C" {
#endif

#define CHOLAMD_OK 0
#define CHOLAMD_ERR_IO (-1)
#define CHOLAMD_ERR_FORMAT (-2)
#define CHOLAMD_ERR_INVARIANT (-3)
#define CHOLAMD_ERR_ARG (-4)
#define CHOLAMD_ERR_NO_DEVICE (-5)
#define CHOLAMD_ERR_HIP (-6)
#define CHOLAMD_ERR_NOMEM (-7)
#define CHOLAMD_ERR_COMM (-9)
#define CHOLAMD_ERR_STALL (-8)

const char *cholamd_last_error(void);
const char *cholamd_version(void);

typedef char MM_typecode[4];
// ... 13 lines not shown

typedef struct cholamd_sepinfo { int levels; int num_separators; } cholamd_sepinfo;

int cholamd_read_separators(const char *file, int dim, int *idx_out, int *sep_out, cholamd_sepinfo *info);

int cholamd_read_clusters(const char *file, int *idx_out, int *interval_out, int *sep_out, int64_t cap, int64_t *count_out);

int cholamd_read_matrix(const char *file, int nz, int *row_out, int *col_out, double *val_out);

int cholamd_read_vector(const char *file, int n, double *out);

typedef struct cholamd_plan cholamd_plan;

typedef struct cholamd_filled {
  int filled;
  int sep_x, sep_y;
  int interval;
  int cluster;
  int lo_x, lo_y, hi_x, hi_y;
} cholamd_filled;

typedef struct cholamd_op {
  int op;
  int level;
  int m, n, k;
  int a_sx, a_sy, a_z;
  int b_sx, b_sy, b_z;
  int c_sx, c_sy, c_z;
} cholamd_op;

int cholamd_plan_create(const char *matrix_file, const char *separator_file, const char *clusters_file, cholamd_plan **out);
int cholamd_plan_create_from_arrays(int n, int levels, const int *perm, const int *sep_sizes,
                                    const int *cl_idx, const int *cl_interval, const int *cl_sep, int64_t cl_count,
                                    int64_t nz, const int *a_row, const int *a_col, const double *a_val,
                                    const char *banner, cholamd_plan **out);
void cholamd_plan_destroy(cholamd_plan *p);

int cholamd_plan_n(const cholamd_plan *p);
int cholamd_plan_nz(const cholamd_plan *p);
int cholamd_plan_levels(const cholamd_plan *p);
int cholamd_plan_num_separators(const cholamd_plan *p);
int cholamd_plan_max_int_size(const cholamd_plan *p);
int cholamd_plan_num_blocks(const cholamd_plan *p);
int64_t cholamd_plan_arena_doubles(const cholamd_plan *p);
int64_t cholamd_plan_arena_dense_doubles(const cholamd_plan *p);
int cholamd_plan_block_tile_map(const cholamd_plan *p, int r, int c, int *out);
int64_t cholamd_plan_dropped_entries(const cholamd_plan *p);
const char *cholamd_plan_banner(const cholamd_plan *p);
void cholamd_plan_perm(const cholamd_plan *p, int *out);
void cholamd_plan_sep_sizes(const cholamd_plan *p, int *out);
void cholamd_plan_sep_offsets(const cholamd_plan *p, int *out);
void cholamd_plan_tree(const cholamd_plan *p, int *out);
void cholamd_plan_blocks(const cholamd_plan *p, int *out);
int64_t cholamd_plan_snapshot_count(const cholamd_plan *p, int interval_lbl);
void cholamd_plan_snapshot(const cholamd_plan *p, int interval_lbl, cholamd_filled *out);
int64_t cholamd_plan_num_ops(const cholamd_plan *p);
void cholamd_plan_ops(const cholamd_plan *p, cholamd_op *out);
void cholamd_plan_counts(const cholamd_plan *p, int level , int64_t calls[4], double flops[4]);
double cholamd_plan_flops(const cholamd_plan *p);
int64_t cholamd_plan_nnz_a(const cholamd_plan *p);
int64_t cholamd_plan_nnz_l(const cholamd_plan *p);
int64_t cholamd_plan_nnz_tiles(const cholamd_plan *p);
double cholamd_plan_fmin(const cholamd_plan *p);
int64_t cholamd_plan_alg_bytes(const cholamd_plan *p);

int cholamd_plan_fill_host(const cholamd_plan *p, double *arena);
int cholamd_plan_entries(const cholamd_plan *p, int *row, int *col);
int cholamd_plan_value_map(const cholamd_plan *p, int64_t *src_out);
int cholamd_plan_fill_host_values(const cholamd_plan *p, const double *vals, int64_t count, double *arena);
int cholamd_plan_diag_list(const cholamd_plan *p, int64_t *a_off, int *cols, int *lda, int *x_off, int *sep, int *prefix);
int cholamd_plan_fill_host_part(const cholamd_plan *p, double *arena, int rank, int world, int64_t *tail_offset_out);
int cholamd_plan_level_work_counts(const cholamd_plan *p, int level, int rank, int world, int out[4]);
int cholamd_plan_level_work_volume_opts(const cholamd_plan *p, int level, int merge_targets, int mt_min_tiles, int64_t out[9]);
int cholamd_plan_level_mt_fill(const cholamd_plan *p, int level, int64_t out[4]);
int cholamd_plan_level_work_volume(const cholamd_plan *p, int level, int rank, int world, int dist_top, int64_t out[6]);
int cholamd_plan_exchange_volume(const cholamd_plan *p, int rank, int world, int dist_top, int64_t out[4]);
int cholamd_plan_exchange_pieces(const cholamd_plan *p, int world, int dist_top, int max, int64_t (*out)[4]);
int cholamd_plan_program_check(const cholamd_plan *p, int follow, int workers);
int cholamd_plan_program_check_opts(const cholamd_plan *p, int follow_tail, int split_min, int split_nb, int workers);
int cholamd_plan_program_counts(const cholamd_plan *p, int follow, int out[6]);
int cholamd_follow_rounds(int n_ext, int tile_columns, int cap, int *rounds_out, int *own_at_out);
int64_t cholamd_plan_program_followers(const cholamd_plan *p, int64_t cap, int *out);
int64_t cholamd_plan_program_jobs(const cholamd_plan *p, int follow, int64_t cap, int *out);
int cholamd_plan_arena_to_dense(const cholamd_plan *p, const double *arena, double *dense);
int cholamd_plan_write_matrix(const cholamd_plan *p, const double *arena, const char *file, int full_precision);
int cholamd_write_solution(const char *file, const double *x, int n, int full_precision);
int cholamd_plan_write_debug_log(const cholamd_plan *p, FILE *f);
int cholamd_plan_write_debug_header(const cholamd_plan *p, FILE *f);
int cholamd_plan_write_blocks_txt(const cholamd_plan *p, const double *arena, const char *file, const char *header);
int cholamd_plan_ntiles_at_level(const cholamd_plan *p, int sep, int level);

typedef struct cholamd_problem cholamd_problem;
int cholamd_generate_laplacian(int nx, int ny, int nz, int levels, int tile, cholamd_problem **out);
void cholamd_problem_destroy(cholamd_problem *g);
int cholamd_problem_n(const cholamd_problem *g);
int cholamd_problem_nz(const cholamd_problem *g);
int cholamd_problem_write(const cholamd_problem *g, const char *prefix);
int cholamd_plan_create_from_problem(const cholamd_problem *g, cholamd_plan **out);
void cholamd_problem_rhs(const cholamd_problem *g, double *b);

typedef struct cholamd_device cholamd_device;

int cholamd_device_count(void);
int cholamd_device_create(const cholamd_plan *plan, int device_id, cholamd_device **out);
void cholamd_device_destroy(cholamd_device *d);
int cholamd_device_alloc(cholamd_device *d, int64_t doubles, double **dptr);
int cholamd_device_free(cholamd_device *d, double *dptr);
int cholamd_device_upload(cholamd_device *d, double *d_dst, const double *h_src, int64_t doubles, void *stream);
int cholamd_device_download(cholamd_device *d, double *h_dst, const double *d_src, int64_t doubles, void *stream);
int cholamd_device_sync(cholamd_device *d, void *stream);
int cholamd_device_fill(cholamd_device *d, double *d_arena, void *stream);
#define CHOLAMD_VALUES_NOCHECK 1
int cholamd_device_set_values(cholamd_device *d, const double *d_vals, int64_t count, int flags, void *stream);
int cholamd_device_values_status(cholamd_device *d, void *stream, int64_t out[4]);
int cholamd_factor(cholamd_device *d, double *d_arena, void *stream);
int cholamd_factor_levels(cholamd_device *d, double *d_arena, int level_hi, int level_lo, void *stream);
int cholamd_device_set_partition(cholamd_device *d, int rank, int world);
int cholamd_device_program_trace(cholamd_device *d, double *d_arena, void *stream, int64_t cap, int64_t *out, int *njobs_out);
int cholamd_factor_debug(cholamd_device *d, double *d_arena, const char *dir, int full_precision, void *stream);
int cholamd_factor_info(cholamd_device *d, int *sep_out);
int cholamd_device_set_option(cholamd_device *d, const char *name, int value);
int cholamd_device_bcast_phases(const cholamd_device *d);
int cholamd_solve(cholamd_device *d, const double *d_arena, const double *d_b, double *d_x, void *stream);
int cholamd_device_fill_f32(cholamd_device *d, float *d_arena32, void *stream);
int cholamd_factor_f32(cholamd_device *d, float *d_arena32, void *stream);
int cholamd_factor_levels_f32(cholamd_device *d, float *d_arena32, int level_hi, int level_lo, void *stream);
int cholamd_solve_f32(cholamd_device *d, const float *d_arena32, const double *d_b, double *d_x, void *stream);
int cholamd_solve_refine(cholamd_device *d, const float *d_arena32, const double *d_b, double *d_x, int max_iter, double tol,
                         int *iters_out, double *relres_out, void *stream);
int cholamd_residual(cholamd_device *d, const double *d_b, const double *d_x, double *d_r, double *relres_out, void *stream);
int cholamd_solve_nrhs(cholamd_device *d, const double *d_arena, const double *d_B, int64_t ldb, double *d_X, int64_t ldx, int nrhs, void *stream);
int cholamd_solve_nrhs_f32(cholamd_device *d, const float *d_arena32, const double *d_B, int64_t ldb, double *d_X, int64_t ldx, int nrhs, void *stream);
int cholamd_solve_refine_nrhs(cholamd_device *d, const float *d_arena32, const double *d_B, int64_t ldb, double *d_X, int64_t ldx, int nrhs, int max_iter,
                              double tol, int *iters_out, double *relres_out , void *stream);
#define CHOLAMD_HALF_FORWARD  0
#define CHOLAMD_HALF_BACKWARD 1
int cholamd_solve_half(cholamd_device *d, const double *d_arena, const double *d_b, double *d_x, int which, void *stream);
int cholamd_solve_half_f32(cholamd_device *d, const float *d_arena32, const double *d_b, double *d_x, int which, void *stream);
int cholamd_solve_half_nrhs(cholamd_device *d, const double *d_arena, const double *d_B, int64_t ldb, double *d_X, int64_t ldx, int nrhs, int which, void *stream);
int cholamd_solve_half_nrhs_f32(cholamd_device *d, const float *d_arena32, const double *d_B, int64_t ldb, double *d_X, int64_t ldx, int nrhs, int which, void *stream);
int cholamd_factor_logdet(cholamd_device *d, const double *d_arena, double *logdet_out, void *stream);
int cholamd_factor_logdet_f32(cholamd_device *d, const float *d_arena32, double *logdet_out, void *stream);
int cholamd_factor_diag(cholamd_device *d, const double *d_arena, double *d_diag, void *stream);
int cholamd_factor_diag_f32(cholamd_device *d, const float *d_arena32, double *d_diag, void *stream);
#define CHOLAMD_SELINV_BLOCK 64
#define CHOLAMD_SELINV_FRONT_MAX 8192
int cholamd_selinv(cholamd_device *d, const double *d_arena, double *d_zarena, void *stream);
int cholamd_selinv_diag(cholamd_device *d, const double *d_zarena, double *d_diag, void *stream);
int cholamd_selinv_entries(cholamd_device *d, const double *d_zarena, double *d_vals, int64_t count, void *stream);
int cholamd_plan_selinv_blocks(const cholamd_plan *p, int sep);
int cholamd_plan_selinv_front(const cholamd_plan *p, int sep, int block, int cap, int cols[2], int *pos, int64_t *off);
int cholamd_device_set_timing(cholamd_device *d, int on);
int cholamd_device_get_timing(cholamd_device *d, float ms_by_kind[4], int launches_by_kind[4]);
int cholamd_device_get_timing_ex(cholamd_device *d, float ms_by_kind[8], int launches_by_kind[8]);
int cholamd_device_event_overhead(cholamd_device *d, void *stream, float *ms_out);

typedef struct cholamd_comm cholamd_comm;
#define CHOLAMD_UNIQUE_ID_BYTES 128
int cholamd_comm_unique_id(char id[CHOLAMD_UNIQUE_ID_BYTES]);
int cholamd_comm_create(cholamd_device *d, int world, int rank, const char id[CHOLAMD_UNIQUE_ID_BYTES], cholamd_comm **out);
int cholamd_comm_create_all(cholamd_device *const *devs, int n, cholamd_comm **out );
int cholamd_comm_create_local(cholamd_device *const *devs, int n, cholamd_comm **out );
int cholamd_comm_adopt(void *nccl_comm , int world, int rank, cholamd_comm **out);
int cholamd_comm_count(const cholamd_comm *c, int *ranks_out);
void cholamd_comm_destroy(cholamd_comm *c);
int cholamd_comm_allreduce(cholamd_comm *c, double *d_buf, int64_t count, void *stream);
int cholamd_device_alloc_arena(cholamd_device *d, int elem_bytes, void **dptr, int64_t *backed_bytes);
int cholamd_device_free_arena(cholamd_device *d, void *dptr);
int64_t cholamd_device_tail_offset(const cholamd_device *d);
int cholamd_exchange_tail(cholamd_device *d, double *d_arena, cholamd_comm *c, void *stream);
int cholamd_exchange_volume(const cholamd_device *d, int64_t out[4]);
int cholamd_factor_sharded(cholamd_device *d, double *d_arena, cholamd_comm *c, void *stream);
int cholamd_factor_sharded_f32(cholamd_device *d, float *d_arena32, cholamd_comm *c, void *stream);
int cholamd_gather_to_root(cholamd_device *d, void *d_arena, int elem_bytes, cholamd_comm *c, void *stream);
int cholamd_factor_multi(cholamd_device *const *devs, double *const *arenas, cholamd_comm *const *comms, int n, void *const *streams );
int cholamd_gather_factor(cholamd_device *const *devs, double *const *arenas, int n, void *const *streams );
int cholamd_factor_multi_f32(cholamd_device *const *devs, float *const *arenas32, cholamd_comm *const *comms, int n, void *const *streams );
int cholamd_gather_factor_f32(cholamd_device *const *devs, float *const *arenas32, int n, void *const *streams );
int cholamd_plan_solve_counts(const cholamd_plan *p, int level, int rank, int world, int64_t out[5]);
int cholamd_plan_solve_skips(const cholamd_plan *p, int level, int *seps, int *runs);
int cholamd_solve_sharded(cholamd_device *d, const double *d_arena, const double *d_b, double *d_x, cholamd_comm *c, void *stream);
int cholamd_solve_sharded_f32(cholamd_device *d, const float *d_arena32, const double *d_b, double *d_x, cholamd_comm *c, void *stream);
int cholamd_solve_refine_sharded(cholamd_device *d, const float *d_arena32, const double *d_b, double *d_x, int max_iter, double tol,
                                 int *iters_out, double *relres_out, cholamd_comm *c, void *stream);
int cholamd_solve_multi(cholamd_device *const *devs, const double *const *arenas, const double *const *bs, double *const *xs, cholamd_comm *const *comms,
                        int n, void *const *streams);
int cholamd_solve_refine_multi(cholamd_device *const *devs, const float *const *arenas32, const double *const *bs, double *const *xs, int max_iter, double tol,
                               int *iters_out, double *relres_out, cholamd_comm *const *comms, int n, void *const *streams);

typedef struct cholamd_region {
  double *ptr;
  int ld;
  int lo_x, lo_y, hi_x, hi_y;
  const int *tile_row;
} cholamd_region;
int cholamd_plan_region(const cholamd_plan *plan, double *d_arena, int r, int c, cholamd_region *out);

int cholamd_fused_dpotrf(const cholamd_region *rA, const cholamd_filled *filled_rA, int nA, int level, int interval, int debug, void *stream);
int cholamd_fused_dtrsm(const cholamd_region *rA, const cholamd_region *rB, const cholamd_filled *filled_rA, int nA,
                        const cholamd_filled *filled_rB, int nB, int level, int interval, int debug, void *stream);
int cholamd_fused_dsyrk(const cholamd_region *rA, const cholamd_region *rB, const cholamd_region *rC,
// ... 34 lines not shown
```

Measured before the change: 800.6 GF/s.

## Add optional XCD-affine per-queue job dispatch to persistent program kernel

Adds an optional scheme in which the persistent program kernel pulls jobs from several queues. Workgroups in bound 'drawers' take jobs from the queue matching their XCD slot (blockIdx & 7) and fall back to a shared last queue. Jobs are reordered by queue on upload, and a separate deadlock checker validates the queue layout, with a fallback to the single-queue program if the check fails. The aim is to keep related jobs on one XCD for L2 locality and to reduce contention on a single global head counter. The feature is off by default (xcd_queues=0), so the default path only changes how the grid size and head counter are set up.

```diff
diff --git a/cholesky_amd/_lib.py b/cholesky_amd/_lib.py
--- a/cholesky_amd/_lib.py
+++ b/cholesky_amd/_lib.py
@@ -94,6 +94,11 @@
     L.cholamd_plan_program_counts.argtypes = [vp, ci, vp]
     L.cholamd_plan_program_jobs.argtypes = [vp, ci, i64, vp]
     L.cholamd_plan_program_jobs.restype = i64
+    L.cholamd_plan_program_jobs_queues.argtypes = [vp, ci, ci, i64, vp]
+    L.cholamd_plan_program_jobs_queues.restype = i64
+    L.cholamd_plan_program_queues.argtypes = [vp, ci, ci, ci, ci, i64, vp]
+    L.cholamd_plan_program_queues.restype = i64
+    L.cholamd_plan_program_check_queues.argtypes = [vp, ci, ci, ci, ci]
     L.cholamd_plan_write_matrix.argtypes = [vp, vp, C.c_char_p, ci]
     L.cholamd_plan_write_debug_log.argtypes = [vp, vp]
     L.cholamd_device_create.argtypes = [vp, ci, C.POINTER(vp)]
@@ -139,6 +144,7 @@
     L.cholamd_factor.argtypes = [vp, vp, vp]
     L.cholamd_factor_levels.argtypes = [vp, vp, ci, ci, vp]
     L.cholamd_device_program_trace.argtypes = [vp, vp, vp, i64, vp, C.POINTER(ci)]
+    L.cholamd_device_program_trace_queues.argtypes = [vp, vp, vp, i64, vp, C.POINTER(ci)]
     L.cholamd_factor_info.argtypes = [vp, C.POINTER(ci)]
     L.cholamd_solve.argtypes = [vp, vp, vp, vp, vp]
     L.cholamd_device_fill_f32.argtypes = [vp, vp, vp]
diff --git a/cholesky_amd/csrc/chol_api.cpp b/cholesky_amd/csrc/chol_api.cpp
--- a/cholesky_amd/csrc/chol_api.cpp
+++ b/cholesky_amd/csrc/chol_api.cpp
@@ -88,6 +88,8 @@
   chol_job *jobs = nullptr; chol_wait *pwaits = nullptr; chol_ext *exts = nullptr;
   int *pctr = nullptr, *pctr_total = nullptr;
   int n_job = 0, n_pctr = 0, prog_grid = 0, prog_epoch = 0, prog_epoch_limit = 0;
+  chol_queues queues;
+  std::vector<int> job_of_slot;
   bool prog_ready = false;
   unsigned long long *trace = nullptr;
   std::vector<chol_job> jobs_host;
@@ -222,23 +224,40 @@
   if (d->world == 1 && d->opt.program) {
     chol_level_work w;
     chol_program g;
-    const bool built = chol_build_program(d->plan, &d->opt, &w, &g) == 0;
-    const bool live = built && chol_program_check_built(d->plan, &d->opt, 4, &w, &g) == 0;
+    int hipcus = 256;
+    hipDeviceProp_t prop;
+    if (hipGetDeviceProperties(&prop, d->dev) == hipSuccess && prop.multiProcessorCount > 0) hipcus = prop.multiProcessorCount;
+    chol_sched_opts po = d->opt;
+    po.prog_cus = hipcus;
+    bool built = chol_build_program(d->plan, &po, &w, &g) == 0;
+    bool live = built && (g.n_queue > 1 ? chol_program_check_queues(d->plan, &po, 1, 1, &w, &g) : chol_program_check_built(d->plan, &po, 4, &w, &g)) == 0;
+    if (built && !live && g.n_queue > 1) {
+      chol_level_work_free(&w); chol_program_free(&g);
+      po.xcd_queues = 0;
+      built = chol_build_program(d->plan, &po, &w, &g) == 0;
+      live = built && chol_program_check_built(d->plan, &po, 4, &w, &g) == 0;
+    }
     if (built && !live) { chol_level_work_free(&w); chol_program_free(&g); }
     if (live) {
       int rc = upload_level(d->prog, w);
-      std::vector<int> tot(g.ctr_total, g.ctr_total + g.n_ctr);
-      int ncu = 256;
-      hipDeviceProp_t prop;
-      if (hipGetDeviceProperties(&prop, d->dev) == hipSuccess && prop.multiProcessorCount > 0) ncu = prop.multiProcessorCount;
-      d->prog_grid = g.n_job < ncu ? g.n_job : ncu;
-      tot.push_back(g.n_job + d->prog_grid);
+      std::vector<int> tot(g.ctr_total, g.ctr_total + g.n_ctr + g.n_queue);
+      d->prog_grid = g.grid;
+      std::memset(&d->queues, 0, sizeof d->queues);
+      d->queues.n_queue = g.n_queue; d->queues.bound_drawers = g.bound_drawers; d->queues.head0 = g.n_ctr;
+      for (int q = 0; q < g.n_queue; q++) { d->queues.first[q + 1] = d->queues.first[q] + g.q_jobs[q]; d->queues.total[q] = g.ctr_total[g.n_ctr + q]; }
+      d->job_of_slot.assign((size_t)g.n_job, 0);
+      std::vector<chol_job> ordered((size_t)g.n_job);
+      {
+        int fill[CHOL_PROG_QUEUES] = { 0 };
+        for (int j = 0; j < g.n_job; j++) { const int q = g.job[j].queue, at = d->queues.first[q] + fill[q]++; d->job_of_slot[(size_t)at] = j; ordered[(size_t)at] = g.job[j]; }
+      }
       int mx = 1;
       for (int t : tot) mx = t > mx ? t : mx;
       d->prog_epoch_limit = (1 << 30) / mx;
+      if (const char *e = getenv("CHOLAMD_PROG_EPOCH_LIMIT")) { const int v = atoi(e); if (v > 0 && v < d->prog_epoch_limit) d->prog_epoch_limit = v; }
       d->n_job = g.n_job; d->n_pctr = (int)tot.size(); d->prog_epoch = 0;
       d->jobs_host.assign(g.job, g.job + g.n_job);
-      if (!rc) rc = upload_vec(&d->jobs, g.job, (size_t)g.n_job);
+      if (!rc) rc = upload_vec(&d->jobs, ordered.data(), (size_t)g.n_job);
       const chol_wait no_wait = { 0, 0 };
       chol_ext no_ext;
       std::memset(&no_ext, 0, sizeof no_ext);
@@ -344,6 +363,8 @@
   else if (n == "program") d->opt.program = value != 0;
   else if (n == "follow") d->opt.follow = value != 0;
   else if (n == "super_blocks") d->opt.super_blocks = value;
+  else if (n == "xcd_queues") d->opt.xcd_queues = value < 0 ? 0 : value;
+  else if (n == "xcd_drawers") d->opt.xcd_drawers = value < 1 ? 1 : value;
   else if (n == "follow_tail") d->opt.follow_tail = value;
   else if (n == "follow_tail_split") d->opt.follow_tail_split = value;
   else if (n == "staged") d->opt.staged = value != 0;
@@ -651,35 +672,41 @@
   {
     scoped_timer t(d, st, 3, true);
     HIPCHK((hipError_t)chol_launch_program(d_arena, d->ws, d->jobs, d->n_job, d->pwaits, l.potrf, l.trsm, l.task, l.src, d->exts, d->pctr, d->pctr_total, d->prog_epoch,
-                                           d->pctr + d->n_pctr - 1, d->prog_epoch * (d->n_job + d->prog_grid), d->prog_grid, info_cur, info_next, d->trace, st));
+                                           &d->queues, d->prog_grid, info_cur, info_next, d->trace, st));
   }
   d->prog_epoch++;
   return 0;
 }
-extern "C" int cholamd_device_program_trace(cholamd_device *d, double *d_arena, void *stream, int64_t cap, int64_t *out, int *njobs_out)
+static int program_trace(cholamd_device *d, double *d_arena, void *stream, int cols, int64_t cap, int64_t *out, int *njobs_out)
 {
   HIPCHK(hipSetDevice(d->dev));
   if (!d->prog_ready) { chol_set_error("no program launch for this problem / these options"); return CHOLAMD_ERR_ARG; }
   *njobs_out = d->n_job;
-  if (cap < (int64_t)5 * d->n_job) return 0;
+  if (cap < (int64_t)cols * d->n_job) return 0;
   const size_t nst = (size_t)(4 + CHOL_TRACE_X) * d->n_job;
   HIPCHK(hipMalloc((void **)&d->trace, nst * sizeof(unsigned long long)));
   HIPCHK(hipMemset(d->trace, 0, nst * sizeof(unsigned long long)));
   int rc = cholamd_factor(d, d_arena, stream);
-  std::vector<unsigned long long> h(nst);
+  std::vector<unsigned long long> hs(nst), h(nst);
   if (!rc) {
     HIPCHK(hipStreamSynchronize((hipStream_t)stream));
-    HIPCHK(hipMemcpy(h.data(), d->trace, h.size() * sizeof(unsigned long long), hipMemcpyDeviceToHost));
+    HIPCHK(hipMemcpy(hs.data(), d->trace, hs.size() * sizeof(unsigned long long), hipMemcpyDeviceToHost));
   }
   (void)hipFree(d->trace);
   d->trace = nullptr;
   if (rc) return rc;
+  for (int sl = 0; sl < d->n_job; sl++) {
+    const int j = d->job_of_slot[(size_t)sl];
+    std::memcpy(&h[(size_t)4 * j], &hs[(size_t)4 * sl], 4 * sizeof(unsigned long long));
+    std::memcpy(&h[(size_t)4 * d->n_job + (size_t)CHOL_TRACE_X * j], &hs[(size_t)4 * d->n_job + (size_t)CHOL_TRACE_X * sl], CHOL_TRACE_X * sizeof(unsigned long long));
+  }
   unsigned long long t0 = ~0ull;
   for (int j = 0; j < d->n_job; j++) if (h[4 * j] && h[4 * j] < t0) t0 = h[4 * j];
   for (int j = 0; j < d->n_job; j++) {
-    out[5 * j] = d->jobs_host[j].kind + (d->jobs_host[j].kind == 0 && d->jobs_host[j].n_ext > 0 ? 10 : 0);
-    for (int q = 0; q < 3; q++) out[5 * j + 1 + q] = (int64_t)(h[4 * j + q] - t0);
-    out[5 * j + 4] = (int64_t)h[4 * j + 3];
+    out[cols * j] = d->jobs_host[j].kind + (d->jobs_host[j].kind == 0 && d->jobs_host[j].n_ext > 0 ? 10 : 0);
+    for (int q = 0; q < 3; q++) out[cols * j + 1 + q] = (int64_t)(h[4 * j + q] - t0);
+    out[cols * j + 4] = (int64_t)(h[4 * j + 3] & 0xffffffffull);
+    if (cols >= 7) { out[cols * j + 5] = d->jobs_host[j].queue; out[cols * j + 6] = (int64_t)(h[4 * j + 3] >> 32); }
   }
   if (const char *path = getenv("CHOLAMD_TRACE_FOLLOW")) {
     if (FILE *fp = fopen(path, "w")) {
@@ -705,6 +732,14 @@
     }
   }
   return 0;
+}
+extern "C" int cholamd_device_program_trace(cholamd_device *d, double *d_arena, void *stream, int64_t cap, int64_t *out, int *njobs_out)
+{
+  return program_trace(d, d_arena, stream, 5, cap, out, njobs_out);
+}
+extern "C" int cholamd_device_program_trace_queues(cholamd_device *d, double *d_arena, void *stream, int64_t cap, int64_t *out, int *njobs_out)
+{
+  return program_trace(d, d_arena, stream, 7, cap, out, njobs_out);
 }
 extern "C" int cholamd_factor_info(cholamd_device *d, int *sep_out)
 {
diff --git a/cholesky_amd/csrc/chol_kernels.h b/cholesky_amd/csrc/chol_kernels.h
--- a/cholesky_amd/csrc/chol_kernels.h
+++ b/cholesky_amd/csrc/chol_kernels.h
@@ -18,7 +18,7 @@
                            const chol_upd_task *tasks, const chol_upd_src *srcs, int n_task,
                            int *info, int *progress, int progress_base, int *done, int done_target, hipStream_t st);
 int chol_launch_program(double *base, double *ws, const chol_job *jobs, int njobs, const chol_wait *waits, const chol_potrf_desc *pdescs, const chol_trsm_desc *tdescs,
-                        const chol_upd_task *tasks, const chol_upd_src *srcs, const chol_ext *exts, int *ctr, const int *ctr_total, int epoch, int *head, int head_base,
+                        const chol_upd_task *tasks, const chol_upd_src *srcs, const chol_ext *exts, int *ctr, const int *ctr_total, int epoch, const chol_queues *queues,
                         int grid, int *info, int *info_next, unsigned long long *trace, hipStream_t st);
 int chol_launch_trsm_w(double *base, const double *ws, const chol_trsm_desc *descs, int n, hipStream_t st);
 int chol_launch_trsm_wt(double *base, const double *ws, const chol_trsm_desc *descs, int n, hipStream_t st);
diff --git a/cholesky_amd/csrc/chol_kernels.hip b/cholesky_amd/csrc/chol_kernels.hip
--- a/cholesky_amd/csrc/chol_kernels.hip
+++ b/cholesky_amd/csrc/chol_kernels.hip
@@ -1601,13 +1601,15 @@
                                                         const chol_wait *__restrict__ waits, const chol_potrf_desc *__restrict__ pdescs,
                                                         const chol_trsm_desc *__restrict__ tdescs, const chol_upd_task *__restrict__ tasks,
                                                         const chol_upd_src *__restrict__ srcs, const chol_ext *__restrict__ exts,
-                                                        int *__restrict__ ctr, const int *__restrict__ ctr_total, int epoch, int *__restrict__ head, int head_base,
+                                                        int *__restrict__ ctr, const int *__restrict__ ctr_total, int epoch, const chol_queues Q,
                                                         int *__restrict__ info, int *__restrict__ info_next, unsigned long long *__restrict__ trace)
 {
   if (info_next && blockIdx.x == 0 && threadIdx.x == 0) { info_next[0] = 0; info_next[1] = 0; }
   __shared__ double smem[RR_SMEM_DOUBLES];
   __shared__ int s_job;
   const int wave_id = __builtin_amdgcn_readfirstlane(threadIdx.x >> 6);
+  const int q_last = Q.n_queue - 1;
+  int q = Q.n_queue > 1 && (int)(blockIdx.x >> 3) < Q.bound_drawers ? (int)(blockIdx.x & 7) : q_last;
   for (;;) {
 #ifdef TID_PLAIN
     int tid = threadIdx.x;
@@ -1619,12 +1621,27 @@
     const int lane = tid & 63;
     const int grp = wave >> 2;
     __syncthreads();
-    if (tid == 0) s_job = atomicAdd(head, 1) - head_base;
+    if (tid == 0) {
+      int i = atomicAdd(&ctr[Q.head0 + q], 1) - epoch * Q.total[q];
+      int at = Q.first[q], end = Q.first[q + 1];
+      if (i >= end - at && q != q_last) {
+        i = atomicAdd(&ctr[Q.head0 + q_last], 1) - epoch * Q.total[q_last];
+        at = Q.first[q_last]; end = Q.first[q_last + 1];
+      }
+      s_job = (unsigned)i < (unsigned)(end - at) ? at + i : -1;
+    }
     __syncthreads();
     const int j = s_job;
-    if (j >= njobs) break;
+    if (j < 0) break;
+    if (j >= Q.first[q_last]) q = q_last;
     const chol_job jb = jobs[j];
-    if (TR && trace && tid == 0) { trace[4 * j] = __builtin_amdgcn_s_memrealtime(); trace[4 * j + 3] = blockIdx.x; }
+    if constexpr (TR) {
+      if (trace && tid == 0) {
+        unsigned xcc;
+        asm volatile("s_getreg_b32 %0, hwreg(HW_REG_XCC_ID, 0, 4)" : "=s"(xcc));
+        trace[4 * j] = __builtin_amdgcn_s_memrealtime(); trace[4 * j + 3] = (unsigned long long)blockIdx.x | ((unsigned long long)xcc << 32);
+      }
+    }
     chol_upd_task tpre;
     if (jb.kind == 2) {
       const int tk = jb.first + min(jb.mode == 0 ? wave : grp, jb.n - 1);
@@ -3025,12 +3042,13 @@
   return (int)hipGetLastError();
 }
 int chol_launch_program(double *base, double *ws, const chol_job *jobs, int njobs, const chol_wait *waits, const chol_potrf_desc *pdescs, const chol_trsm_desc *tdescs,
-                        const chol_upd_task *tasks, const chol_upd_src *srcs, const chol_ext *exts, int *ctr, const int *ctr_total, int epoch, int *head, int head_base,
+                        const chol_upd_task *tasks, const chol_upd_src *srcs, const chol_ext *exts, int *ctr, const int *ctr_total, int epoch, const chol_queues *queues,
                         int grid, int *info, int *info_next, unsigned long long *trace, hipStream_t st)
 {
   if (njobs <= 0) return 0;
-  if (trace) hipLaunchKernelGGL(k_program<true>, dim3(grid), dim3(RR_THREADS), 0, st, base, ws, jobs, njobs, waits, pdescs, tdescs, tasks, srcs, exts, ctr, ctr_total, epoch, head, head_base, info, info_next, trace);
-  else hipLaunchKernelGGL(k_program<false>, dim3(grid), dim3(RR_THREADS), 0, st, base, ws, jobs, njobs, waits, pdescs, tdescs, tasks, srcs, exts, ctr, ctr_total, epoch, head, head_base, info, info_next, trace);
+  const chol_queues Q = *queues;
+  if (trace) hipLaunchKernelGGL(k_program<true>, dim3(grid), dim3(RR_THREADS), 0, st, base, ws, jobs, njobs, waits, pdescs, tdescs, tasks, srcs, exts, ctr, ctr_total, epoch, Q, info, info_next, trace);
+  else hipLaunchKernelGGL(k_program<false>, dim3(grid), dim3(RR_THREADS), 0, st, base, ws, jobs, njobs, waits, pdescs, tdescs, tasks, srcs, exts, ctr, ctr_total, epoch, Q, info, info_next, trace);
   return (int)hipGetLastError();
 }
 int chol_launch_trsm_w(double *base, const double *ws, const chol_trsm_desc *descs, int n, hipStream_t st)
diff --git a/cholesky_amd/csrc/chol_plan.h b/cholesky_amd/csrc/chol_plan.h
--- a/cholesky_amd/csrc/chol_plan.h
+++ b/cholesky_amd/csrc/chol_plan.h
@@ -137,6 +137,7 @@
   int wait_first, n_wait;
   int sig[2], sig_add;
   int ext_first, n_ext;
+  int queue;
   int mode, n_pre;
 } chol_job;
 typedef struct {
@@ -165,13 +166,22 @@
   return own_at;
 }
 
+#define CHOL_PROG_BOUND 8
+#define CHOL_PROG_QUEUES (CHOL_PROG_BOUND + 1)
+#define CHOL_XCD_DRAWERS 16
+#define CHOL_XCD_QUEUES 0
 typedef struct {
   int n_job; chol_job *job;
   int n_wait; chol_wait *wait;
   int n_ext; chol_ext *ext;
   int n_ctr; int *ctr_total;
   int follow;
+  int n_queue;
+  int grid;
+  int bound_drawers;
+  int q_jobs[CHOL_PROG_QUEUES];
 } chol_program;
+typedef struct { int n_queue, bound_drawers, head0; int first[CHOL_PROG_QUEUES + 1]; int total[CHOL_PROG_QUEUES]; } chol_queues;
 
 typedef struct {
   int kind;
@@ -210,6 +220,9 @@
   int follow_tail;
   int merge_targets;
   int leaf_envelope;
+  int xcd_queues;
+  int xcd_drawers;
+  int prog_cus;
   int super_blocks;
 } chol_sched_opts;
 #define CHOL_SUPER_BLOCKS 3
@@ -281,6 +294,7 @@
 void chol_program_free(chol_program *prog);
 int chol_program_check(const struct cholamd_plan *p, const chol_sched_opts *opts, int workers);
 int chol_program_check_built(const struct cholamd_plan *p, const chol_sched_opts *opts, int workers, const chol_level_work *w, const chol_program *g);
+int chol_program_check_queues(const struct cholamd_plan *p, const chol_sched_opts *opts, int bound, int shared, const chol_level_work *w, const chol_program *g);
 int chol_build_level_work(const struct cholamd_plan *p, const chol_sched_opts *opts , int level, int rank, int world, chol_level_work *out);
 void chol_level_work_free(chol_level_work *w);
 int chol_owner_of(const struct cholamd_plan *p, int label, int world);
diff --git a/cholesky_amd/csrc/chol_schedule.c b/cholesky_amd/csrc/chol_schedule.c
--- a/cholesky_amd/csrc/chol_schedule.c
+++ b/cholesky_amd/csrc/chol_schedule.c
@@ -94,6 +94,7 @@
 {
   o->split_min = CHOL_SPLIT_MIN; o->split_nb = CHOL_SPLIT_NB; o->fuse = 1; o->fuse_update_max = CHOL_FUSE_UPDATE_MAX;
   o->mt_min_tiles = CHOL_MT_MIN_TILES; o->trsm_wt_min = CHOL_TRSM_WT_MIN; o->trsm_group = 0; o->cells = 1; o->program = 1; o->follow = 1; o->super_blocks = CHOL_SUPER_BLOCKS; o->dist_top = 2; o->follow_tail = CHOL_FOLLOW_TAIL; o->follow_tail_split = CHOL_FOLLOW_TAIL; o->staged = 1; o->fine_upd = 1; o->skyline = 1; o->stage_chunk = CHOL_STAGE_CHUNK; o->merge_targets = 1; o->leaf_envelope = 1;
+  o->xcd_queues = CHOL_XCD_QUEUES; o->xcd_drawers = CHOL_XCD_DRAWERS; o->prog_cus = 256;
 }
 void chol_sched_opts_from_env(chol_sched_opts *o)
 {
@@ -117,6 +118,8 @@
   o->merge_targets = !env_int("CHOLAMD_NO_MERGE_TARGETS", 0);
   o->leaf_envelope = !env_int("CHOLAMD_NO_LEAF_ENVELOPE", 0);
   o->stage_chunk = env_int("CHOLAMD_STAGE_CHUNK", o->stage_chunk);
+  o->xcd_queues = env_int("CHOLAMD_XCD_QUEUES", o->xcd_queues);
+  o->xcd_drawers = env_int("CHOLAMD_XCD_DRAWERS", o->xcd_drawers);
 }
 static int split_nb(const chol_sched_opts *o) { int v = o->split_nb; if (v > CHOL_RR_MAXN) v = CHOL_RR_MAXN; v = (v + 15) / 16 * 16; if (v < 16) v = 16; return v; }
 static int pivot_blocks(const chol_sched_opts *o, int n) { return n > o->split_min || n > CHOL_RR_MAXN ? (n + split_nb(o) - 1) / split_nb(o) : 1; }
@@ -765,7 +768,7 @@
 {
   chol_program *g = P->pg;
   if (g->n_job == P->cap_j) { P->cap_j = P->cap_j ? 2 * P->cap_j : 1024; g->job = realloc(g->job, P->cap_j * sizeof(chol_job)); }
-  chol_job j = { kind, first, n, wait_first, g->n_wait - wait_first, { -1, -1 }, 0, g->n_ext, 0, 0, g->n_wait - wait_first };
+  chol_job j = { kind, first, n, wait_first, g->n_wait - wait_first, { -1, -1 }, 0, g->n_ext, 0, 0, 0, g->n_wait - wait_first };
   g->job[g->n_job] = j;
   return &g->job[g->n_job++];
 }
@@ -977,6 +980,61 @@
   free(sc); free(sn); free(sq); free(sch);
 }
 
+static void assign_queues(const plan_t *p, const chol_sched_opts *opts, const chol_level_work *w, chol_program *pg, const int *est_start)
+{
+  const int ns = p->nsep, nj = pg->n_job;
+  const int cus = opts->prog_cus > 0 ? opts->prog_cus : 256;
+  int R = opts->xcd_drawers;
+  pg->grid = nj < cus ? nj : cus;
+  if (R < 1) R = 1;
+  pg->n_queue = opts->xcd_queues > 0 && pg->grid >= CHOL_PROG_BOUND * (R + 1) ? CHOL_PROG_QUEUES : 1;
+  pg->bound_drawers = pg->n_queue > 1 ? R : 0;
+  memset(pg->q_jobs, 0, sizeof pg->q_jobs);
+  for (int j = 0; j < nj; j++) pg->job[j].queue = 0;
+  if (pg->n_queue > 1) {
+    int *sep_of_ctr = calloc(pg->n_ctr > 0 ? pg->n_ctr : 1, sizeof(int)), *sep_of_job = calloc(nj > 0 ? nj : 1, sizeof(int));
+    int *bound = calloc(ns + 1, sizeof(int)), *chain = calloc(ns + 2, sizeof(int)), *group;
+    for (int i = 0; i < w->n_potrf; i++) sep_of_ctr[w->potrf[i].ctr] = w->potrf[i].sep;
+    for (int j = 0; j < nj; j++) {
+      const chol_job *jb = &pg->job[j];
+      if (jb->kind == 0) sep_of_job[j] = w->potrf[jb->first].sep;
+      else if (jb->kind == 1) sep_of_job[j] = sep_of_ctr[w->trsm[jb->first].flag];
+      if (jb->kind <= 1) bound[sep_of_job[j]]++;
+    }
+    int nchain = 1;
+    chain[1] = 0;
+    for (int h = 1; 2 * h <= ns; h++) {
+      int keep = 2 * h;
+      if (2 * h + 1 <= ns) {
+        const int a = p->tree[2 * h], b = p->tree[2 * h + 1];
+        if (est_start[b] + (p->sep_size[b] + CHOL_NB - 1) / CHOL_NB > est_start[a] + (p->sep_size[a] + CHOL_NB - 1) / CHOL_NB) keep = 2 * h + 1;
+      }
+      for (int c = 2 * h; c <= 2 * h + 1 && c <= ns; c++) chain[c] = c == keep ? chain[h] : nchain++;
+    }
+    int *njc = calloc(nchain, sizeof(int)), load[CHOL_PROG_BOUND] = { 0 };
+    group = calloc(nchain, sizeof(int));
+    for (int h = 1; h <= ns; h++) njc[chain[h]] += bound[p->tree[h]];
+    for (int c = 0; c < nchain; c++) {
+      int g = 0;
+      for (int q = 1; q < CHOL_PROG_BOUND; q++) if (load[q] < load[g]) g = q;
+      group[c] = g; load[g] += njc[c];
+    }
+    for (int j = 0; j < nj; j++) {
+      chol_job *jb = &pg->job[j];
+      if (jb->kind <= 1) jb->queue = group[chain[p->heap_of[sep_of_job[j]]]];
+      else if (opts->xcd_queues >= 2 && jb->sig[1] >= 0) jb->queue = group[chain[p->heap_of[p->blk[w->task[jb->first].blk].c]]];
+      else jb->queue = CHOL_PROG_BOUND;
+    }
+    free(sep_of_ctr); free(sep_of_job); free(bound); free(chain); free(njc); free(group);
+  }
+  for (int j = 0; j < nj; j++) pg->q_jobs[pg->job[j].queue]++;
+  pg->ctr_total = realloc(pg->ctr_total, (size_t)(pg->n_ctr + pg->n_queue) * sizeof(int));
+  for (int q = 0; q < pg->n_queue; q++) {
+    int drawers = pg->grid;
+    if (pg->n_queue > 1 && q < CHOL_PROG_BOUND) { drawers = 0; for (int b = q; b < pg->grid && (b >> 3) < pg->bound_drawers; b += CHOL_PROG_BOUND) drawers++; }
+    pg->ctr_total[pg->n_ctr + q] = pg->q_jobs[q] + drawers;
+  }
+}
 static chol_sched_opts chol_program_opts(const chol_sched_opts *o)
 {
   chol_sched_opts r = *o;
@@ -1467,6 +1525,7 @@
   if (!rc && w->n_task_mt > 0) { chol_set_error("program launch: macro-tile update phases"); rc = CHOLAMD_ERR_ARG; }
   if (!rc && w->n_task > PROG_MAX_TASKS) { chol_set_error("program launch: %d update tasks", w->n_task); rc = CHOLAMD_ERR_ARG; }
   for (int s = 1; s <= ns; s++) { pg->ctr_total[c_upd[s]] = cnt_upd[s]; pg->ctr_total[c_updd[s]] = cnt_updd[s]; if (P->c_updp) pg->ctr_total[P->c_updp[s]] = P->cnt_updp[s]; }
+  if (!rc) assign_queues(p, opts, w, pg, est_start);
   free(P->c_updp); free(P->cnt_updp); P->c_updp = P->cnt_updp = NULL;
   for (int s = 1; s <= ns; s++) free(pb[s]);
   free_skylines(sky, ns); free(bw_of); free(band_of); free(sw_of);
@@ -1490,19 +1549,48 @@
   chol_program_free(&g);
   return rc;
 }
+static int program_simulate(const plan_t *p, const chol_sched_opts *opts, int bound, int shared, int use_queues, const chol_level_work *wp, const chol_program *gp);
 int chol_program_check_built(const plan_t *p, const chol_sched_opts *opts, int workers, const chol_level_work *wp, const chol_program *gp)
+{
+  return program_simulate(p, opts, 0, workers, 0, wp, gp);
+}
+int chol_program_check_queues(const plan_t *p, const chol_sched_opts *opts, int bound, int shared, const chol_level_work *wp, const chol_program *gp)
+{
+  return program_simulate(p, opts, bound, shared, 1, wp, gp);
+}
+static int program_simulate(const plan_t *p, const chol_sched_opts *opts, int bound, int shared, int use_queues, const chol_level_work *wp, const chol_program *gp)
 {
   const chol_level_work w = *wp;
   const chol_program g = *gp;
   int rc = 0;
+  if (bound < 0) bound = 0;
+  if (shared < 0) shared = 0;
+  const int nq = use_queues && g.n_queue > 1 ? g.n_queue : 1, last = nq - 1;
+  if (nq == 1) { shared += use_queues ? bound : 0; bound = 0; }
+  const int workers = bound * (nq - 1) + shared;
   int *val = calloc(g.n_ctr > 0 ? g.n_ctr : 1, sizeof(int));
-  char *state = calloc(g.n_job > 0 ? g.n_job : 1, 1);
-  int next = 0, running = 0, done = 0;
+  int *qlist = malloc((g.n_job > 0 ? g.n_job : 1) * sizeof(int)), qfirst[CHOL_PROG_QUEUES + 1] = { 0 }, qnext[CHOL_PROG_QUEUES] = { 0 };
+  for (int j = 0; j < g.n_job; j++) {
+    const int q = nq > 1 ? g.job[j].queue : 0;
+    if (q < 0 || q >= nq) { chol_set_error("program job %d is in queue %d of %d", j, q, nq); rc = CHOLAMD_ERR_ARG; break; }
+    qfirst[q + 1]++;
+  }
+  for (int q = 0; q < nq; q++) qfirst[q + 1] += qfirst[q];
+  if (!rc) { int fill[CHOL_PROG_QUEUES] = { 0 }; for (int j = 0; j < g.n_job; j++) { const int q = nq > 1 ? g.job[j].queue : 0; qlist[qfirst[q] + fill[q]++] = j; } }
+  int *wq = malloc((workers > 0 ? workers : 1) * sizeof(int)), *wjob = malloc((workers > 0 ? workers : 1) * sizeof(int));
+  for (int i = 0; i < workers; i++) { wq[i] = i < bound * (nq - 1) ? i % (nq - 1) : last; wjob[i] = -1; }
+  int done = 0;
   while (done < g.n_job && !rc) {
-    while (running < workers && next < g.n_job) { state[next++] = 1; running++; }
     int progressed = 0;
-    for (int j = 0; j < next; j++) {
-      if (state[j] != 1) continue;
+    for (int i = 0; i < workers; i++)
+      while (wjob[i] < 0 && wq[i] >= 0) {
+        const int q = wq[i];
+        if (qnext[q] < qfirst[q + 1] - qfirst[q]) { wjob[i] = qlist[qfirst[q] + qnext[q]++]; progressed = 1; }
+        else wq[i] = q != last ? last : -1;
+      }
+    for (int i = 0; i < workers; i++) {
+      const int j = wjob[i];
+      if (j < 0) continue;
       const chol_job *jb = &g.job[j];
       int ok = 1;
       for (int q = 0; q < jb->n_wait && ok; q++) {
@@ -1520,22 +1608,24 @@
       if (!ok) continue;
       if (jb->kind == 0) val[w.potrf[jb->first].ctr] = g.ctr_total[w.potrf[jb->first].ctr];
       if (jb->kind == 1)
-        for (int i = jb->first; i < jb->first + jb->n; i++)
-          if (w.trsm[i].chan >= 0 && w.trsm[i].m > 0)
-            for (int t = 0; t < (w.trsm[i].n + CHOL_NB - 1) / CHOL_NB; t++) val[w.trsm[i].chan + t]++;
+        for (int t2 = jb->first; t2 < jb->first + jb->n; t2++)
+          if (w.trsm[t2].chan >= 0 && w.trsm[t2].m > 0)
+            for (int t = 0; t < (w.trsm[t2].n + CHOL_NB - 1) / CHOL_NB; t++) val[w.trsm[t2].chan + t]++;
       for (int q = 0; q < 2; q++) if (jb->sig[q] >= 0) val[jb->sig[q]] += jb->sig_add;
-      state[j] = 2; running--; done++; progressed = 1;
-    }
-    if (!rc && !progressed && (running == workers || next == g.n_job)) {
-      int j = 0;
-      while (j < next && state[j] != 1) j++;
-      chol_set_error("program dead-locks with %d resident workgroups: job %d (kind %d) can never run; %d of %d jobs done", workers, j, j < g.n_job ? g.job[j].kind : -1, done, g.n_job);
+      wjob[i] = -1; done++; progressed = 1;
+    }
+    if (!rc && !progressed) {
+      int j = -1;
+      for (int i = 0; i < workers; i++) if (wjob[i] >= 0 && (j < 0 || wjob[i] < j)) j = wjob[i];
+      if (j < 0) for (int q = 0; q < nq && j < 0; q++) if (qnext[q] < qfirst[q + 1] - qfirst[q]) j = qlist[qfirst[q] + qnext[q]];
+      chol_set_error("program dead-locks with %d + %d resident workgroups on %d queue(s): job %d (kind %d) can never run; %d of %d jobs done", bound, shared, nq, j, j >= 0 && j < g.n_job ? g.job[j].kind : -1, done, g.n_job);
       rc = CHOLAMD_ERR_ARG;
     }
   }
+  free(qlist); free(wq); free(wjob);
   for (int c = 0; c < g.n_ctr && !rc; c++)
     if (val[c] != g.ctr_total[c]) { chol_set_error("program counter %d ends at %d, total %d", c, val[c], g.ctr_total[c]); rc = CHOLAMD_ERR_ARG; }
-  free(val); free(state);
+  free(val);
   if (!rc) {
     quad *a = NULL, *b = NULL;
     int64_t na = 0, nb = 0, ca = 0, cb = 0;
@@ -1577,11 +1667,48 @@
   if (split_nb >= 0) o.split_nb = split_nb;
   return chol_program_check(p, &o, workers);
 }
-int64_t cholamd_plan_program_jobs(const cholamd_plan *p, int follow, int64_t cap, int *out)
+int cholamd_plan_program_check_queues(const cholamd_plan *p, int follow, int xcd_queues, int bound_drawers, int shared_drawers)
 {
   chol_sched_opts o;
   chol_sched_opts_default(&o);
   o.follow = follow;
+  if (xcd_queues >= 0) o.xcd_queues = xcd_queues;
+  chol_level_work w; chol_program g;
+  int rc = chol_build_program(p, &o, &w, &g);
+  if (rc) return rc;
+  rc = chol_program_check_queues(p, &o, bound_drawers, shared_drawers, &w, &g);
+  chol_level_work_free(&w); chol_program_free(&g);
+  return rc;
+}
+int64_t cholamd_plan_program_queues(const cholamd_plan *p, int follow, int xcd_queues, int xcd_drawers, int grid_max, int64_t cap, int *out)
+{
+  chol_sched_opts o;
+  chol_sched_opts_default(&o);
+  o.follow = follow;
+  if (xcd_queues >= 0) o.xcd_queues = xcd_queues;
+  if (xcd_drawers >= 0) o.xcd_drawers = xcd_drawers;
+  if (grid_max >= 0) o.prog_cus = grid_max;
+  chol_level_work w; chol_program g;
+  if (chol_build_program(p, &o, &w, &g)) return -1;
+  const int64_t need = 12 + (int64_t)g.n_job;
+  if (cap >= need) {
+    out[0] = g.n_queue; out[1] = g.grid; out[2] = g.bound_drawers;
+    for (int q = 0; q < CHOL_PROG_QUEUES; q++) out[3 + q] = q < g.n_queue ? g.ctr_total[g.n_ctr + q] : 0;
+    for (int j = 0; j < g.n_job; j++) out[12 + j] = g.job[j].queue;
+  }
+  chol_level_work_free(&w); chol_program_free(&g);
+  return need;
+}
+int64_t cholamd_plan_program_jobs(const cholamd_plan *p, int follow, int64_t cap, int *out)
+{
+  return cholamd_plan_program_jobs_queues(p, follow, -1, cap, out);
+}
+int64_t cholamd_plan_program_jobs_queues(const cholamd_plan *p, int follow, int xcd_queues, int64_t cap, int *out)
+{
+  chol_sched_opts o;
+  chol_sched_opts_default(&o);
+  o.follow = follow;
+  if (xcd_queues >= 0) o.xcd_queues = xcd_queues;
   chol_level_work w; chol_program g;
   if (chol_build_program(p, &o, &w, &g)) return -1;
   const int64_t need = (int64_t)8 * g.n_job + (int64_t)3 * g.n_wait + 1;
diff --git a/cholesky_amd/device.py b/cholesky_amd/device.py
--- a/cholesky_amd/device.py
+++ b/cholesky_amd/device.py
@@ -140,11 +140,12 @@
     def set_option(self, name, value):
         check(self.L.cholamd_device_set_option(self.h, name.encode(), int(value)), "cholamd_device_set_option")
 
-    def program_trace(self, arena, stream=None):
+    def program_trace(self, arena, stream=None, queues=False):
         n = C.c_int(0)
-        check(self.L.cholamd_device_program_trace(self.h, self.ptr(arena), _stream_ptr(stream), 0, None, C.byref(n)), "cholamd_device_program_trace")
-        out = np.zeros((n.value, 5), dtype=np.int64)
-        check(self.L.cholamd_device_program_trace(self.h, self.ptr(arena), _stream_ptr(stream), out.size, out.ctypes.data, C.byref(n)), "cholamd_device_program_trace")
+        fn = self.L.cholamd_device_program_trace_queues if queues else self.L.cholamd_device_program_trace
+        check(fn(self.h, self.ptr(arena), _stream_ptr(stream), 0, None, C.byref(n)), "cholamd_device_program_trace")
+        out = np.zeros((n.value, 7 if queues else 5), dtype=np.int64)
+        check(fn(self.h, self.ptr(arena), _stream_ptr(stream), out.size, out.ctypes.data, C.byref(n)), "cholamd_device_program_trace")
         return out
 
     def tail_offset(self):
diff --git a/cholesky_amd/plan.py b/cholesky_amd/plan.py
--- a/cholesky_amd/plan.py
+++ b/cholesky_amd/plan.py
@@ -236,12 +236,28 @@
         check(self.L.cholamd_plan_program_counts(self.h, int(follow), out.ctypes.data), "cholamd_plan_program_counts")
         return dict(zip(("jobs", "followers", "tasks", "strips", "counters", "followed_panels"), (int(v) for v in out)))
 
-    def program_jobs(self, follow=True):
-        need = self.L.cholamd_plan_program_jobs(self.h, int(follow), 0, None)
-        buf = np.zeros(need, dtype=np.int32)
-        self.L.cholamd_plan_program_jobs(self.h, int(follow), need, buf.ctypes.data)
+    def program_jobs(self, follow=True, xcd_queues=None):
+        if xcd_queues is None:
+            need = self.L.cholamd_plan_program_jobs(self.h, int(follow), 0, None)
+            buf = np.zeros(need, dtype=np.int32)
+            self.L.cholamd_plan_program_jobs(self.h, int(follow), need, buf.ctypes.data)
+        else:
+            need = self.L.cholamd_plan_program_jobs_queues(self.h, int(follow), int(xcd_queues), 0, None)
+            buf = np.zeros(need, dtype=np.int32)
+            self.L.cholamd_plan_program_jobs_queues(self.h, int(follow), int(xcd_queues), need, buf.ctypes.data)
         nj = int(buf[-1])
         return buf[:8 * nj].reshape(nj, 8), buf[8 * nj:-1].reshape(-1, 3)
+
+    def program_queues(self, follow=True, xcd_queues=-1, xcd_drawers=-1, grid_max=-1):
+        need = self.L.cholamd_plan_program_queues(self.h, int(follow), int(xcd_queues), int(xcd_drawers), int(grid_max), 0, None)
+        check(0 if need >= 0 else int(need), "cholamd_plan_program_queues")
+        buf = np.zeros(need, dtype=np.int32)
+        self.L.cholamd_plan_program_queues(self.h, int(follow), int(xcd_queues), int(xcd_drawers), int(grid_max), need, buf.ctypes.data)
+        nq = int(buf[0])
+        return dict(queues=nq, grid=int(buf[1]), bound_drawers=int(buf[2]), head_totals=buf[3:3 + nq].copy(), queue=buf[12:].copy())
+
+    def program_check_queues(self, follow=True, xcd_queues=-1, bound_drawers=1, shared_drawers=1):
+        check(self.L.cholamd_plan_program_check_queues(self.h, int(follow), int(xcd_queues), int(bound_drawers), int(shared_drawers)), "cholamd_plan_program_check_queues")
 
     def arena_to_dense(self, arena):
         arena = np.ascontiguousarray(arena, dtype=np.float64)
diff --git a/include/cholamd.h b/include/cholamd.h
--- a/include/cholamd.h
+++ b/include/cholamd.h
@@ -119,6 +119,9 @@
 int cholamd_follow_rounds(int n_ext, int tile_columns, int cap, int *rounds_out, int *own_at_out);
 int64_t cholamd_plan_program_followers(const cholamd_plan *p, int64_t cap, int *out);
 int64_t cholamd_plan_program_jobs(const cholamd_plan *p, int follow, int64_t cap, int *out);
+int64_t cholamd_plan_program_jobs_queues(const cholamd_plan *p, int follow, int xcd_queues, int64_t cap, int *out);
+int64_t cholamd_plan_program_queues(const cholamd_plan *p, int follow, int xcd_queues, int xcd_drawers, int grid_max, int64_t cap, int *out);
+int cholamd_plan_program_check_queues(const cholamd_plan *p, int follow, int xcd_queues, int bound_drawers, int shared_drawers);
 int cholamd_plan_arena_to_dense(const cholamd_plan *p, const double *arena, double *dense);
 int cholamd_plan_write_matrix(const cholamd_plan *p, const double *arena, const char *file, int full_precision);
 int cholamd_write_solution(const char *file, const double *x, int n, int full_precision);
@@ -154,6 +157,7 @@
 int cholamd_factor_levels(cholamd_device *d, double *d_arena, int level_hi, int level_lo, void *stream);
 int cholamd_device_set_partition(cholamd_device *d, int rank, int world);
 int cholamd_device_program_trace(cholamd_device *d, double *d_arena, void *stream, int64_t cap, int64_t *out, int *njobs_out);
+int cholamd_device_program_trace_queues(cholamd_device *d, double *d_arena, void *stream, int64_t cap, int64_t *out, int *njobs_out);
 int cholamd_factor_debug(cholamd_device *d, double *d_arena, const char *dir, int full_precision, void *stream);
 int cholamd_factor_info(cholamd_device *d, int *sep_out);
 int cholamd_device_set_option(cholamd_device *d, const char *name, int value);
```

After: 765.3 GF/s. 4.4% lower.
